# rileyhales/river-route

Hardware: AMD Instinct MI355X
Metric: reach-steps/sec (higher is better)
Workload: dtype f64

## Files before the change

### include/rr_hip.h

```cpp
#ifndef RR_HIP_H
#define RR_HIP_H

#include <stdint.h>

#ifdef __cplusplus
extern "C" {
#endif

#define RR_OK 0
#define RR_E_INVALID (-1)
#define RR_E_NOT_TOPOLOGICAL (-2)
#define RR_E_HIP (-3)
#define RR_E_NO_DEVICE (-4)
#define RR_E_STATE (-5)
#define RR_E_ALLOC (-6)
#define RR_E_UNSUPPORTED (-7)

#define RR_DEVICE_NONE (-1)

typedef struct rr_plan rr_plan;

int rr_version(void);
const char *rr_last_error(void);
int rr_device_count(void);


int rr_plan_create(int64_t n, const int32_t *csc_indptr, const int32_t *csc_indices, int device, rr_plan **out);
void rr_plan_destroy(rr_plan *plan);

int rr_plan_info(const rr_plan *plan, int64_t info[8]);

int rr_plan_layout(const rr_plan *plan, int32_t *perm, int32_t *lag, int32_t *child_ptr);

int rr_plan_tile_info(const rr_plan *plan, int64_t info[8]);
int rr_plan_tile_layout(const rr_plan *plan, int32_t *tile_ptr, int32_t *tile_level, int32_t *perm, int32_t *lag,
                        int32_t *cfirst, uint32_t *ccnt, int32_t *xpos);

int rr_plan_set_coeffs(rr_plan *plan, const double *lhs_off_data, const double *c2, const double *c3,
                       const double *c4_dt);

int rr_plan_set_unit_weights(rr_plan *plan, const double *c1, const double *a_data);

#define RR_MODE_RAPID 0
#define RR_MODE_MUSKINGUM 1
#define RR_MODE_UNIT 2
#define RR_ROWS_NOT_PLAIN 2
#define RR_ROWS_F32_OUT 4
#define RR_ROWS_UH 8
int rr_plan_reserve(rr_plan *plan, int mode, int64_t T, int64_t nsub, int host_rows, int64_t info[8]);

int rr_plan_direct_info(const rr_plan *plan, int64_t info[8], char *why, int64_t why_cap);
int rr_plan_direct_layout(const rr_plan *plan, int32_t *tile_c0, int32_t *tile_nc, int32_t *tile_lag_lo, int32_t *tile_span,
                          int32_t *delay, int32_t *up3, int32_t *xinfo);
int rr_plan_profile_aux(rr_plan *plan, double aux[12]);
#define RR_KERNEL_TICK 0
#define RR_KERNEL_TILE 1
#define RR_KERNEL_DIRECT 2
#define RR_KERNEL_TILE_ENSEMBLE 3
int rr_plan_last_kernel(const rr_plan *plan);

int rr_plan_set_row_format(rr_plan *plan, int in32_big_endian, int out32_big_endian);

int rr_plan_set_options(rr_plan *plan, int64_t rows_per_chunk, int64_t sample_every);

int rr_plan_profile(rr_plan *plan, double prof[10]);


int rr_rapid_route(rr_plan *plan, double *q_t, const double *qlateral, double *discharge,
                   int64_t num_runoff_steps, int64_t num_substeps);

int rr_muskingum_route(rr_plan *plan, double *q_t, double *discharge,
                       int64_t num_output_steps, int64_t num_routing_per_output);

int rr_unit_route(rr_plan *plan, double *q_ch, double *q_full, const double *convolved_lateral,
                  double *discharge, int64_t num_runoff_steps, int64_t num_substeps);

int rr_uh_convolve(int device, const double *kernel, double *state, const double *lateral, double *out,
                   int64_t T, int64_t n_ks, int64_t n);


int rr_rapid_route_dev(rr_plan *plan, double *q_t, const double *qlateral, int64_t ql_rows,
                       double *discharge, int64_t out_rows, int64_t num_runoff_steps, int64_t num_substeps,
                       void *stream);
int rr_muskingum_route_dev(rr_plan *plan, double *q_t, double *discharge, int64_t out_rows,
                           int64_t num_output_steps, int64_t num_routing_per_output, void *stream);
int rr_unit_route_dev(rr_plan *plan, double *q_ch, double *q_full, const double *convolved_lateral,
                      int64_t conv_rows, double *discharge, int64_t out_rows,
                      int64_t num_runoff_steps, int64_t num_substeps, void *stream);
int rr_uh_convolve_dev(int device, const double *kernel, double *state, const double *lateral, double *out,
                       int64_t T, int64_t n_ks, int64_t n, void *stream);

int rr_rapid_route_f32_dev(rr_plan *plan, double *q_t, const double *qlateral, int64_t ql_rows, float *discharge32,
                           int64_t num_runoff_steps, int64_t num_substeps, int64_t factor, void *stream);
int rr_rapid_route_f32in_dev(rr_plan *plan, double *q_t, const float *qlateral32, int64_t ql_rows, double *discharge, int64_t out_rows,
                             float *discharge32, int64_t factor, int64_t T, int64_t nsub, void *stream);

#define RR_ROWS_F32_IN 16
int rr_plan_reserve_ensemble(rr_plan *plan, int64_t members, int64_t T, int64_t nsub, int flags, int64_t info[9]);
int rr_rapid_route_ensemble_dev(rr_plan *plan, int64_t members, double *q_t, int64_t q_pitch, const void *lateral, int lateral_is_f32,
                                int64_t lateral_member_pitch, void *discharge, int discharge_is_f32, int64_t discharge_member_pitch,
                                int64_t factor, int64_t T, int64_t nsub, void *stream);
int rr_muskingum_route_f32_dev(rr_plan *plan, double *q_t, float *discharge32, int64_t num_output_steps,
                               int64_t num_routing_per_output, void *stream);
int rr_unit_route_f32_dev(rr_plan *plan, double *q_ch, double *q_full, const double *convolved_lateral, int64_t conv_rows,
                          float *discharge32, int64_t num_runoff_steps, int64_t num_substeps, int64_t factor, void *stream);

int rr_rapid_route_runoff_dev(rr_plan *plan, double *q_t, int64_t n_points, const int32_t *indptr, const int32_t *indices,
                              const double *weights, const void *runoff, int runoff_is_f32, int64_t stride_t, int64_t stride_p,
                              const double *area, int flags, double *discharge, float *discharge32, int64_t factor,
                              int64_t num_runoff_steps, void *stream);

int rr_unit_route_uh_dev(rr_plan *plan, double *q_ch, double *q_full, double *q_final, const double *uh_kernel, double *uh_state,
                         int64_t n_ks, const double *depth, double *discharge, float *discharge32, int64_t factor,
                         int64_t num_runoff_steps, int64_t num_substeps, void *stream);
int rr_unit_route_uh_f32in_dev(rr_plan *plan, double *q_ch, double *q_full, double *q_final, const double *uh_kernel, double *uh_state,
                               int64_t n_ks, const float *depth32, double *discharge, float *discharge32, int64_t factor,
                               int64_t num_runoff_steps, int64_t num_substeps, void *stream);


int rr_plan_set_boundary(rr_plan *plan, int64_t n_ghost, const int64_t *ghost_reaches, int64_t n_export,
                         const int64_t *export_reaches);

int rr_stream_begin(rr_plan *plan, int has_lateral, const double *q_t, const double *lateral, int64_t lat_rows,
                    double *discharge, int64_t out_rows, int64_t T, int64_t nsub, const double *ghost_series,
                    double *export_series, void *stream);
int rr_stream_advance(rr_plan *plan, int64_t lateral_rows_ready, int64_t ghost_substeps_ready,
                      int64_t *export_substeps_ready);
int rr_stream_end(rr_plan *plan, double *q_t);

int rr_stream_begin_unit(rr_plan *plan, const double *q_ch, const double *q_full, const double *lateral, int64_t lat_rows,
                         double *discharge, int64_t out_rows, int64_t T, int64_t nsub, const double *ghost_series,
                         double *export_series, void *stream);
int rr_stream_end_unit(rr_plan *plan, double *q_ch, double *q_full);

int rr_partition_forest(int64_t n, const int32_t *csc_indptr, const int32_t *csc_indices, int32_t n_parts,
                        int32_t *part_of, int64_t *part_sizes);

int rr_postorder(int64_t n, const int64_t *down_index, int64_t *order);

int rr_resample_cast_dev(int device, const double *discharge, int64_t num_rows, int64_t n, int64_t factor, float *out,
                         void *stream);

#define RR_RUNOFF_CUMULATIVE 1
#define RR_RUNOFF_FORCE_POSITIVE 2
#define RR_RUNOFF_KEEP_NAN 4
int rr_runoff_to_qlateral(int device, int64_t n_rivers, int64_t n_points, int64_t T, const int32_t *indptr,
                          const int32_t *indices, const double *weights, const void *runoff, int runoff_is_f32,
                          int64_t stride_t, int64_t stride_p, const double *area, int flags, double *qlateral);
int rr_runoff_to_qlateral_dev(int device, int64_t n_rivers, int64_t n_points, int64_t T, const int32_t *indptr,
                              const int32_t *indices, const double *weights, const void *runoff, int runoff_is_f32,
                              int64_t stride_t, int64_t stride_p, const double *area, int flags, double *qlateral,
                              void *stream);

#define RR_METRICS_STATE 9
#define RR_METRICS_SCORES 5
int rr_metrics_work_bytes(int64_t n, int64_t rows, int64_t *bytes);
int rr_metrics_update_dev(int device, int64_t n, int64_t rows, const void *y_true, int true_is_f32, int64_t true_pitch,
                          const void *y_pred, int pred_is_f32, int64_t pred_pitch, const int32_t *pred_columns, double *state,
                          void *work, int64_t work_bytes, void *stream);
int rr_metrics_finish_dev(int device, int64_t n, const double *state, double *out, void *stream);

int rr_grid_overlap_area(int device, int64_t n_rows, int64_t n_rings, int64_t n_vertices, int64_t nx, int64_t ny, int64_t n_pairs,
                         const int64_t *row_rings, const int64_t *ring_offsets, const double *ring_weight, const double *lon,
                         const double *lat, const double *x_bounds, const double *y_bounds, const int32_t *row_cells,
                         const int64_t *pair_offsets, double *area);
int rr_grid_overlap_area_dev(int device, int64_t n_rows, int64_t n_rings, int64_t n_vertices, int64_t nx, int64_t ny, int64_t n_pairs,
                             const int64_t *row_rings, const int64_t *ring_offsets, const double *ring_weight, const double *lon,
                             const double *lat, const double *x_bounds, const double *y_bounds, const int32_t *row_cells,
                             const int64_t *pair_offsets, double *area, void *stream);

int rr_rapid_adjoint_work_bytes(rr_plan *plan, int64_t T, int64_t nsub, int64_t *bytes);
int rr_rapid_adjoint_dev(rr_plan *plan, const double *q0, const double *lateral, int64_t lat_rows, const double *discharge,
                         const double *grad_out, const double *grad_qfinal, double *grad_lateral, double *grad_q0, double *grad_coef,
                         void *work, int64_t work_bytes, int64_t T, int64_t nsub, void *stream);

int rr_rapid_adjoint_batch_work_bytes(rr_plan *plan, int64_t members, int64_t T, int64_t nsub, int64_t *bytes);
int rr_rapid_adjoint_batch_dev(rr_plan *plan, int64_t members, const double *q0, int64_t q0_pitch, const double *lateral, int64_t lat_rows,
                               int64_t lat_pitch, const double *discharge, const double *grad_out, int64_t out_pitch,
                               const double *grad_qfinal, double *grad_lateral, double *grad_q0, double *grad_coef, void *work,
                               int64_t work_bytes, int64_t T, int64_t nsub, void *stream);

int rr_unit_adjoint_work_bytes(rr_plan *plan, int64_t T, int64_t nsub, int64_t *bytes);
int rr_unit_adjoint_dev(rr_plan *plan, const double *q_ch0, const double *q_full0, const double *lateral, int64_t lat_rows,
                        const double *discharge, const double *grad_out, const double *grad_qch_final, const double *grad_qfull_final,
                        double *grad_lateral, double *grad_qch0, double *grad_qfull0, double *grad_coef, void *work, int64_t work_bytes,
                        int64_t T, int64_t nsub, void *stream);

// ... 35 lines not shown
```

### river_route_amd/_lib.py

```python
from __future__ import annotations

import ctypes as C
import importlib.util
import os
import subprocess

import numpy as np

_HERE = os.path.dirname(os.path.abspath(__file__))
LIB_PATH = os.environ.get('RR_LIB_PATH') or os.path.join(_HERE, 'librr_hip.so')
CSRC = os.path.join(_HERE, 'csrc')
SOURCES = ('rr_plan.cpp', 'rr_engine.hip')

RR_OK = 0
RR_E_INVALID, RR_E_NOT_TOPOLOGICAL, RR_E_HIP, RR_E_NO_DEVICE, RR_E_STATE, RR_E_ALLOC, RR_E_UNSUPPORTED = \
    -1, -2, -3, -4, -5, -6, -7
RR_DEVICE_NONE = -1


class RRError(RuntimeError):
    def __init__(self, code: int, message: str):
        super().__init__(f'librr_hip error {code}: {message}')
        self.code = code
        self.message = message


SANITIZED_LIB_PATH = os.path.join(_HERE, 'librr_hip_asan.so')


def sanitizer_runtime() -> str | None:
    import glob
    found = sorted(glob.glob('/opt/rocm/lib/llvm/lib/clang/*/lib/linux/libclang_rt.asan-x86_64.so'))
    return found[-1] if found else None


def build(force: bool = False, verbose: bool = False, sanitize: bool = False) -> str:
    srcs = [os.path.join(CSRC, s) for s in SOURCES]
    deps = srcs + [os.path.join(CSRC, f) for f in sorted(os.listdir(CSRC)) if f.endswith('.hpp')] + [os.path.join(os.path.dirname(_HERE), 'include', 'rr_hip.h')]
    target = SANITIZED_LIB_PATH if sanitize else LIB_PATH
    if not force and os.path.exists(target) and all(os.path.getmtime(target) >= os.path.getmtime(d) for d in deps):
        return target
    hipcc = os.environ.get('HIPCC') or ('/opt/rocm/bin/hipcc' if os.path.exists('/opt/rocm/bin/hipcc') else 'hipcc')
    opt = ['-O1', '-g', '-fsanitize=address,undefined', '-fno-gpu-sanitize', '-fno-omit-frame-pointer', '-shared-libsan'] if sanitize else ['-O3']
    cmd = [hipcc, '--offload-arch=gfx950', *opt, '-std=c++17', '-fPIC', '-shared', '-pthread', '-Wall', '-Wno-unused-result',
           *srcs, '-o', target]
    if verbose:
        print(' '.join(cmd))
    subprocess.check_call(cmd)
    return target


def _preload_hip_runtime() -> None:
    try:
        spec = importlib.util.find_spec('torch')
    except (ImportError, ValueError):
        spec = None
    if spec is None or not spec.origin:
        return
    cand = os.path.join(os.path.dirname(spec.origin), 'lib', 'libamdhip64.so')
    if os.path.exists(cand):
        try:
            C.CDLL(cand, mode=C.RTLD_GLOBAL)
        except OSError:
            pass


_i64 = C.c_int64
_vp = C.c_void_p
_lib: C.CDLL | None = None

_SIGNATURES = {
    'rr_version': (C.c_int, []),
    'rr_last_error': (C.c_char_p, []),
    'rr_device_count': (C.c_int, []),
    'rr_plan_create': (C.c_int, [_i64, _vp, _vp, C.c_int, C.POINTER(_vp)]),
    'rr_plan_destroy': (None, [_vp]),
    'rr_plan_info': (C.c_int, [_vp, _vp]),
    'rr_plan_layout': (C.c_int, [_vp, _vp, _vp, _vp]),
    'rr_plan_tile_info': (C.c_int, [_vp, _vp]),
    'rr_plan_tile_layout': (C.c_int, [_vp, _vp, _vp, _vp, _vp, _vp, _vp, _vp]),
    'rr_plan_direct_info': (C.c_int, [_vp, _vp, _vp, _i64]),
    'rr_plan_direct_layout': (C.c_int, [_vp, _vp, _vp, _vp, _vp, _vp, _vp, _vp]),
    'rr_plan_last_kernel': (C.c_int, [_vp]),
    'rr_plan_set_coeffs': (C.c_int, [_vp, _vp, _vp, _vp, _vp]),
    'rr_plan_set_unit_weights': (C.c_int, [_vp, _vp, _vp]),
    'rr_plan_reserve': (C.c_int, [_vp, C.c_int, _i64, _i64, C.c_int, _vp]),
    'rr_plan_set_options': (C.c_int, [_vp, _i64, _i64]),
    'rr_plan_set_row_format': (C.c_int, [_vp, C.c_int, C.c_int]),
    'rr_plan_profile': (C.c_int, [_vp, _vp]),
    'rr_plan_profile_aux': (C.c_int, [_vp, _vp]),
    'rr_rapid_route': (C.c_int, [_vp, _vp, _vp, _vp, _i64, _i64]),
    'rr_muskingum_route': (C.c_int, [_vp, _vp, _vp, _i64, _i64]),
    'rr_unit_route': (C.c_int, [_vp, _vp, _vp, _vp, _vp, _i64, _i64]),
    'rr_uh_convolve': (C.c_int, [C.c_int, _vp, _vp, _vp, _vp, _i64, _i64, _i64]),
    'rr_rapid_route_dev': (C.c_int, [_vp, _vp, _vp, _i64, _vp, _i64, _i64, _i64, _vp]),
    'rr_muskingum_route_dev': (C.c_int, [_vp, _vp, _vp, _i64, _i64, _i64, _vp]),
    'rr_unit_route_dev': (C.c_int, [_vp, _vp, _vp, _vp, _i64, _vp, _i64, _i64, _i64, _vp]),
    'rr_uh_convolve_dev': (C.c_int, [C.c_int, _vp, _vp, _vp, _vp, _i64, _i64, _i64, _vp]),
    'rr_rapid_route_runoff_dev': (C.c_int, [_vp, _vp, _i64, _vp, _vp, _vp, _vp, C.c_int, _i64, _i64, _vp, C.c_int, _vp, _vp, _i64, _i64, _vp]),
    'rr_unit_route_uh_dev': (C.c_int, [_vp, _vp, _vp, _vp, _vp, _vp, _i64, _vp, _vp, _vp, _i64, _i64, _i64, _vp]),
    'rr_unit_route_uh_f32in_dev': (C.c_int, [_vp, _vp, _vp, _vp, _vp, _vp, _i64, _vp, _vp, _vp, _i64, _i64, _i64, _vp]),
    'rr_rapid_route_f32_dev': (C.c_int, [_vp, _vp, _vp, _i64, _vp, _i64, _i64, _i64, _vp]),
    'rr_rapid_route_f32in_dev': (C.c_int, [_vp, _vp, _vp, _i64, _vp, _i64, _vp, _i64, _i64, _i64, _vp]),
    'rr_plan_reserve_ensemble': (C.c_int, [_vp, _i64, _i64, _i64, C.c_int, _vp]),
    'rr_rapid_route_ensemble_dev': (C.c_int, [_vp, _i64, _vp, _i64, _vp, C.c_int, _i64, _vp, C.c_int, _i64, _i64, _i64, _i64, _vp]),
    'rr_muskingum_route_f32_dev': (C.c_int, [_vp, _vp, _vp, _i64, _i64, _vp]),
    'rr_unit_route_f32_dev': (C.c_int, [_vp, _vp, _vp, _vp, _i64, _vp, _i64, _i64, _i64, _vp]),
    'rr_plan_set_boundary': (C.c_int, [_vp, _i64, _vp, _i64, _vp]),
    'rr_stream_begin': (C.c_int, [_vp, C.c_int, _vp, _vp, _i64, _vp, _i64, _i64, _i64, _vp, _vp, _vp]),
    'rr_stream_advance': (C.c_int, [_vp, _i64, _i64, C.POINTER(_i64)]),
    'rr_stream_end': (C.c_int, [_vp, _vp]),
    'rr_stream_begin_unit': (C.c_int, [_vp, _vp, _vp, _vp, _i64, _vp, _i64, _i64, _i64, _vp, _vp, _vp]),
    'rr_stream_end_unit': (C.c_int, [_vp, _vp, _vp]),
    'rr_partition_forest': (C.c_int, [_i64, _vp, _vp, C.c_int32, _vp, _vp]),
    'rr_postorder': (C.c_int, [_i64, _vp, _vp]),
    'rr_resample_cast_dev': (C.c_int, [C.c_int, _vp, _i64, _i64, _i64, _vp, _vp]),
    'rr_runoff_to_qlateral': (C.c_int, [C.c_int, _i64, _i64, _i64, _vp, _vp, _vp, _vp, C.c_int, _i64, _i64, _vp, C.c_int, _vp]),
    'rr_runoff_to_qlateral_dev': (C.c_int, [C.c_int, _i64, _i64, _i64, _vp, _vp, _vp, _vp, C.c_int, _i64, _i64, _vp,
                                            C.c_int, _vp, _vp]),
    'rr_metrics_work_bytes': (C.c_int, [_i64, _i64, C.POINTER(_i64)]),
    'rr_metrics_update_dev': (C.c_int, [C.c_int, _i64, _i64, _vp, C.c_int, _i64, _vp, C.c_int, _i64, _vp, _vp, _vp, _i64, _vp]),
    'rr_metrics_finish_dev': (C.c_int, [C.c_int, _i64, _vp, _vp, _vp]),
    'rr_grid_overlap_area': (C.c_int, [C.c_int, _i64, _i64, _i64, _i64, _i64, _i64, _vp, _vp, _vp, _vp, _vp, _vp, _vp, _vp, _vp, _vp]),
    'rr_grid_overlap_area_dev': (C.c_int, [C.c_int, _i64, _i64, _i64, _i64, _i64, _i64, _vp, _vp, _vp, _vp, _vp, _vp, _vp, _vp, _vp, _vp,
                                           _vp]),
    'rr_rapid_adjoint_work_bytes': (C.c_int, [_vp, _i64, _i64, C.POINTER(_i64)]),
    'rr_rapid_adjoint_dev': (C.c_int, [_vp, _vp, _vp, _i64, _vp, _vp, _vp, _vp, _vp, _vp, _vp, _i64, _i64, _i64, _vp]),
    'rr_rapid_adjoint_batch_work_bytes': (C.c_int, [_vp, _i64, _i64, _i64, C.POINTER(_i64)]),
    'rr_rapid_adjoint_batch_dev': (C.c_int, [_vp, _i64, _vp, _i64, _vp, _i64, _i64, _vp, _vp, _i64, _vp, _vp, _vp, _vp, _vp, _i64, _i64, _i64, _vp]),
    'rr_unit_adjoint_work_bytes': (C.c_int, [_vp, _i64, _i64, C.POINTER(_i64)]),
    'rr_unit_adjoint_dev': (C.c_int, [_vp, _vp, _vp, _vp, _i64, _vp, _vp, _vp, _vp, _vp, _vp, _vp, _vp, _vp, _i64, _i64, _i64, _vp]),
    'rr_unit_adjoint_batch_work_bytes': (C.c_int, [_vp, _i64, _i64, _i64, C.POINTER(_i64)]),
    'rr_unit_adjoint_batch_dev': (C.c_int, [_vp, _i64, _vp, _vp, _i64, _vp, _i64, _i64, _vp, _vp, _i64, _vp, _vp, _vp, _vp, _vp, _vp, _vp, _i64,
                                            _i64, _i64, _vp]),
    'rr_uh_adjoint_work_bytes': (C.c_int, [_i64, _i64, _i64, C.POINTER(_i64)]),
    'rr_uh_adjoint_dev': (C.c_int, [C.c_int, _vp, _vp, _vp, _vp, _vp, _vp, _vp, _vp, _i64, _i64, _i64, _i64, _vp]),
    'rr_metrics_adjoint_work_bytes': (C.c_int, [_i64, C.POINTER(_i64)]),
    'rr_metrics_adjoint_dev': (C.c_int, [C.c_int, _i64, _i64, _vp, C.c_int, _i64, _vp, C.c_int, _i64, _vp, _vp, _i64, _vp, _vp, _vp, _vp, _i64,
                                         _vp, _i64, _vp]),
    'rr_dev_malloc': (C.c_int, [C.c_int, _i64, C.POINTER(_vp)]),
    'rr_dev_free': (C.c_int, [C.c_int, _vp]),
    'rr_dev_upload': (C.c_int, [C.c_int, _vp, _vp, _i64]),
    'rr_dev_download': (C.c_int, [C.c_int, _vp, _vp, _i64]),
    'rr_dev_synchronize': (C.c_int, [C.c_int]),
    'rr_copy_bandwidth': (C.c_int, [C.c_int, _i64, C.c_int, C.POINTER(C.c_double)]),
    'rr_rows_upload': (C.c_int, [C.c_int, _vp, _i64, C.c_char_p, _i64, _i64, _i64, _i64, _vp]),
    'rr_rows_download': (C.c_int, [C.c_int, _vp, _i64, C.c_char_p, _i64, _i64, _i64, _i64, _vp]),
}
EXPORTS = tuple(_SIGNATURES)


def lib() -> C.CDLL:
    global _lib
    if _lib is None:
        if not os.path.exists(LIB_PATH):
            raise RuntimeError(
                f'{LIB_PATH} is missing: the HIP engine is not built and there is no CPU fallback. '
                'Run `python -c "import __graft_entry__ as g; g.build()"` (needs hipcc) first.')
        _preload_hip_runtime()
        handle = C.CDLL(LIB_PATH)
        for name, (res, args) in _SIGNATURES.items():
            fn = getattr(handle, name)
            fn.restype = res
            fn.argtypes = args
        _lib = handle
    return _lib


def check(rc: int) -> None:
    if rc != RR_OK:
        raise RRError(rc, lib().rr_last_error().decode('utf-8', 'replace'))


def device_count() -> int:
    return int(lib().rr_device_count())


def ptr(a) -> int | None:
    if a is None:
        return None
    if isinstance(a, int):
        return a
    if isinstance(a, np.ndarray):
        if not a.flags['C_CONTIGUOUS']:
            raise ValueError('array must be C-contiguous')
        return a.ctypes.data
    if hasattr(a, 'address'):
        return int(a.address)
    if hasattr(a, 'data_ptr'):
        if not a.is_contiguous():
            raise ValueError('tensor must be contiguous')
        return a.data_ptr()
    raise TypeError(f'cannot take the address of {type(a).__name__}')
```

### river_route_amd/csrc/rr_engine.hip

```cpp
#include "rr_common.hpp"
#include "rr_kernels_tick.hpp"
#include "rr_kernels_tile.hpp"
#include "rr_kernels_uh.hpp"
#include "rr_kernels_rec.hpp"
#include "rr_kernels_runoff.hpp"
#include "rr_kernels_direct.hpp"
#include "rr_kernels_metrics.hpp"
#include "rr_kernels_overlap.hpp"
#include "rr_kernels_adjoint.hpp"
#include "rr_kernels_adjoint_unit.hpp"
#include "rr_exec.hpp"


extern "C" {

int rr_version(void) { return RR_VERSION_NUM; }

const char *rr_last_error(void) { return g_err.c_str(); }

int rr_device_count(void)
{
    int c = 0;
    if (hipGetDeviceCount(&c) != hipSuccess) return 0;
    return c;
}

void rr_plan_destroy(rr_plan *P)
{
    if (!P) return;
    if (P->device >= 0 && hipSetDevice(P->device) == hipSuccess) {
        void *ptrs[] = {P->d_child_ptr, P->d_lag, P->d_perm, P->d_inv, P->d_inner_pos, P->d_bidx, P->d_hwc, P->d_w, P->d_c1row_h, P->d_c2,
                        P->d_coef, P->d_coef_unit, P->d_sq, P->d_ss, P->d_si, P->d_sqch, P->d_full, P->d_chan,
                        P->d_tmeta, P->d_pmeta,
                        P->d_tperm, P->d_tinv, P->d_inner_idx, P->d_colmeta, P->d_ghostmeta, P->d_c4_params,
                        P->d_c3, P->d_c4, P->d_x, P->d_isum, P->d_qch, P->d_a2, P->d_c1own, P->d_z, P->d_ring, P->d_stage, P->d_mrows,
                        P->d_slot_a[0], P->d_slot_a[1], P->d_slot_b[0], P->d_slot_b[1], P->d_m_index[0], P->d_m_index[1],
                        P->d_dtiles, P->d_dlane, P->d_dsend_ptr, P->d_dsend_lane, P->d_dcoef, P->d_dq, P->d_ktmeta, P->d_kpmeta, P->d_kperm, P->d_kholecol, P->d_kcoef, P->d_ksq, P->d_kss, P->d_ksi, P->d_ksqch,
                        P->d_kholemeta, P->d_kghostmeta, P->d_esq, P->d_ess, P->d_esi, P->d_adj_down};
        for (void *p : ptrs) if (p) (void)hipFree(p);
        P->pipe.destroy();
        for (hipEvent_t e : P->ev) (void)hipEventDestroy(e);
        for (hipEvent_t e : P->aux_ev) (void)hipEventDestroy(e);
        if (P->ev_first) (void)hipEventDestroy(P->ev_first);
        if (P->ev_last) (void)hipEventDestroy(P->ev_last);
    }
    delete P;
}

int rr_plan_create(int64_t n, const int32_t *csc_indptr, const int32_t *csc_indices, int device, rr_plan **out)
{
    if (!out) return fail(RR_E_INVALID, "rr_plan_create: null out");
    *out = nullptr;
    rr_plan *P = new (std::nothrow) rr_plan();
    if (!P) return fail(RR_E_ALLOC, "rr_plan_create: out of memory");
    if (const char *e = getenv("RR_WAVE")) { P->wave_enabled = atoi(e) != 0; P->wave_forced = atoi(e) == 1; }
    if (const char *e = getenv("RR_REC_BATCHES")) { P->rec_batches = std::max(1, std::min(kRecMaxLaunchBatches, atoi(e))); P->rec_batches_forced = true; }
    if (const char *e = getenv("RR_WAVE_K")) P->wave_K = std::max(kRec, atoi(e) / kRec * kRec);
    std::string err;
    int rc = rr::build_host_plan(n, csc_indptr, csc_indices, P->h, err);
    if (rc) { delete P; return fail(rc, err); }
    if (device != RR_DEVICE_NONE) {
        int count = rr_device_count(), cus = 0;
        if (device >= 0 && device < count && hipDeviceGetAttribute(&cus, hipDeviceAttributeMultiprocessorCount, device) == hipSuccess && cus > 0) P->cu_count = cus;
    }
    {
        P->wave_threads = kTileThreads;
        int32_t block = P->wave_threads;
        if (const char *e = getenv("RR_TILE_BLOCK")) block = std::max(8, std::min(block, atoi(e)));
        std::vector<int32_t> lag_of((size_t)n);
        for (int64_t i = 0; i < n; ++i) lag_of[i] = P->h.lag[P->h.inv[i]];
        rr::build_tile_plan(P->h.down, lag_of, block, P->tp);
        if (const char *e = getenv("RR_DIRECT")) P->direct_enabled = atoi(e) != 0;
        P->direct_block = block;
        rr::build_direct_plan(P->h.down, lag_of, std::min<int32_t>(kDirectLanes, block), kDirectMaxWindow - 2, block, P->dp);
        P->direct_window = 3;
        for (int32_t sp : P->dp.tile_span) P->direct_window = std::max(P->direct_window, sp + 3);
    }
    if (device != RR_DEVICE_NONE) {
        int count = rr_device_count();
        if (device < 0 || device >= count) {
            delete P;
            return fail(RR_E_NO_DEVICE, "rr_plan_create: HIP device " + std::to_string(device) + " not available (" +
                                            std::to_string(count) + " visible)");
        }
        hipError_t e = hipSetDevice(device);
        if (e != hipSuccess) { delete P; return fail(RR_E_HIP, hipGetErrorString(e)); }
        P->device = device;
        {
            size_t free_b = 0, total_b = 0;
            if (hipMemGetInfo(&free_b, &total_b) == hipSuccess) P->dev_total_bytes = total_b;
        }
        if (const char *e2 = getenv("RR_TILE_LEAN")) P->lean_enabled = atoi(e2) != 0;
        for (int v = 0; v < 7; ++v)
            if (hipFuncSetAttribute((const void *)tile_kernel(v < 4 ? (v & 1) != 0 : v == 5, v < 4 && (v & 2) != 0, v >= 4, v == 6), hipFuncAttributeMaxDynamicSharedMemorySize,
                                    (int)tile_lds_bytes(P->wave_threads)) != hipSuccess) {
                (void)hipGetLastError();
                P->wave_enabled = false;
            }
        for (int v = 0; v < 2; ++v)
            if (hipFuncSetAttribute((const void *)tile_ens_kernel(v == 1), hipFuncAttributeMaxDynamicSharedMemorySize, (int)tile_lds_bytes(kTileThreads)) != hipSuccess) {
                (void)hipGetLastError();
                P->ens_enabled = false;
            }
        if (const char *e2 = getenv("RR_UH_PAIRS")) P->uh_pairs = atoi(e2) != 0;
        for (int v = 0; v < 4; ++v)
            (void)hipFuncSetAttribute((const void *)rec_in_uh_kernel((v & 1) != 0, 64, 1 + (v >> 1)), hipFuncAttributeMaxDynamicSharedMemorySize, (int)rec_in_uh_lds_bytes(64, 1 + (v >> 1)));
        (void)hipGetLastError();
        const rr::HostPlan &H = P->h;
        const int64_t ni = (int64_t)H.inner_pos.size();
        rc = dev_alloc(&P->d_child_ptr, n + 1);
        if (!rc) rc = dev_alloc(&P->d_lag, n);
        if (!rc) rc = dev_alloc(&P->d_perm, n);
        if (!rc) rc = dev_alloc(&P->d_inv, n);
        if (!rc) rc = dev_alloc(&P->d_inner_pos, ni);
        if (!rc) rc = dev_alloc(&P->d_hwc, n);
        if (!rc) rc = dev_alloc(&P->d_bidx, n);
        if (!rc) rc = dev_alloc(&P->d_c4_params, n);
        if (!rc && P->tp.ok) {
            const rr::TilePlan &TP = P->tp;
            const int64_t np = TP.np;
            std::vector<int2> cm(n);
            for (int64_t i = 0; i < n; ++i)
                cm[i] = make_int2(TP.inv[i], (TP.lag[TP.inv[i]] & kLagMask) | (H.child_ptr[H.inv[i] + 1] == H.child_ptr[H.inv[i]] ? kColHeadwater : 0));
            std::vector<int32_t> inner_idx;
            inner_idx.reserve(ni);
            for (int64_t i = 0; i < n; ++i) if (H.child_ptr[H.inv[i] + 1] > H.child_ptr[H.inv[i]]) inner_idx.push_back((int32_t)i);
            rc = dev_alloc(&P->d_colmeta, n);
            if (!rc) rc = dev_upload(P->d_colmeta, cm);
            if (!rc) rc = dev_alloc(&P->d_inner_idx, ni);
            if (!rc) rc = dev_upload(P->d_inner_idx, inner_idx);
            if (!rc) rc = upload_tile_meta(P, TP.lag, TP.xpos, TP.tile_flags);
            for (int32_t f : TP.tile_flags) P->n_wide_tiles += (f & kTileWide) ? 1 : 0;
            if (!rc) rc = dev_alloc(&P->d_tperm, np);
            if (!rc) rc = dev_upload(P->d_tperm, TP.perm);
            if (!rc) rc = dev_alloc(&P->d_tinv, n);
            if (!rc) rc = dev_upload(P->d_tinv, TP.inv);
            if (!rc) rc = dev_alloc(&P->d_coef, 3 * np);
            if (!rc) rc = dev_alloc(&P->d_coef_unit, 3 * np);
            if (!rc) rc = dev_alloc(&P->d_sq, np);
            if (!rc) rc = dev_alloc(&P->d_ss, np);
            if (!rc) rc = dev_alloc(&P->d_si, np);
            if (!rc) rc = dev_alloc(&P->d_sqch, np);
            if (!rc) rc = dev_alloc(&P->d_full, n);
            if (!rc) rc = dev_alloc(&P->d_chan, n);
        }
        if (!rc) rc = upload_direct_plan(P);
        if (!rc) rc = dev_alloc(&P->d_w, n);
        if (!rc) rc = dev_alloc(&P->d_c1row_h, n);
        if (!rc) rc = dev_alloc(&P->d_c2, n);
        if (!rc) rc = dev_alloc(&P->d_c3, n);
        if (!rc) rc = dev_alloc(&P->d_c4, n);
        if (!rc) rc = dev_alloc(&P->d_x, 3 * n);
        if (!rc) rc = dev_alloc(&P->d_isum, n);
        if (!rc) rc = dev_alloc(&P->d_qch, n);
        if (!rc) rc = dev_upload(P->d_child_ptr, H.child_ptr);
        if (!rc) rc = dev_upload(P->d_lag, H.lag);
        if (!rc) rc = dev_upload(P->d_perm, H.perm);
        if (!rc) rc = dev_upload(P->d_inv, H.inv);
        if (!rc) rc = dev_upload(P->d_inner_pos, H.inner_pos);
        if (!rc) rc = dev_upload(P->d_hwc, H.hw_children);
        if (rc) { rr_plan_destroy(P); return rc; }
    }
    *out = P;
    return RR_OK;
}

int rr_plan_info(const rr_plan *P, int64_t info[8])
{
    if (!P || !info) return fail(RR_E_INVALID, "rr_plan_info: null argument");
    info[0] = P->h.n; info[1] = P->h.n_edges; info[2] = P->h.depth; info[3] = P->h.widest_level;
    info[4] = P->h.n_headwaters; info[5] = P->h.n_outlets; info[6] = P->h.identity ? 1 : 0; info[7] = P->device;
    return RR_OK;
}

int rr_plan_layout(const rr_plan *P, int32_t *perm, int32_t *lag, int32_t *child_ptr)
{
    if (!P) return fail(RR_E_INVALID, "rr_plan_layout: null plan");
    const size_t n = (size_t)P->h.n;
    if (perm && n) std::memcpy(perm, P->h.perm.data(), n * sizeof(int32_t));
    if (lag && n) std::memcpy(lag, P->h.lag.data(), n * sizeof(int32_t));
    if (child_ptr) std::memcpy(child_ptr, P->h.child_ptr.data(), (n + 1) * sizeof(int32_t));
    return RR_OK;
}

int rr_plan_tile_info(const rr_plan *P, int64_t info[8])
{
    if (!P || !info) return fail(RR_E_INVALID, "rr_plan_tile_info: null argument");
    const rr::TilePlan &T = P->tp;
    info[0] = T.ok ? 1 : 0; info[1] = T.block; info[2] = T.np; info[3] = T.n_ghost; info[4] = T.n_tiles; info[5] = T.n_levels;
    info[6] = P->wave_threads; info[7] = kRecRows;
    return RR_OK;
}

int rr_plan_tile_layout(const rr_plan *P, int32_t *tile_ptr, int32_t *tile_level, int32_t *perm, int32_t *lag, int32_t *cfirst,
                        uint32_t *ccnt, int32_t *xpos)
{
    if (!P) return fail(RR_E_INVALID, "rr_plan_tile_layout: null plan");
    const rr::TilePlan &T = P->tp;
    if (!T.ok) return fail(RR_E_UNSUPPORTED, "rr_plan_tile_layout: this network does not tile (a reach has more upstream reaches than a tile holds)");
    auto copy = [](auto *dst, const auto &src) { if (dst && !src.empty()) std::memcpy(dst, src.data(), src.size() * sizeof(src[0])); };
    copy(tile_ptr, T.tile_ptr); copy(tile_level, T.tile_level); copy(perm, T.perm); copy(lag, T.lag); copy(cfirst, T.cfirst);
    copy(ccnt, T.ccnt); copy(xpos, T.xpos);
    return RR_OK;
}

int rr_plan_direct_info(const rr_plan *P, int64_t info[8], char *why, int64_t why_cap)
{
    if (!P || !info) return fail(RR_E_INVALID, "rr_plan_direct_info: null argument");
    const rr::DirectPlan &D = P->dp;
    info[0] = D.ok ? 1 : 0; info[1] = D.n_tiles; info[2] = D.n_holes; info[3] = D.n_exports; info[4] = D.skel.np; info[5] = D.skel.n_tiles;
    info[6] = D.skel.n_levels; info[7] = P->direct_window;
    if (why && why_cap > 0) { std::strncpy(why, D.why.c_str(), (size_t)why_cap - 1); why[why_cap - 1] = 0; }
    return RR_OK;
}

int rr_plan_direct_layout(const rr_plan *P, int32_t *tile_c0, int32_t *tile_nc, int32_t *tile_lag_lo, int32_t *tile_span, int32_t *delay, int32_t *up3, int32_t *xinfo)
{
    if (!P) return fail(RR_E_INVALID, "rr_plan_direct_layout: null plan");
    const rr::DirectPlan &D = P->dp;
    if (!D.ok) return fail(RR_E_UNSUPPORTED, "rr_plan_direct_layout: the direct row path does not apply to this plan: " + D.why);
    auto copy = [](auto *dst, const auto &src) { if (dst && !src.empty()) std::memcpy(dst, src.data(), src.size() * sizeof(src[0])); };
    copy(tile_c0, D.tile_c0); copy(tile_nc, D.tile_nc); copy(tile_lag_lo, D.tile_lag_lo); copy(tile_span, D.tile_span);
    copy(delay, D.delay); copy(up3, D.up3); copy(xinfo, D.xinfo);
    return RR_OK;
}

int rr_plan_last_kernel(const rr_plan *P)
{
    if (!P) return -1;
    return P->ses.members > 0 ? RR_KERNEL_TILE_ENSEMBLE : (int)P->ses.kernel;
}

int rr_plan_set_options(rr_plan *P, int64_t rows_per_chunk, int64_t sample_every)
{
    if (!P) return fail(RR_E_INVALID, "rr_plan_set_options: null plan");
    if (rows_per_chunk > 0) P->chunk_rows = rows_per_chunk;
    if (sample_every >= 0) P->sample_every = sample_every;
    return RR_OK;
}

int rr_plan_set_row_format(rr_plan *P, int in32_big_endian, int out32_big_endian)
{
    if (!P) return fail(RR_E_INVALID, "rr_plan_set_row_format: null plan");
    if (P->ses.open) return fail(RR_E_STATE, "rr_plan_set_row_format: a routing call is open");
    P->in32_big_endian = in32_big_endian != 0; P->out32_big_endian = out32_big_endian != 0;
    return RR_OK;
}

int rr_plan_set_coeffs(rr_plan *P, const double *lhs_off_data, const double *c2, const double *c3, const double *c4_dt)
{
    int rc = need_device(P);
    if (rc) return rc;
    const rr::HostPlan &H = P->h;
    const int64_t n = H.n;
    if (n > 0 && (!c2 || !c3 || (H.n_edges > 0 && !lhs_off_data)))
        return fail(RR_E_INVALID, "rr_plan_set_coeffs: null coefficient array");
    std::vector<double> w(n), a2(n), a3(n), a4(n, 0.0);
    for (int64_t p = 0; p < n; ++p) {
        const int32_t i = H.perm[p];
        const int32_t e = H.edge_of[i];
        w[p] = e >= 0 ? -lhs_off_data[e] : 0.0;
        a2[p] = c2[i];
        a3[p] = c3[i];
        if (c4_dt) a4[p] = c4_dt[i];
    }
    std::vector<double> c1row(n, 0.0);
    bool uniform = true;
    for (int64_t p = 0; p < n; ++p) {
        const int32_t u0 = H.child_ptr[p], u1 = H.child_ptr[p + 1];
        if (u1 > u0) c1row[p] = w[u0];
        for (int32_t u = u0 + 1; u < u1; ++u) if (w[u] != w[u0]) uniform = false;
    }
    P->weights_uniform = uniform;
    rc = dev_upload(P->d_w, w);
    if (!rc) rc = dev_upload(P->d_c1row_h, c1row);
    if (!rc && P->tp.ok) {
        const rr::TilePlan &TP = P->tp;
        P->h_coef.assign(3 * TP.np, 0.0);
        for (int64_t p = 0; p < TP.np; ++p) {
            if (TP.lag[p] & kTileGhostBit) continue;
            const int32_t i = TP.perm[p];
            P->h_coef[3 * p] = c1row[H.inv[i]]; P->h_coef[3 * p + 1] = c2[i]; P->h_coef[3 * p + 2] = c3[i];
        }
        rc = upload_tile_coef(P);
    }
    {
        P->h_dcoef.assign(4 * (size_t)n, 0.0);
        for (int64_t i = 0; i < n; ++i) { P->h_dcoef[4 * i] = c1row[H.inv[i]]; P->h_dcoef[4 * i + 1] = c2[i]; P->h_dcoef[4 * i + 2] = c3[i]; P->h_dcoef[4 * i + 3] = c4_dt ? c4_dt[i] : 0.0; }
        if (!rc) rc = upload_direct_coef(P);
    }
    if (!rc) rc = dev_upload(P->d_c2, a2);
    if (!rc) rc = dev_upload(P->d_c3, a3);
    if (!rc) rc = dev_upload(P->d_c4, a4);
    if (!rc && c4_dt && n > 0) {
        hipError_t e = hipMemcpy(P->d_c4_params, c4_dt, (size_t)n * sizeof(double), hipMemcpyHostToDevice);
        if (e != hipSuccess) rc = fail(RR_E_HIP, hipGetErrorString(e));
    }
    if (rc) return rc;
    P->coeffs_set = true;
    P->has_c4 = c4_dt != nullptr;
    return RR_OK;
}

int rr_plan_set_unit_weights(rr_plan *P, const double *c1, const double *a_data)
{
    int rc = need_device(P);
    if (rc) return rc;
    if (P->ses.open) return fail(RR_E_STATE, "rr_plan_set_unit_weights: a routing call is open");
    if (!c1 && !a_data) { P->unit_general = false; return RR_OK; }
    const rr::HostPlan &H = P->h;
    const int64_t n = H.n;
    if (!c1 || (H.n_edges > 0 && !a_data)) return fail(RR_E_INVALID, "rr_plan_set_unit_weights: give both arrays, or neither to go back to unit weights");
    if (P->n_ghost > 0 || P->n_export > 0) return fail(RR_E_UNSUPPORTED, "rr_plan_set_unit_weights: general edge data on a partitioned network is not supported");
    std::vector<double> a2(n, 0.0), own(n, 0.0);
    for (int64_t p = 0; p < n; ++p) {
        const int32_t i = H.perm[p], e = H.edge_of[i];
        a2[p] = e >= 0 ? a_data[e] : 0.0;
        own[p] = c1[i];
    }
    if (!P->d_a2) rc = dev_alloc(&P->d_a2, n);
    if (!rc && !P->d_c1own) rc = dev_alloc(&P->d_c1own, n);
    if (!rc && !P->d_z) rc = dev_alloc(&P->d_z, 3 * n);
    if (!rc) rc = dev_upload(P->d_a2, a2);
    if (!rc) rc = dev_upload(P->d_c1own, own);
    if (rc) return rc;
    P->unit_general = true;
    return RR_OK;
}

int rr_plan_reserve(rr_plan *P, int mode, int64_t T, int64_t nsub, int host_rows, int64_t info[8])
{
    int rc = need_device(P);
    if (rc) return rc;
    if (mode < RR_MODE_RAPID || mode > RR_MODE_UNIT || T < 0 || nsub < 1) return fail(RR_E_INVALID, "rr_plan_reserve: unknown mode, negative step count or sub-steps < 1");
    if (!P->coeffs_set) return fail(RR_E_STATE, "rr_plan_reserve before rr_plan_set_coeffs (per-edge weights decide which kernel routes)");
    if (P->ses.open) return fail(RR_E_STATE, "rr_plan_reserve: a routing call is open");
    const Mode m = mode == RR_MODE_RAPID ? Mode::Rapid : (mode == RR_MODE_MUSKINGUM ? Mode::Muskingum : Mode::Unit);
    CallShape shape;
    shape.mode = m; shape.T = T; shape.nsub = nsub;
    shape.host = (host_rows & 1) != 0;
    shape.dev_rows = !shape.host && (host_rows & RR_ROWS_NOT_PLAIN) == 0;
    shape.out32 = (host_rows & RR_ROWS_F32_OUT) != 0;
    shape.uh = (host_rows & RR_ROWS_UH) != 0;
// ... 1210 lines not shown
```

### river_route_amd/csrc/rr_exec.hpp

```cpp
#pragma once


enum class Mode { Rapid, Muskingum, Unit };

struct Rows {
    const double *dev_in = nullptr;
    const float *dev_in32 = nullptr;
    const double *host_in = nullptr;
    int64_t rows_in = 0;
    double *dev_out = nullptr;
    double *host_out = nullptr;
    int64_t rows_out = 0;
    float *dev_out32 = nullptr;
    int64_t out_factor = 1;
    const double *uh_kernel = nullptr, *uh_state = nullptr;
    int64_t uh_nks = 0;
    const RunoffArgs *runoff = nullptr;
    int64_t members = 0, in_pitch = 0, out_pitch = 0;
};

struct CallShape {
    Mode mode = Mode::Rapid;
    int64_t T = 0, nsub = 1;
    bool host = false;
    bool dev_rows = false;
    bool in32 = false;
    bool out32 = false;
    int64_t factor = 1;
    bool uh = false;
    bool runoff = false;
    int64_t ring_in = 0, ring_out = 0;
    int64_t members = 0;
};

enum class Kernel { Tick = RR_KERNEL_TICK, Tile = RR_KERNEL_TILE, Direct = RR_KERNEL_DIRECT };

struct Schedule {
    Kernel kernel = Kernel::Tick;
    int64_t KC = 1;
    int64_t KS = 1;
    int64_t chunks = 0;
    int64_t ring = 0;
    int64_t mrows = 0, stage = 0;
    int64_t rec_nb = 1;
};

struct Session {
    bool open = false;
    Mode mode = Mode::Rapid;
    int64_t T = 0, nsub = 1, total = 0, total_ticks = 0;
    Rows io;
    hipStream_t stream = nullptr;
    Kernel kernel = Kernel::Tick;
    bool in_place = false;
    bool has_in = true;
    int64_t ring_rows = 0;
    int64_t rows_loaded = 0, rows_stored = 0, tau = 0;
    const double *ghost_series = nullptr;
    double *export_series = nullptr;
    TickArgs a{};
    int64_t KC = 1;
    int64_t rec_chunks = 0, in_batches = 0, n_in_batches = 0, out_batches = 0, n_out_batches = 0;
    int64_t rec_nb = 1;
    int64_t ticks_stored = 0;
    int64_t out_limit = std::numeric_limits<int64_t>::max();
    int64_t diag = 0, n_diags = 0, n_macro = 0;
    int64_t ghost_batches = 0;
    int64_t ghost_slack = 0, export_skew = 0;
    TileArgs ta{};
    int64_t n_tasks = 0;
    int64_t d_done = 0;
    int64_t KS = 1;
    bool export_lanes = false, export_skel = false;
    DirectArgs da{};
    bool bracket_open = false;
    int64_t bracket_reaches = 0;
    size_t max_samples = 0;
    int64_t members = 0;
    int64_t ring_stride = 0;
};

struct HostPipe {
    static constexpr int kPinned = 3, kCopyThreads = 8;
    int copy_threads = kCopyThreads;
    int64_t chunk_mib = 512;
    int64_t chunk_rows = 64, ring_chunks = 8;
    double *pin_in[kPinned] = {nullptr, nullptr, nullptr}, *pin_out[kPinned] = {nullptr, nullptr, nullptr};
    double *dev_in = nullptr, *dev_out = nullptr;
    int64_t pin_cap = 0, dev_cap = 0;
    hipStream_t s_h2d = nullptr, s_d2h = nullptr;
    std::vector<hipEvent_t> ev_h2d, ev_d2h, ev_adv;
    void destroy()
    {
        for (int k = 0; k < kPinned; ++k) { if (pin_in[k]) (void)hipHostFree(pin_in[k]); if (pin_out[k]) (void)hipHostFree(pin_out[k]); pin_in[k] = pin_out[k] = nullptr; }
        if (dev_in) (void)hipFree(dev_in);
        if (dev_out) (void)hipFree(dev_out);
        dev_in = dev_out = nullptr; pin_cap = dev_cap = 0;
        for (auto *v : {&ev_h2d, &ev_d2h, &ev_adv}) { for (hipEvent_t e : *v) (void)hipEventDestroy(e); v->clear(); }
        if (s_h2d) (void)hipStreamDestroy(s_h2d);
        if (s_d2h) (void)hipStreamDestroy(s_d2h);
        s_h2d = s_d2h = nullptr;
    }
};

struct rr_plan {
    rr::HostPlan h;
    int device = RR_DEVICE_NONE;
    bool coeffs_set = false, has_c4 = false;
    int64_t chunk_rows = 16, sample_every = 0;

    int32_t *d_child_ptr = nullptr, *d_lag = nullptr, *d_perm = nullptr, *d_inv = nullptr, *d_inner_pos = nullptr;
    int32_t *d_bidx = nullptr;
    uint16_t *d_hwc = nullptr;
    double *d_w = nullptr, *d_c1row_h = nullptr, *d_c2 = nullptr, *d_c3 = nullptr, *d_c4 = nullptr;
    double *d_x = nullptr, *d_isum = nullptr, *d_qch = nullptr;
    double *d_a2 = nullptr, *d_c1own = nullptr, *d_z = nullptr;
    bool unit_general = false;
    double *d_ring = nullptr;
    int64_t ring_cap = 0;
    double *d_stage = nullptr;
    int64_t stage_cap = 0;
    double *d_mrows = nullptr;
    int64_t mrows_cap = 0;
    uint16_t *d_slot_a[2] = {nullptr, nullptr}, *d_slot_b[2] = {nullptr, nullptr};
    int32_t *d_m_index[2] = {nullptr, nullptr};
    int64_t perm_rows_per_block = 2;

    rr::TilePlan tp;
    bool wave_enabled = true, wave_forced = false, weights_uniform = false;
    bool ens_enabled = true;
    int wave_threads = 512;
    int64_t wave_K = 0;
    Schedule sch;
    int64_t kc_cap = int64_t{1} << 20;
    TileMeta *d_tmeta = nullptr;
    int4 *d_pmeta = nullptr;
    int32_t *d_tperm = nullptr, *d_tinv = nullptr;
    int32_t *d_inner_idx = nullptr;
    bool export_inside = false;
    double *d_coef = nullptr;
    double *d_coef_unit = nullptr;
    std::vector<double> h_coef;
    int32_t n_wide_tiles = 0;
    double *d_sq = nullptr, *d_ss = nullptr, *d_si = nullptr, *d_sqch = nullptr;
    double *d_esq = nullptr, *d_ess = nullptr, *d_esi = nullptr;
    int64_t ens_cap = 0;
    double *d_full = nullptr, *d_chan = nullptr;
    int2 *d_colmeta = nullptr;
    int2 *d_ghostmeta = nullptr;
    double *d_c4_params = nullptr;
    size_t dev_total_bytes = 0;
    int cu_count = 256;

    int64_t n_ghost = 0, n_export = 0;
    int64_t ghost_min_lag = 0, export_max_lag = 0;
    std::vector<int32_t> ghost_reach, export_reach;

    Session ses;
    HostPipe pipe;
    rr::DirectPlan dp;
    bool direct_enabled = true;
    bool uh_rows_ok = true;
    int direct_window = 1;
    DirectTile *d_dtiles = nullptr;
    int4 *d_dlane = nullptr;
    int32_t *d_dsend_ptr = nullptr, *d_dsend_lane = nullptr;
    double *d_dcoef = nullptr, *d_dq = nullptr;
    TileMeta *d_ktmeta = nullptr;
    int4 *d_kpmeta = nullptr;
    int32_t *d_kperm = nullptr, *d_kholecol = nullptr;
    double *d_kcoef = nullptr, *d_ksq = nullptr, *d_kss = nullptr, *d_ksi = nullptr, *d_ksqch = nullptr;
    int2 *d_kholemeta = nullptr;
    int2 *d_kghostmeta = nullptr;
    std::vector<double> h_dcoef;
    int32_t direct_block = 0;
    int64_t n_kholes = 0;
    int32_t n_kwide = 0;
    bool in32_big_endian = false, out32_big_endian = false;
    bool lean_enabled = true;
    bool uh_pairs = true;
    int32_t rec_batches = kRecLaunchBatches;
    bool rec_batches_forced = false;
    bool perm_ready = false;
    int32_t *d_adj_down = nullptr;

    static constexpr int kAuxKinds = 4, kAuxSamples = 256;
    std::vector<hipEvent_t> aux_ev;
    std::vector<int> aux_kind;
    int64_t aux_launches[kAuxKinds] = {0, 0, 0, 0};
    std::vector<hipEvent_t> ev;
    std::vector<int64_t> ev_reaches;
    hipEvent_t ev_first = nullptr, ev_last = nullptr;
    int64_t prof_launches = 0, prof_samples = 0, prof_brackets = 0, prof_reach_steps = 0;
    hipStream_t last_stream = nullptr;
};

namespace {

template <typename T>
int dev_alloc(T **p, int64_t count)
{
    *p = nullptr;
    if (count <= 0) count = 1;
    hipError_t e = hipMalloc((void **)p, (size_t)count * sizeof(T));
    if (e != hipSuccess)
        return fail(RR_E_ALLOC, std::string("hipMalloc of ") + std::to_string((size_t)count * sizeof(T)) +
                                    " bytes failed: " + hipGetErrorString(e));
    return RR_OK;
}

template <typename T>
int dev_upload(T *dst, const std::vector<T> &src)
{
    if (src.empty()) return RR_OK;
    HIPCHK(hipMemcpy(dst, src.data(), src.size() * sizeof(T), hipMemcpyHostToDevice));
    return RR_OK;
}

int need_device(const rr_plan *plan)
{
    if (!plan) return fail(RR_E_INVALID, "null plan");
    if (plan->device < 0)
        return fail(RR_E_NO_DEVICE, "this plan is host-only (RR_DEVICE_NONE): the HIP engine has no CPU fallback");
    HIPCHK(hipSetDevice(plan->device));
    return RR_OK;
}

template <typename T>
int ensure_cap(T **buf, int64_t *cap, int64_t count)
{
    if (*cap >= count) return RR_OK;
    if (*buf) { (void)hipFree(*buf); *buf = nullptr; *cap = 0; }
    int rc = dev_alloc(buf, count);
    if (rc) return rc;
    *cap = count;
    return RR_OK;
}

int upload_tile_meta(rr_plan *P, const std::vector<int32_t> &lag, const std::vector<int32_t> &xpos, const std::vector<int32_t> &flags)
{
    const rr::TilePlan &TP = P->tp;
    std::vector<TileMeta> tm((size_t)TP.n_tiles);
    for (int32_t t = 0; t < TP.n_tiles; ++t)
        tm[t] = TileMeta{TP.tile_ptr[t], TP.tile_ptr[t + 1], TP.tile_level[t], TP.tile_lag_lo[t], TP.tile_lag_hi[t], flags[t], 0, 0};
    std::vector<int4> pm((size_t)TP.np);
    for (int64_t p = 0; p < TP.np; ++p) pm[p] = make_int4(lag[p], TP.cfirst[p], xpos[p], (int32_t)TP.ccnt[p]);
    int rc = RR_OK;
    if (!P->d_tmeta) rc = dev_alloc(&P->d_tmeta, TP.n_tiles);
    if (!rc && !P->d_pmeta) rc = dev_alloc(&P->d_pmeta, TP.np);
    if (!rc) rc = dev_upload(P->d_tmeta, tm);
    if (!rc) rc = dev_upload(P->d_pmeta, pm);
    return rc;
}

int upload_tile_coef(rr_plan *P)
{
    if (P->h_coef.empty()) return RR_OK;
    std::vector<double> coef(P->h_coef);
    for (int32_t i : P->ghost_reach) { const int64_t p = P->tp.inv[i]; coef[3 * p] = coef[3 * p + 1] = coef[3 * p + 2] = 0.0; }
    int rc = dev_upload(P->d_coef, coef);
    if (rc) return rc;
    for (int64_t p = 0; p < P->tp.np; ++p)
        if ((P->tp.ccnt[p] & 0xFFFFu) == 0) coef[3 * p] = coef[3 * p + 1] = coef[3 * p + 2] = 0.0;
    return dev_upload(P->d_coef_unit, coef);
}

typedef void (*direct_kernel_t)(const DirectArgs);
direct_kernel_t direct_kernel(bool in32, bool out32, bool sub = false, int unit = 0)
{
    if (unit == 1)
        return sub ? (out32 ? (direct_kernel_t)k_direct<kDirectAhead, false, true, true, 1> : (direct_kernel_t)k_direct<kDirectAhead, false, false, true, 1>)
                   : (out32 ? (direct_kernel_t)k_direct<kDirectAhead, false, true, false, 1> : (direct_kernel_t)k_direct<kDirectAhead, false, false, false, 1>);
#define RR_DK(I_, O_) (sub ? (direct_kernel_t)k_direct<kDirectAhead, I_, O_, true> : (direct_kernel_t)k_direct<kDirectAhead, I_, O_, false>)
    return in32 ? (out32 ? RR_DK(true, true) : RR_DK(true, false)) : (out32 ? RR_DK(false, true) : RR_DK(false, false));
#undef RR_DK
}

int upload_direct_plan(rr_plan *P)
{
    void *old[] = {P->d_dtiles, P->d_dlane, P->d_dsend_ptr, P->d_dsend_lane, P->d_dcoef, P->d_dq, P->d_ktmeta, P->d_kpmeta, P->d_kperm, P->d_kholecol, P->d_kcoef,
                   P->d_ksq, P->d_kss, P->d_ksi, P->d_ksqch, P->d_kholemeta, P->d_kghostmeta};
    for (void *p : old) if (p) (void)hipFree(p);
    P->d_dtiles = nullptr; P->d_dlane = nullptr; P->d_dsend_ptr = P->d_dsend_lane = nullptr; P->d_dcoef = P->d_dq = nullptr; P->d_ktmeta = nullptr; P->d_kpmeta = nullptr;
    P->d_kperm = P->d_kholecol = nullptr; P->d_kcoef = P->d_ksq = P->d_kss = P->d_ksi = P->d_ksqch = nullptr; P->d_kholemeta = P->d_kghostmeta = nullptr;
    P->n_kholes = 0; P->n_kwide = 0;
    P->direct_window = 3;
    for (int32_t sp : P->dp.tile_span) P->direct_window = std::max(P->direct_window, sp + 3);
    if (!P->dp.ok || P->device < 0) return RR_OK;
    const rr::HostPlan &H = P->h;
    const rr::DirectPlan &D = P->dp;
    const rr::TilePlan &K = D.skel;
    const int64_t n = H.n;
    for (int v = 0; v < 12; ++v)
        if (hipFuncSetAttribute((const void *)direct_kernel(v < 8 && (v & 1) != 0, (v & 2) != 0, v < 8 ? (v & 4) != 0 : (v & 1) != 0, v >= 8 ? 1 : 0), hipFuncAttributeMaxDynamicSharedMemorySize, (int)direct_lds_bytes(kDirectMaxWindow)) != hipSuccess) {
            (void)hipGetLastError();
            P->direct_enabled = false;
        }
    std::vector<DirectTile> dt((size_t)D.n_tiles);
    for (int32_t t = 0; t < D.n_tiles; ++t) dt[t] = DirectTile{D.tile_c0[t], D.tile_nc[t], D.tile_lag_lo[t], D.tile_span[t]};
    std::vector<int4> dl((size_t)n);
    for (int64_t i = 0; i < n; ++i) dl[i] = make_int4(D.delay[i], D.up3[i], D.xinfo[i], H.lag[H.inv[i]]);
    int rc = dev_alloc(&P->d_dtiles, D.n_tiles);
    if (!rc) rc = dev_upload(P->d_dtiles, dt);
    if (!rc) rc = dev_alloc(&P->d_dlane, n);
    if (!rc) rc = dev_upload(P->d_dlane, dl);
    if (!rc) rc = dev_alloc(&P->d_dsend_ptr, D.n_tiles + 1);
    if (!rc) rc = dev_upload(P->d_dsend_ptr, D.send_ptr);
    if (!rc) rc = dev_alloc(&P->d_dsend_lane, (int64_t)D.send_lane.size());
    if (!rc) rc = dev_upload(P->d_dsend_lane, D.send_lane);
    if (!rc) rc = dev_alloc(&P->d_dcoef, 4 * n);
    if (!rc) rc = dev_alloc(&P->d_dq, n);
    std::vector<TileMeta> tm((size_t)K.n_tiles);
    std::vector<int32_t> klag(K.lag), kxpos(K.xpos), kflags(K.tile_flags);
    for (size_t e = 0; e < P->export_reach.size(); ++e) {
        const int32_t i = P->export_reach[e];
        if (!D.big[i]) continue;
        const int32_t p = K.inv[i];
        klag[p] |= kExportBit; kxpos[p] = (int32_t)e; kflags[K.tile_of[p]] |= kTileExports;
    }
    for (int32_t t = 0; t < K.n_tiles; ++t) {
        tm[t] = TileMeta{K.tile_ptr[t], K.tile_ptr[t + 1], K.tile_level[t], K.tile_lag_lo[t], K.tile_lag_hi[t], kflags[t], 0, 0};
        P->n_kwide += (kflags[t] & kTileWide) ? 1 : 0;
    }
    std::vector<int4> pm((size_t)K.np);
    for (int64_t p = 0; p < K.np; ++p) pm[p] = make_int4(klag[p], K.cfirst[p], kxpos[p], (int32_t)K.ccnt[p]);
    std::vector<int2> hm, gm;
    std::vector<int32_t> hc;
    for (int64_t i = 0; i < n; ++i)
        if (D.big[i]) { hm.push_back(make_int2(K.inv[i], K.lag[K.inv[i]] & kLagMask)); hc.push_back((int32_t)i); }
    for (int32_t i : P->ghost_reach) { const int32_t g = K.ext_ghost[i]; gm.push_back(make_int2(g, K.lag[g] & kLagMask)); }
    P->n_kholes = (int64_t)hm.size();
    if (!rc) rc = dev_alloc(&P->d_ktmeta, K.n_tiles);
    if (!rc) rc = dev_upload(P->d_ktmeta, tm);
    if (!rc) rc = dev_alloc(&P->d_kpmeta, K.np);
    if (!rc) rc = dev_upload(P->d_kpmeta, pm);
    if (!rc) rc = dev_alloc(&P->d_kperm, K.np);
    if (!rc) rc = dev_upload(P->d_kperm, K.perm);
    if (!rc) rc = dev_alloc(&P->d_kcoef, 3 * K.np);
    if (!rc) rc = dev_alloc(&P->d_ksq, K.np);
    if (!rc) rc = dev_alloc(&P->d_kss, K.np);
    if (!rc) rc = dev_alloc(&P->d_ksi, K.np);
    if (!rc) rc = dev_alloc(&P->d_ksqch, K.np);
    if (!rc) rc = dev_alloc(&P->d_kholemeta, P->n_kholes);
    if (!rc) rc = dev_upload(P->d_kholemeta, hm);
    if (!rc) rc = dev_alloc(&P->d_kholecol, P->n_kholes);
    if (!rc) rc = dev_upload(P->d_kholecol, hc);
    if (!rc) rc = dev_alloc(&P->d_kghostmeta, (int64_t)gm.size());
    if (!rc) rc = dev_upload(P->d_kghostmeta, gm);
    return rc;
}

int upload_direct_coef(rr_plan *P)
{
    if (!P->dp.ok || P->device < 0 || P->h_dcoef.empty()) return RR_OK;
    int rc = dev_upload(P->d_dcoef, P->h_dcoef);
    const rr::TilePlan &K = P->dp.skel;
    std::vector<double> kc(3 * (size_t)K.np, 0.0);
    for (int64_t p = 0; p < K.np; ++p) {
        if (K.lag[p] & kTileGhostBit) continue;
        const int64_t i = K.perm[p];
        kc[3 * p] = P->h_dcoef[4 * i]; kc[3 * p + 1] = P->h_dcoef[4 * i + 1]; kc[3 * p + 2] = P->h_dcoef[4 * i + 2];
    }
    if (!rc) rc = dev_upload(P->d_kcoef, kc);
    return rc;
}

int upload_tiled_permutations(rr_plan *P)
{
    const rr::HostPlan &H = P->h;
    const int64_t n = H.n;
    const int32_t *pis[2] = {H.perm.data(), H.inv.data()};
    int rc = RR_OK;
    for (int w = 0; w < 2 && !rc; ++w) {
        rr::TiledPermutation tp;
        rr::build_tiled_permutation(pis[w], n, kPermE * kPermThreads, tp);
        rc = dev_alloc(&P->d_slot_a[w], n);
        if (!rc) rc = dev_alloc(&P->d_slot_b[w], n);
        if (!rc) rc = dev_alloc(&P->d_m_index[w], n);
        if (!rc) rc = dev_upload(P->d_slot_a[w], tp.slot_a);
        if (!rc) rc = dev_upload(P->d_slot_b[w], tp.slot_b);
        if (!rc) rc = dev_upload(P->d_m_index[w], tp.m_index);
    }
    if (rc) {
        for (int w = 0; w < 2; ++w) {
            if (P->d_slot_a[w]) (void)hipFree(P->d_slot_a[w]);
            if (P->d_slot_b[w]) (void)hipFree(P->d_slot_b[w]);
            if (P->d_m_index[w]) (void)hipFree(P->d_m_index[w]);
            P->d_slot_a[w] = P->d_slot_b[w] = nullptr; P->d_m_index[w] = nullptr;
        }
        return rc;
    }
    P->perm_ready = true;
    return RR_OK;
}

int aux_begin(rr_plan *P, int kind, hipStream_t stream)
{
    const int64_t seq = P->aux_launches[kind]++;
    if (P->sample_every < kSampleGroup || (seq & 3) != 0 || 2 * (P->aux_kind.size() + 1) > P->aux_ev.size()) return -1;
    if (hipEventRecord(P->aux_ev[2 * P->aux_kind.size()], stream) != hipSuccess) return -1;
    P->aux_kind.push_back(kind);
    return (int)P->aux_kind.size() - 1;
}
void aux_end(rr_plan *P, int sample, hipStream_t stream)
{
    if (sample >= 0) (void)hipEventRecord(P->aux_ev[2 * sample + 1], stream);
}


int64_t pick_KC(const rr_plan *P, int64_t total_ticks)
{
    if (P->wave_K > 0) return std::max<int64_t>(1, std::min<int64_t>(P->wave_K, 256) / kRec);
    return total_ticks >= 32768 ? 16 : (total_ticks >= 16384 ? 8 : (total_ticks >= 4096 ? 4 : (total_ticks >= 512 ? 2 : 1)));
}
// ... 80 lines not shown
        const int64_t C = std::max<int64_t>(1, P->chunk_rows), lag_rows = (dmax + nsub - 1) / std::max<int64_t>(1, nsub);
        const bool in_place = P->h.identity && !s.host;
        sch.ring = in_place ? 0 : std::min<int64_t>(T, lag_rows + 2 * C + 2) * n;
        sch.mrows = in_place ? 0 : C * n;
        sch.stage = s.host ? C * n : 0;
    }
    return sch;
}

int host_pipe_prepare(rr_plan *P);

int reserve_core(rr_plan *P, const CallShape &s, Schedule *out)
{
    if (P->h.n == 0 || s.T <= 0) { *out = Schedule(); return RR_OK; }
    Schedule sch;
    for (;;) {
        sch = choose_schedule(P, s);
        if (sch.kernel == Kernel::Direct && s.uh && ensure_cap(&P->d_mrows, &P->mrows_cap, sch.mrows) != RR_OK) {
            (void)hipGetLastError();
            P->uh_rows_ok = false;
            continue;
        }
        if (ensure_cap(&P->d_ring, &P->ring_cap, sch.ring) == RR_OK) break;
        (void)hipGetLastError();
        if (sch.kernel == Kernel::Direct) return fail(RR_E_ALLOC, "route: the skeleton's record ring does not fit on the device");
        if (sch.kernel == Kernel::Tick) return fail(RR_E_ALLOC, "route: the work rows of the streaming kernel do not fit on the device");
        if (s.members > 0) return fail(RR_E_ALLOC, "route: the record rings of " + std::to_string(s.members) + " ensemble members do not fit on the device");
        P->kc_cap = sch.KC / 2;
    }
    int rc = ensure_cap(&P->d_mrows, &P->mrows_cap, sch.mrows);
    if (!rc) rc = ensure_cap(&P->d_stage, &P->stage_cap, sch.stage);
    if (!rc && sch.kernel == Kernel::Tick && !P->perm_ready) rc = upload_tiled_permutations(P);
    if (!rc && sch.kernel == Kernel::Tile && s.host) rc = host_pipe_prepare(P);
    if (rc) return rc;
    if (!P->ev_first) { HIPCHK(hipEventCreate(&P->ev_first)); HIPCHK(hipEventCreate(&P->ev_last)); }
    const int64_t K = sch.KC * kRec, total_ticks = s.T * s.nsub + P->h.depth - 1;
    size_t samples = P->sample_every >= kSampleGroup ? (size_t)std::min<int64_t>(4096, total_ticks / P->sample_every + 1) : 0;
    if (sch.kernel == Kernel::Tile && samples > 0) samples = (size_t)std::min<int64_t>(4096, ((total_ticks + K - 1) / K + P->tp.n_levels) / 4 + 1);
    if (sch.kernel == Kernel::Direct && samples > 0) samples = (size_t)std::min<int64_t>(4096, (s.T + K - 1) / K + 1);
    while (P->ev.size() < 2 * samples) { hipEvent_t e; HIPCHK(hipEventCreate(&e)); P->ev.push_back(e); }
    if (samples > 0) while (P->aux_ev.size() < 2 * rr_plan::kAuxSamples) { hipEvent_t e; HIPCHK(hipEventCreate(&e)); P->aux_ev.push_back(e); }
    *out = sch;
    return RR_OK;
}

int prepare_call(rr_plan *P, const CallShape &s, const char *who)
{
    if (s.host) return reserve_core(P, s, &P->sch);
    if (s.out32 && (s.factor < 1 || s.T % s.factor != 0))
        return fail(RR_E_INVALID, std::string(who) + ": float32 output: the number of rows must be a multiple of factor >= 1");
    if (s.out32 && kRecRows % (s.factor * s.nsub) != 0)
        return fail(RR_E_UNSUPPORTED, std::string(who) + ": float32 output: factor x sub-steps must divide the rows of a record batch (128)");
    const Schedule sch = choose_schedule(P, s);
    if ((s.in32 || s.out32 || s.uh || s.runoff) && sch.kernel == Kernel::Tick)
        return fail(RR_E_UNSUPPORTED, std::string(who) + " needs the time-tiled kernel or the direct row path, which this call does not get");
    const size_t samples = P->sample_every >= kSampleGroup ? 1 : 0;
    if (P->h.n > 0 && s.T > 0 && (sch.ring > P->ring_cap || sch.mrows > P->mrows_cap || sch.stage > P->stage_cap || !P->ev_first || P->ev.size() < 2 * samples ||
                                  (sch.kernel == Kernel::Tick && !P->perm_ready && sch.mrows > 0)))
        return fail(RR_E_STATE, "this call needs " + std::to_string((sch.ring + sch.mrows + sch.stage) * 8) + " bytes of work memory on the device (" +
                                    std::to_string((P->ring_cap + P->mrows_cap + P->stage_cap) * 8) + " reserved): call " +
                                    (s.members > 0 ? "rr_plan_reserve_ensemble(plan, " + std::to_string(s.members) + ", " : std::string("rr_plan_reserve(plan, mode, ")) +
                                    std::to_string(s.T) + ", " + std::to_string(s.nsub) + ", ...) first; the *_dev entry points only enqueue work");
    P->sch = sch;
    return RR_OK;
}

hipStream_t rec_stream(const rr_plan *P) { return P->ses.stream; }

int session_begin(rr_plan *P, Mode mode, int64_t T, int64_t nsub, const Rows &io, hipStream_t stream,
                  const double *ghost_series, double *export_series)
{
    const rr::HostPlan &H = P->h;
    const int64_t n = H.n;
    Session &S = P->ses;
    if (S.open) return fail(RR_E_STATE, "a routing call is already open on this plan (rr_stream_end it first)");
    S = Session();
    S.mode = mode; S.T = T; S.nsub = nsub; S.total = T * nsub; S.io = io; S.stream = stream;
    S.members = io.members;
    S.ghost_series = ghost_series; S.export_series = export_series;
    const int64_t dmax = H.depth - 1;
    S.total_ticks = S.total + dmax;
    if (S.total_ticks >= (int64_t{1} << 31) - (int64_t{1} << 20) || io.rows_in >= (int64_t{1} << 31) || io.rows_out >= (int64_t{1} << 31))
        return fail(RR_E_UNSUPPORTED, "more than 2^31 routing ticks or rows in one call: split it into several calls");
    S.has_in = mode != Mode::Muskingum;
    const bool host_io = io.host_out != nullptr || io.host_in != nullptr;
    S.kernel = P->sch.kernel;
    S.in_place = H.identity && !host_io && S.kernel == Kernel::Tick;
    const int64_t C = std::max<int64_t>(1, P->chunk_rows);

    P->prof_launches = P->prof_samples = P->prof_brackets = 0;
    P->aux_kind.clear();
    for (int k = 0; k < rr_plan::kAuxKinds; ++k) P->aux_launches[k] = 0;
    P->prof_reach_steps = n * S.total * std::max<int64_t>(1, S.members);
    P->ev_reaches.clear();
    P->last_stream = stream;
    S.open = true;
    if (n == 0 || S.total == 0) return RR_OK;
    if (P->n_ghost > 0 && !ghost_series) { S.open = false; return fail(RR_E_INVALID, "plan has ghost reaches but no ghost series was given"); }
    if (P->n_export > 0 && !export_series) { S.open = false; return fail(RR_E_INVALID, "plan has export reaches but no export series was given"); }

    S.KC = P->sch.KC; S.KS = P->sch.KS; S.rec_chunks = P->sch.chunks;
    S.rec_nb = S.kernel == Kernel::Tile ? std::max<int64_t>(1, P->sch.rec_nb) : 1;
    if (S.kernel == Kernel::Direct) {
        if (io.uh_kernel || io.runoff || (!io.dev_out && !io.dev_out32) || (mode == Mode::Unit && (io.dev_in32 || P->n_ghost > 0 || P->n_export > 0)) || nsub > kDirectMaxSub ||
            (io.dev_out32 && (io.out_factor < 1 || (S.KC * kRec) % io.out_factor != 0 || T % io.out_factor != 0))) {
            S.open = false;
            return fail(RR_E_STATE, "route: the direct row path was chosen for a call it does not take");
        }
        const rr::TilePlan &TP = P->dp.skel;
        const int64_t K = S.KC * kRec;
        S.n_tasks = (S.T + K - 1) / K;
        S.n_macro = (S.total_ticks + S.KS * kRec - 1) / (S.KS * kRec);
        S.n_diags = TP.n_tiles > 0 ? S.n_macro + TP.n_levels - 1 : 0;
        S.n_in_batches = (S.total + 14) / kRecRows + 1;
        S.n_out_batches = TP.np > 0 ? (S.total + kRecRows - 1) / kRecRows : 0;
        S.export_skew = 0; S.export_lanes = S.export_skel = false;
        for (int32_t i : P->export_reach) {
            if (!P->dp.big[i]) { S.export_lanes = true; continue; }
            S.export_skel = true;
            const int32_t p = TP.inv[i];
            S.export_skew = std::max<int64_t>(S.export_skew, (int64_t)TP.tile_level[TP.tile_of[p]] * S.KS * kRec + (TP.lag[p] & kLagMask));
        }
        DirectArgs &da = S.da;
        da.tiles = P->d_dtiles; da.n_tiles = P->dp.n_tiles; da.lane = P->d_dlane; da.coef = P->d_dcoef; da.q = P->d_dq; da.qch = nullptr;
        if (mode == Mode::Unit) { da.q = P->d_full; da.qch = P->d_chan; }
        da.send_ptr = P->d_dsend_ptr; da.send_lane = P->d_dsend_lane;
        da.in = S.has_in ? io.dev_in : nullptr; da.out = io.dev_out; da.n = n; da.in_rows = (uint32_t)std::max<int64_t>(1, io.rows_in); da.out_rows = (uint32_t)std::max<int64_t>(1, io.rows_out);
        da.in32 = S.has_in ? io.dev_in32 : nullptr; da.out32 = io.dev_out32; da.factor = (int32_t)std::max<int64_t>(1, io.out_factor);
        da.nsub = (int32_t)nsub; da.inv_nsub = 1.0 / (double)nsub;
        da.in32_sel = P->in32_big_endian ? kSelSwap : kSelNative; da.out32_sel = P->out32_big_endian ? kSelSwap : kSelNative;
        da.rec = P->d_ring; da.rec_chunks = (uint32_t)std::max<int64_t>(1, S.rec_chunks); da.np = (int32_t)TP.np;
        da.K = (int32_t)K; da.total = (int32_t)S.T;
        da.exports = export_series; da.n_export = (int32_t)P->n_export;
        TileArgs &w = S.ta;
        w.tiles = P->d_ktmeta; w.pos = P->d_kpmeta; w.coef = P->d_kcoef;
        w.sq = P->d_ksq; w.ss = P->d_kss; w.si = P->d_ksi; w.sqch = P->d_ksqch;
        w.np = (int32_t)TP.np; w.KC = (int32_t)S.KS;
    }
    if (S.kernel == Kernel::Tile) {
        const rr::TilePlan &TP = P->tp;
        const int64_t K = S.KC * kRec;
        S.n_macro = (S.total_ticks + K - 1) / K;
        S.n_diags = S.n_macro + TP.n_levels - 1;
        S.n_in_batches = (S.total + 14) / kRecRows + 1;
        S.n_out_batches = (S.total + kRecRows - 1) / kRecRows;
        S.export_skew = 0;
        S.ghost_slack = P->ghost_reach.empty() ? 0 : S.total_ticks + (int64_t)TP.n_levels * K;
        for (int32_t i : P->ghost_reach) { const int32_t p = TP.inv[i]; S.ghost_slack = std::min<int64_t>(S.ghost_slack, (int64_t)TP.tile_level[TP.tile_of[p]] * K + (TP.lag[p] & kLagMask)); }
        for (int32_t i : P->export_reach) { const int32_t p = TP.inv[i]; S.export_skew = std::max<int64_t>(S.export_skew, (int64_t)TP.tile_level[TP.tile_of[p]] * K + (TP.lag[p] & kLagMask)); }
        TileArgs &w = S.ta;
        w.tiles = P->d_tmeta; w.pos = P->d_pmeta; w.coef = P->d_coef;
        w.sq = P->d_sq; w.ss = P->d_ss; w.si = P->d_si; w.sqch = P->d_sqch;
        w.np = (int32_t)TP.np; w.KC = (int32_t)S.KC;
        if (S.members > 0) {
            if (S.members > P->ens_cap || (S.rec_chunks * kRec * TP.np) * S.members > P->ring_cap) { S.open = false; return fail(RR_E_STATE, "route: the ensemble was not reserved"); }
            S.ring_stride = S.rec_chunks * kRec * TP.np;
            w.sq = P->d_esq; w.ss = P->d_ess; w.si = P->d_esi; w.sqch = nullptr;
        }
    }
    if (S.kernel != Kernel::Tick) {
        TileArgs &w = S.ta;
        w.exports = export_series; w.n_export = (int32_t)P->n_export;
        w.rec = P->d_ring; w.rec_chunks = Div32((uint32_t)S.rec_chunks);
        w.n_macro = (int32_t)S.n_macro; w.total = (int32_t)S.total;
        w.has_lat = S.has_in ? 1 : 0; w.nsub = Div32((uint32_t)nsub); w.inv_nsub = 1.0 / (double)nsub;
    }
    if (getenv("RR_VERBOSE") && S.kernel == Kernel::Direct)
        fprintf(stderr, "rr: n=%lld T=%lld direct rows: K=%lld tiles=%d window=%d holes=%lld outlets=%lld; skeleton: positions=%lld tiles=%d levels=%d ring_chunks=%lld (%.1f GB)\n",
                (long long)n, (long long)T, (long long)(S.KC * kRec), P->dp.n_tiles, P->direct_window, (long long)P->dp.n_holes, (long long)P->dp.n_exports,
                (long long)P->dp.skel.np, P->dp.skel.n_tiles, P->dp.skel.n_levels, (long long)S.rec_chunks, (double)S.rec_chunks * kRec * P->dp.skel.np * 8 / 1e9);
    else if (getenv("RR_VERBOSE"))
        fprintf(stderr, "rr: n=%lld T=%lld nsub=%lld tiled=%d K=%lld tiles=%d levels=%d block=%d ghosts=%lld ring_chunks=%lld (%.1f GB) rec_batches=%lld lds=%zu\n",
                (long long)n, (long long)T, (long long)nsub, (int)(S.kernel == Kernel::Tile), (long long)(S.KC * kRec), P->tp.n_tiles, P->tp.n_levels, P->tp.block,
                (long long)P->tp.n_ghost, (long long)S.rec_chunks, S.kernel == Kernel::Tile ? (double)S.rec_chunks * kRec * P->tp.np * 8 / 1e9 : 0.0,
                (long long)S.rec_nb, tile_lds_bytes(P->wave_threads));
    if (S.kernel == Kernel::Tick) {
        const int64_t lag_rows = (dmax + nsub - 1) / nsub;
        S.ring_rows = S.in_place ? 0 : std::min<int64_t>(T, lag_rows + 2 * C + 2);
        if (S.ring_rows > 0xFFFFFFFFLL || T > 0x7FFFFFFFLL) { S.open = false; return fail(RR_E_INVALID, "route: too many time rows"); }
        if (S.ring_rows * n > P->ring_cap || (!S.in_place && C * n > P->mrows_cap) || (host_io && C * n > P->stage_cap)) {
            S.open = false;
            return fail(RR_E_STATE, "route: work rows of the streaming kernel were not reserved");
        }
        TickArgs &a = S.a;
        a.child_ptr = P->d_child_ptr; a.lag = P->d_lag; a.w = P->d_w; a.c2 = P->d_c2; a.c3 = P->d_c3; a.c4 = P->d_c4;
        a.c1row = P->weights_uniform ? P->d_c1row_h : nullptr;
        a.isum = P->d_isum; a.bidx = P->d_bidx;
        a.ghost = ghost_series; a.exports = export_series; a.n_ghost = (int32_t)P->n_ghost; a.n_export = (int32_t)P->n_export;
        a.total_substeps = S.total; a.nsub = Div32((uint32_t)nsub); a.inv_nsub = 1.0 / (double)nsub;
        if (S.in_place) {
            a.in = io.dev_in; a.in_ld = n; a.in_rows = Div32((uint32_t)std::max<int64_t>(1, io.rows_in));
            a.out = io.dev_out; a.out_ld = n; a.out_rows = Div32((uint32_t)io.rows_out);
        } else {
            a.in = S.has_in ? P->d_ring : nullptr; a.in_ld = n; a.in_rows = Div32((uint32_t)S.ring_rows);
            a.out = P->d_ring; a.out_ld = n; a.out_rows = Div32((uint32_t)S.ring_rows);
        }
    }
    S.max_samples = P->sample_every >= kSampleGroup ? (size_t)std::min<int64_t>(4096, S.total_ticks / P->sample_every + 1) : 0;
    if (S.kernel == Kernel::Tile && S.max_samples > 0) S.max_samples = (size_t)std::min<int64_t>(4096, S.n_diags / 4 + 1);
    if (S.kernel == Kernel::Direct && S.max_samples > 0) S.max_samples = (size_t)std::min<int64_t>(4096, S.n_tasks);
    S.max_samples = std::min(S.max_samples, P->ev.size() / 2);
    if (!P->ev_first) { S.open = false; return fail(RR_E_STATE, "route: the plan's events were not reserved"); }
    HIPCHK(hipEventRecord(P->ev_first, stream));
    return RR_OK;
}

void permute_rows_via(rr_plan *P, int which, const RowView &src, const RowView &dst, int64_t t0, int nrows, double *mrows, hipStream_t stream)
{
    const int64_t n = P->h.n;
    constexpr int E = kPermE;
    const int64_t tile = (int64_t)E * kPermThreads;
    const int rpb = (int)std::max<int64_t>(1, P->perm_rows_per_block);
    dim3 g((unsigned)((n + tile - 1) / tile), (unsigned)((nrows + rpb - 1) / rpb));
    const size_t lds_bytes = (size_t)tile * sizeof(double);
    hipLaunchKernelGGL(k_perm_a<E>, g, dim3(kPermThreads), lds_bytes, stream, src, mrows, n,
                       (const uint16_t *)P->d_slot_a[which], (const int32_t *)P->d_m_index[which], t0, nrows, rpb);
    hipLaunchKernelGGL(k_perm_b<E>, g, dim3(kPermThreads), lds_bytes, stream, dst, (const double *)mrows, n,
                       (const uint16_t *)P->d_slot_b[which], t0, nrows, rpb);
}

void permute_rows(rr_plan *P, int which, const RowView &src, const RowView &dst, int64_t t0, int nrows)
{
    permute_rows_via(P, which, src, dst, t0, nrows, P->d_mrows, P->ses.stream);
}

int session_load_rows(rr_plan *P, int64_t r0, int64_t r1)
{
    Session &S = P->ses;
    if (S.in_place || !S.has_in) return RR_OK;
    const int64_t n = P->h.n, C = std::max<int64_t>(1, P->chunk_rows);
    const int nrows = (int)(r1 - r0);
    const RowView ring_view{P->d_ring, n, 0, (uint32_t)std::max<int64_t>(1, S.ring_rows)};
    if (S.io.host_in) {
        HIPCHK(hipMemcpyAsync(P->d_stage, S.io.host_in + r0 * n, (size_t)nrows * n * sizeof(double),
                              hipMemcpyHostToDevice, S.stream));
        permute_rows(P, 0, RowView{P->d_stage, n, r0, (uint32_t)C}, ring_view, r0, nrows);
        HIPCHK(hipStreamSynchronize(S.stream));
    } else {
        permute_rows(P, 0, RowView{const_cast<double *>(S.io.dev_in), n, 0, (uint32_t)S.io.rows_in}, ring_view, r0, nrows);
    }
    return RR_OK;
}

int session_store_rows(rr_plan *P, int64_t r0, int64_t r1)
{
    Session &S = P->ses;
    if (S.in_place) return RR_OK;
    const int64_t n = P->h.n, C = std::max<int64_t>(1, P->chunk_rows);
    const RowView ring_view{P->d_ring, n, 0, (uint32_t)std::max<int64_t>(1, S.ring_rows)};
    for (int64_t b0 = r0; b0 < r1; b0 += C) {
        const int nrows = (int)std::min<int64_t>(C, r1 - b0);
        if (S.io.host_out) {
            permute_rows(P, 1, ring_view, RowView{P->d_stage, n, b0, (uint32_t)C}, b0, nrows);
            HIPCHK(hipMemcpyAsync(S.io.host_out + b0 * n, P->d_stage, (size_t)nrows * n * sizeof(double),
                                  hipMemcpyDeviceToHost, S.stream));
            HIPCHK(hipStreamSynchronize(S.stream));
        } else {
            permute_rows(P, 1, ring_view, RowView{S.io.dev_out, n, 0, (uint32_t)S.io.rows_out}, b0, nrows);
        }
    }
    return RR_OK;
}

inline bool tick_window(const rr::HostPlan &H, int64_t tau, int64_t total, int64_t &p_lo, int64_t &p_hi)
{
    p_lo = H.lag_start[std::max<int64_t>(0, tau - total + 1)];
    p_hi = H.lag_start[std::min<int64_t>(tau, H.depth - 1) + 1];
    return p_hi > p_lo;
}

int session_launch_tick(rr_plan *P, int64_t tau)
{
    Session &S = P->ses;
    const int64_t n = P->h.n;
    int64_t p_lo, p_hi;
    if (!tick_window(P->h, tau, S.total, p_lo, p_hi)) return RR_OK;
    TickArgs &a = S.a;
    a.p_lo = (int32_t)p_lo; a.p_hi = (int32_t)p_hi; a.tau = tau;
    a.xc = P->d_x + (tau % 3) * n;
    a.xa = P->d_x + ((tau + 2) % 3) * n;
    a.xb = P->d_x + ((tau + 1) % 3) * n;
    const int64_t phase = S.max_samples > 0 ? P->prof_launches % P->sample_every : -1;
    if (phase == 0 && !S.bracket_open && (size_t)P->prof_brackets < S.max_samples) {
        HIPCHK(hipEventRecord(P->ev[2 * P->prof_brackets], S.stream));
        S.bracket_open = true;
    }
    const dim3 g = grid1(p_hi - p_lo);
    const bool one = S.nsub == 1;
    if (S.mode == Mode::Unit) {
        UnitTickArgs ua{};
        ua.t = a; ua.hw_children = P->d_hwc; ua.qch = P->d_qch;
        ua.a2 = P->unit_general ? P->d_a2 : nullptr; ua.c1own = P->d_c1own;
        if (P->unit_general) { ua.t.c1row = nullptr; ua.zc = P->d_z + (tau % 3) * n; ua.za = P->d_z + ((tau + 2) % 3) * n; }
        if (one) hipLaunchKernelGGL(k_tick_unit<true>, g, dim3(kBlock), 0, S.stream, ua);
        else hipLaunchKernelGGL(k_tick_unit<false>, g, dim3(kBlock), 0, S.stream, ua);
    } else if (S.mode == Mode::Rapid) {
        if (one) hipLaunchKernelGGL((k_tick<true, true>), g, dim3(kBlock), 0, S.stream, a);
        else hipLaunchKernelGGL((k_tick<true, false>), g, dim3(kBlock), 0, S.stream, a);
    } else {
        if (one) hipLaunchKernelGGL((k_tick<false, true>), g, dim3(kBlock), 0, S.stream, a);
        else hipLaunchKernelGGL((k_tick<false, false>), g, dim3(kBlock), 0, S.stream, a);
    }
    if (S.bracket_open) {
        S.bracket_reaches += p_hi - p_lo;
        ++P->prof_samples;
        if (P->prof_samples % kSampleGroup == 0) {
            HIPCHK(hipEventRecord(P->ev[2 * P->prof_brackets + 1], S.stream));
            ++P->prof_brackets;
            P->ev_reaches.push_back(S.bracket_reaches);
            S.bracket_reaches = 0;
            S.bracket_open = false;
        }
    }
    ++P->prof_launches;
    return RR_OK;
}

typedef void (*tile_kernel_t)(const TileArgs);

constexpr int kTileThreads = 512;
tile_kernel_t tile_kernel(bool unit, bool sub, bool lean = false, bool nolat = false)
{
    constexpr int T = kTileThreads;
    if (lean && nolat && !unit && !sub) return (tile_kernel_t)k_tile<T, false, false, true, true>;
    return unit ? (sub ? (tile_kernel_t)k_tile<T, true, true> : (lean ? (tile_kernel_t)k_tile<T, true, false, true> : (tile_kernel_t)k_tile<T, true, false>))
                : (sub ? (tile_kernel_t)k_tile<T, false, true> : (lean ? (tile_kernel_t)k_tile<T, false, false, true> : (tile_kernel_t)k_tile<T, false, false>));
}

tile_kernel_t tile_ens_kernel(bool sub)
{
    constexpr int T = kTileThreads;
    return sub ? (tile_kernel_t)k_tile<T, false, true, false, false, true> : (tile_kernel_t)k_tile<T, false, false, false, false, true>;
}

void launch_tile_diag_ens(rr_plan *P, const TileArgs &w, int64_t tiles)
{
    Session &S = P->ses;
    const int64_t slots = (int64_t)P->cu_count * (1024 / kTileThreads);
    const dim3 g((unsigned)std::min<int64_t>(tiles, std::max<int64_t>(1, (slots + S.members - 1) / S.members)), (unsigned)S.members);
    const size_t lds_bytes = tile_lds_bytes(kTileThreads);
    TileArgs e = w;
    e.tile_filter = 0; e.coef = P->d_coef;
    hipLaunchKernelGGL(tile_ens_kernel(S.nsub > 1), g, dim3((unsigned)kTileThreads), lds_bytes, S.stream, e);
}

int launch_tile_diag(rr_plan *P, const rr::TilePlan &TP, TileArgs &w, int32_t n_wide, const double *coef, const double *coef_unit, int64_t d, bool sampled)
{
    Session &S = P->ses;
    const int64_t l_lo = std::max<int64_t>(0, d - (S.n_macro - 1)), l_hi = std::min<int64_t>(TP.n_levels - 1, d);
    if (l_hi < l_lo) return RR_OK;
    int64_t t_lo = TP.level_start[l_lo], t_hi = TP.level_start[l_hi + 1];
    const int64_t K = (int64_t)w.KC * kRec;
    if (l_lo == 0) {
        const int64_t end0 = TP.level_start[1];
        int64_t hi = std::min<int64_t>(t_hi, end0);
        while (hi > t_lo && (d + 1) * K <= TP.tile_lag_lo[hi - 1]) --hi;
        if (t_hi <= end0) t_hi = hi;
    }
    if (t_hi <= t_lo) return RR_OK;
    w.diag = (int32_t)d; w.t_first = (int32_t)t_lo; w.t_last = (int32_t)t_hi - 1;
    const bool sample = sampled && S.max_samples > 0 && (P->prof_launches % 4) == 0 && (size_t)P->prof_brackets < S.max_samples;
    if (sample) HIPCHK(hipEventRecord(P->ev[2 * P->prof_brackets], S.stream));
    const dim3 g((unsigned)std::min<int64_t>(t_hi - t_lo, (int64_t)P->cu_count * (1024 / P->wave_threads)));
    const size_t lds_bytes = tile_lds_bytes(P->wave_threads);
    const bool unit = S.mode == Mode::Unit;
    const bool lean = S.nsub == 1 && P->lean_enabled;
    if (S.members > 0) {
        launch_tile_diag_ens(P, w, t_hi - t_lo);
    } else {
        w.tile_filter = lean ? 1 : 0;
        w.coef = (lean && unit) ? coef_unit : coef;
        hipLaunchKernelGGL(tile_kernel(unit, S.nsub > 1, lean, S.mode == Mode::Muskingum), g, dim3((unsigned)P->wave_threads), lds_bytes, S.stream, w);
        if (lean && n_wide > 0) {
            w.tile_filter = 2; w.coef = coef;
            hipLaunchKernelGGL(tile_kernel(unit, false, false), g, dim3((unsigned)P->wave_threads), lds_bytes, S.stream, w);
        }
    }
    if (sample) {
        HIPCHK(hipEventRecord(P->ev[2 * P->prof_brackets + 1], S.stream));
        int64_t moved = 0;
        for (int64_t c = t_lo; c < t_hi; ++c) {
            const int64_t m = d - TP.tile_level[c];
            if (m < 0 || m >= S.n_macro || m * K >= TP.tile_lag_hi[c] + S.total || (m + 1) * K <= TP.tile_lag_lo[c]) continue;
            moved += TP.tile_ptr[c + 1] - TP.tile_ptr[c];
        }
        P->ev_reaches.push_back(moved * K * std::max<int64_t>(1, S.members));
        P->prof_samples += K;
        ++P->prof_brackets;
    }
    return RR_OK;
}

bool tile_diag_launches(const rr_plan *P, const rr::TilePlan &TP, int64_t d)
{
    const Session &S = P->ses;
    const int64_t l_lo = std::max<int64_t>(0, d - (S.n_macro - 1)), l_hi = std::min<int64_t>(TP.n_levels - 1, d);
    return l_hi >= l_lo && TP.level_start[l_hi + 1] > TP.level_start[l_lo];
}

int session_launch_diag(rr_plan *P, int64_t d)
{
    int rc = launch_tile_diag(P, P->tp, P->ses.ta, P->n_wide_tiles, P->d_coef, P->d_coef_unit, d, true);
    ++P->prof_launches;
    return rc;
}

void launch_ghost_permute(rr_plan *P, int64_t batch)
{
    Session &S = P->ses;
    RecPermArgs ra{};
    ra.in32_sel = P->in32_big_endian ? kSelSwap : kSelNative; ra.out32_sel = P->out32_big_endian ? kSelSwap : kSelNative;
    ra.rec = P->d_ring; ra.rec_chunks = Div32((uint32_t)S.rec_chunks); ra.n = P->n_ghost; ra.np = S.kernel == Kernel::Direct ? P->dp.skel.np : P->tp.np; ra.T = S.total; ra.total = S.total;
    ra.batch = batch; ra.nsub = Div32(1u); ra.colmeta = S.kernel == Kernel::Direct ? P->d_kghostmeta : P->d_ghostmeta; ra.scale = nullptr;
    ra.rows = RowView{const_cast<double *>(S.ghost_series), P->n_ghost, 0, (uint32_t)S.total};
    ra.factor = Div32(1u);
    hipLaunchKernelGGL(k_rec_in<false>, dim3((unsigned)((P->n_ghost + kRecInCols - 1) / kRecInCols)), dim3(kRecInThreads), 0, rec_stream(P), ra);
}

typedef void (*rec_in_uh_t)(const RecPermArgs, const UhArgs);
constexpr int kUhFusedMaxTaps = 64;
int uh_padded_taps(int64_t n_ks) { return n_ks <= 16 ? 16 : (n_ks <= 48 ? 48 : 64); }
rec_in_uh_t rec_in_uh_kernel(bool sub, int64_t n_ks, int batches, bool in32 = false)
{
    const int nk = uh_padded_taps(n_ks);
#define RR_UHIN_IN(NK_, B_, S_) (in32 ? (rec_in_uh_t)k_rec_in_uh<S_, NK_, B_, true> : (rec_in_uh_t)k_rec_in_uh<S_, NK_, B_, false>)
#define RR_UHIN_SUB(NK_, B_) (sub ? RR_UHIN_IN(NK_, B_, true) : RR_UHIN_IN(NK_, B_, false))
#define RR_UHIN_PICK(NK_) (batches == 2 ? RR_UHIN_SUB(NK_, 2) : RR_UHIN_SUB(NK_, 1))
    return nk == 16 ? RR_UHIN_PICK(16) : (nk == 48 ? RR_UHIN_PICK(48) : RR_UHIN_PICK(64));
#undef RR_UHIN_PICK
#undef RR_UHIN_SUB
#undef RR_UHIN_IN
}

void launch_rec_out(const RecPermArgs &ra, bool sub, int64_t cols, hipStream_t st)
{
    const dim3 g((unsigned)((cols + kRecOutCols - 1) / kRecOutCols));
    if (ra.rows32) {
        if (sub) hipLaunchKernelGGL((k_rec_out<true, true>), g, dim3(kRecOutThreads), 0, st, ra);
        else hipLaunchKernelGGL((k_rec_out<false, true>), g, dim3(kRecOutThreads), 0, st, ra);
    } else {
        if (sub) hipLaunchKernelGGL((k_rec_out<true, false>), g, dim3(kRecOutThreads), 0, st, ra);
        else hipLaunchKernelGGL((k_rec_out<false, false>), g, dim3(kRecOutThreads), 0, st, ra);
    }
}

void launch_rec_permute(rr_plan *P, bool in, int64_t batch, int count = 1)
{
    Session &S = P->ses;
    const int64_t n = P->h.n;
    RecPermArgs ra{};
    ra.batches = count;
    ra.in32_sel = P->in32_big_endian ? kSelSwap : kSelNative; ra.out32_sel = P->out32_big_endian ? kSelSwap : kSelNative;
    ra.rec = P->d_ring; ra.rec_chunks = Div32((uint32_t)S.rec_chunks); ra.n = n; ra.np = P->tp.np; ra.T = S.T; ra.total = S.total; ra.batch = batch;
    ra.nsub = Div32((uint32_t)S.nsub);
    ra.colmeta = P->d_colmeta;
    ra.scale = (in && S.mode == Mode::Rapid) ? P->d_c4_params : nullptr;
    ra.rows = in ? RowView{const_cast<double *>(S.io.dev_in), n, 0, (uint32_t)S.io.rows_in}
                 : RowView{S.io.dev_out, n, 0, (uint32_t)std::max<int64_t>(1, S.io.rows_out)};
    ra.rows32 = in ? nullptr : S.io.dev_out32;
    ra.rows_in32 = in ? S.io.dev_in32 : nullptr;
    ra.factor = Div32((uint32_t)std::max<int64_t>(1, S.io.out_factor));
    ra.clamp = S.nsub > 1 ? 0 : (S.mode == Mode::Unit ? 2 : 1);
    ra.swizzle = in ? 0 : 1;
    const dim3 gp((unsigned)((n + kRecInCols - 1) / kRecInCols));
    const bool sub = S.nsub > 1;
    hipStream_t st = rec_stream(P);
    const int aux = aux_begin(P, in ? 0 : 1, st);
    if (S.members > 0) {
        const RecEnsArgs e{ra, S.ring_stride, in ? S.io.in_pitch : S.io.out_pitch};
        const dim3 ge((unsigned)((n + kRecInCols - 1) / kRecInCols), (unsigned)S.members);
        if (in && ra.rows_in32) {
            if (sub) hipLaunchKernelGGL((k_rec_in<true, true, true>), ge, dim3(kRecInThreads), 0, st, e);
            else hipLaunchKernelGGL((k_rec_in<false, true, true>), ge, dim3(kRecInThreads), 0, st, e);
        } else if (in) {
            if (sub) hipLaunchKernelGGL((k_rec_in<true, false, true>), ge, dim3(kRecInThreads), 0, st, e);
            else hipLaunchKernelGGL((k_rec_in<false, false, true>), ge, dim3(kRecInThreads), 0, st, e);
        } else {
            const dim3 go((unsigned)((n + kRecOutCols - 1) / kRecOutCols), (unsigned)S.members);
            if (ra.rows32) {
                if (sub) hipLaunchKernelGGL((k_rec_out<true, true, true>), go, dim3(kRecOutThreads), 0, st, e);
                else hipLaunchKernelGGL((k_rec_out<false, true, true>), go, dim3(kRecOutThreads), 0, st, e);
            } else {
                if (sub) hipLaunchKernelGGL((k_rec_out<true, false, true>), go, dim3(kRecOutThreads), 0, st, e);
                else hipLaunchKernelGGL((k_rec_out<false, false, true>), go, dim3(kRecOutThreads), 0, st, e);
            }
        }
    } else if (in && S.io.runoff) {
        const dim3 gr((unsigned)((n + kRunoffInThreads - 1) / kRunoffInThreads), (unsigned)kRecBatch);
        if (S.io.runoff->is_f32) hipLaunchKernelGGL(k_rec_in_runoff<float>, gr, dim3(kRunoffInThreads), 0, st, ra, *S.io.runoff);
        else hipLaunchKernelGGL(k_rec_in_runoff<double>, gr, dim3(kRunoffInThreads), 0, st, ra, *S.io.runoff);
    } else if (in && S.io.uh_kernel) {
        UhArgs ua{S.io.uh_kernel, S.io.uh_state, (int32_t)S.io.uh_nks};
        hipLaunchKernelGGL(rec_in_uh_kernel(sub, S.io.uh_nks, count, ra.rows_in32 != nullptr), dim3((unsigned)((n + kUhCols - 1) / kUhCols)), dim3(uh_threads(count)),
                           rec_in_uh_lds_bytes(uh_padded_taps(S.io.uh_nks), count), st, ra, ua);
    } else if (in && ra.rows_in32) {
        if (sub) hipLaunchKernelGGL((k_rec_in<true, true>), gp, dim3(kRecInThreads), 0, st, ra);
        else hipLaunchKernelGGL((k_rec_in<false, true>), gp, dim3(kRecInThreads), 0, st, ra);
    } else if (in) {
        if (sub) hipLaunchKernelGGL(k_rec_in<true>, gp, dim3(kRecInThreads), 0, st, ra);
        else hipLaunchKernelGGL(k_rec_in<false>, gp, dim3(kRecInThreads), 0, st, ra);
    } else {
        launch_rec_out(ra, sub, n, st);
    }
    aux_end(P, aux, st);
}

int session_advance_tile(rr_plan *P, int64_t rows_ready, int64_t ghost_ready, int64_t *export_ready)
{
    Session &S = P->ses;
    const int64_t dmax = P->h.depth - 1, levels = P->tp.n_levels, K = S.KC * kRec;
    const int64_t ticks_ready = std::min(rows_ready, S.T) * S.nsub;
    for (;;) {
        bool progressed = false;
        auto slot_free = [&](int64_t j) {
            const int64_t must_have_left = kRecRows * (j + 1) + kRec - kRec * S.rec_chunks;
            return must_have_left <= 0 || S.ticks_stored >= std::min(S.total, must_have_left);
        };
        if (S.has_in && S.in_batches < S.n_in_batches && ticks_ready >= std::min(kRecRows * (S.in_batches + 1), S.total) && slot_free(S.in_batches)) {
            const int max_count = S.io.runoff ? 1 : (S.io.uh_kernel ? (P->uh_pairs ? 2 : 1) : (int)S.rec_nb);
            int count = 1;
            while (count < max_count && S.in_batches + count < S.n_in_batches &&
                   ticks_ready >= std::min(kRecRows * (S.in_batches + count + 1), S.total) && slot_free(S.in_batches + count)) ++count;
            launch_rec_permute(P, true, S.in_batches, count);
            S.in_batches += count;
            progressed = true;
        }
        if (P->n_ghost > 0 && S.ghost_batches < S.n_in_batches && (!S.has_in || S.ghost_batches < S.in_batches) &&
            ghost_ready >= std::min(kRecRows * (S.ghost_batches + 1), S.total) && slot_free(S.ghost_batches)) {
            launch_ghost_permute(P, S.ghost_batches);
            ++S.ghost_batches;
            progressed = true;
        }
        auto loaded_ticks = [&](int64_t batches) { return batches >= S.n_in_batches ? S.total : std::max<int64_t>(0, kRecRows * batches - 15); };
        const int64_t have = S.has_in ? loaded_ticks(S.in_batches) : S.total;
        const int64_t have_ghost = P->n_ghost > 0 ? loaded_ticks(S.ghost_batches) : S.total;
        S.rows_loaded = have / S.nsub;
        int64_t launched = 0;
        const int64_t batch = std::max<int64_t>(1, kRecRows / K);
        while (S.diag < S.n_diags && launched < batch) {
            const int64_t need_ticks = std::min((S.diag + 1) * K, S.total);
            if (have < need_ticks) break;
            if (have_ghost < std::min(std::max<int64_t>(0, (S.diag + 1) * K - S.ghost_slack), S.total)) break;
            const int64_t top = std::min(std::min(S.diag + 1, S.n_macro) * S.KC - 1, (S.total_ticks - 1) / kRec);
            if (top >= S.rec_chunks && S.ticks_stored < std::min(S.total, kRec * (top - S.rec_chunks + 1))) break;
            int rc = session_launch_diag(P, S.diag);
            if (rc) return rc;
            ++S.diag; ++launched;
            progressed = true;
        }
        const int64_t m_done = S.diag - levels;
        int64_t done = 0;
        if (S.diag >= S.n_diags) done = S.total;
        else if (m_done >= 0) done = std::max<int64_t>(0, (m_done + 1) * K - dmax);
        done = std::min(done, S.total);
        auto out_ready = [&](int64_t j) {
            const int64_t end = std::min(kRecRows * (j + 1), S.total);
            return done >= end && (end + S.nsub - 1) / S.nsub <= S.out_limit;
        };
        while (S.out_batches < S.n_out_batches) {
            int count = 0;
            while (count < S.rec_nb && S.out_batches + count < S.n_out_batches && out_ready(S.out_batches + count)) ++count;
            if (count == 0 || (count < S.rec_nb && S.out_batches + count < S.n_out_batches && progressed)) break;
            launch_rec_permute(P, false, S.out_batches, count);
            S.out_batches += count;
            S.ticks_stored = std::min(S.total, kRecRows * S.out_batches);
            progressed = true;
        }
        if (!progressed) break;
    }
    S.rows_stored = S.ticks_stored / S.nsub;
    if (S.diag >= S.n_diags) S.tau = S.total_ticks;
    if (export_ready) {
        const int64_t e = S.diag >= S.n_diags ? S.total : S.diag * K - S.export_skew;
        *export_ready = std::max<int64_t>(0, std::min(e, S.total));
    }
    return RR_OK;
}

int session_advance_direct(rr_plan *P, int64_t rows_ready, int64_t ghost_ready, int64_t *export_ready)
{
    Session &S = P->ses;
    const rr::TilePlan &TP = P->dp.skel;
    const int64_t dmax = P->h.depth - 1, levels = TP.n_levels, K = S.KC * kRec, Kt = K * S.nsub, KS = S.KS * kRec, per = Kt / KS, n = P->h.n;
    rows_ready = std::min(rows_ready, S.T);
    const bool skel = TP.n_tiles > 0, ghosts = skel && P->n_ghost > 0;
    auto slot_free = [&](int64_t j) {
        const int64_t must_have_left = kRecRows * (j + 1) + kRec - kRec * S.rec_chunks;
        return must_have_left <= 0 || S.ticks_stored >= std::min(S.total, must_have_left);
    };
    for (;;) {
        bool progressed = false;
        while (S.d_done < S.n_tasks) {
            const int64_t d = S.d_done;
            if (rows_ready < std::min((d + 1) * K, S.T)) break;
            if (skel) {
                const int64_t top = std::min((d + 1) * Kt + dmax, S.total_ticks) / kRec;
                if (top >= S.rec_chunks && S.ticks_stored < std::min(S.total, kRec * (top - S.rec_chunks + 1))) break;
            }
            const bool sample = S.max_samples > 0 && (size_t)P->prof_brackets < S.max_samples;
            if (sample) HIPCHK(hipEventRecord(P->ev[2 * P->prof_brackets], S.stream));
            S.da.m = (int32_t)d;
            const dim3 g((unsigned)std::min<int64_t>(P->dp.n_tiles, (int64_t)P->cu_count));
            hipLaunchKernelGGL(direct_kernel(S.io.dev_in32 != nullptr && S.has_in, S.da.out32 != nullptr, S.nsub > 1, S.mode == Mode::Unit ? 1 : 0), g, dim3(kDirectThreads), direct_lds_bytes(P->direct_window), S.stream, S.da);
            if (sample) {
                HIPCHK(hipEventRecord(P->ev[2 * P->prof_brackets + 1], S.stream));
                P->ev_reaches.push_back(n * (std::min((d + 1) * K, S.T) - d * K));
                P->prof_samples += K;
                ++P->prof_brackets;
            }
            ++P->prof_launches;
            ++S.d_done;
            progressed = true;
        }
        const int64_t rows_routed = S.d_done >= S.n_tasks ? S.T : S.d_done * K;
        const int64_t ticks_routed = rows_routed * S.nsub;
        S.rows_loaded = rows_routed;
        while (ghosts && S.ghost_batches < S.n_in_batches) {
            const int64_t need = std::min(kRecRows * (S.ghost_batches + 1), S.total);
            if (ghost_ready < need || need > ticks_routed || !slot_free(S.ghost_batches)) break;
            launch_ghost_permute(P, S.ghost_batches);
            ++S.ghost_batches;
            progressed = true;
        }
        const int64_t ghost_loaded = !ghosts || S.ghost_batches >= S.n_in_batches ? S.total : std::max<int64_t>(0, kRecRows * S.ghost_batches - 15);
        while (skel && S.diag < S.n_diags) {
            const int64_t j = S.diag;
            if (S.d_done < S.n_tasks && j > S.d_done * per - 1) break;
            if (ghost_loaded < std::min(S.total, j * KS)) break;
            if (tile_diag_launches(P, TP, j)) {
                const int aux = aux_begin(P, 2, S.stream);
                int rc = launch_tile_diag(P, TP, S.ta, P->n_kwide, P->d_kcoef, P->d_kcoef, j, false);
                aux_end(P, aux, S.stream);
                if (rc) return rc;
            }
            ++S.diag;
            progressed = true;
        }
        int64_t done = ticks_routed;
        if (skel) {
            const int64_t m_done = S.diag - levels;
            int64_t sk = S.diag >= S.n_diags ? S.total : (m_done >= 0 ? std::max<int64_t>(0, (m_done + 1) * KS - dmax) : 0);
            done = std::min(done, std::min(sk, S.total));
            while (S.out_batches < S.n_out_batches && done >= std::min(kRecRows * (S.out_batches + 1), S.total)) {
                RecPermArgs ra{};
                ra.in32_sel = P->in32_big_endian ? kSelSwap : kSelNative; ra.out32_sel = P->out32_big_endian ? kSelSwap : kSelNative;
                ra.rec = P->d_ring; ra.rec_chunks = Div32((uint32_t)S.rec_chunks); ra.n = P->n_kholes; ra.np = TP.np; ra.T = S.T; ra.total = S.total;
                ra.batch = S.out_batches; ra.nsub = Div32((uint32_t)S.nsub); ra.colmeta = P->d_kholemeta; ra.cols = P->d_kholecol; ra.scale = nullptr;
                ra.rows = RowView{S.io.dev_out, n, 0, (uint32_t)std::max<int64_t>(1, S.io.rows_out)};
                ra.rows32 = S.io.dev_out32;
                ra.factor = Div32((uint32_t)std::max<int64_t>(1, S.io.out_factor)); ra.clamp = S.nsub > 1 ? 0 : 1; ra.swizzle = 0;
                const int aux = aux_begin(P, 3, S.stream);
                if (P->n_kholes > 0) launch_rec_out(ra, S.nsub > 1, P->n_kholes, S.stream);
                aux_end(P, aux, S.stream);
                ++S.out_batches;
                S.ticks_stored = std::min(S.total, kRecRows * S.out_batches);
                progressed = true;
            }
            S.rows_stored = S.ticks_stored / S.nsub;
        } else {
            S.ticks_stored = done; S.rows_stored = done / S.nsub;
        }
        if (!progressed) break;
    }
    if (S.d_done >= S.n_tasks && S.diag >= S.n_diags) S.tau = S.total_ticks;
    if (export_ready) {
        int64_t e = S.d_done >= S.n_tasks ? S.total : S.d_done * Kt;
        if (S.export_skel) e = std::min(e, S.diag >= S.n_diags ? S.total : S.diag * KS - S.export_skew);
        *export_ready = P->n_export > 0 ? std::max<int64_t>(0, std::min(e, S.total)) : S.total;
    }
    return RR_OK;
}

int session_advance(rr_plan *P, int64_t rows_ready, int64_t ghost_ready, int64_t *export_ready)
{
    Session &S = P->ses;
    if (!S.open) return fail(RR_E_STATE, "no routing call is open on this plan");
    const int64_t n = P->h.n, dmax = P->h.depth - 1, C = std::max<int64_t>(1, P->chunk_rows);
    if (export_ready) *export_ready = 0;
    if (n == 0 || S.total == 0) { if (export_ready) *export_ready = S.total; return RR_OK; }
    if (S.kernel == Kernel::Tile) return session_advance_tile(P, rows_ready, std::min(ghost_ready, S.total), export_ready);
    if (S.kernel == Kernel::Direct) return session_advance_direct(P, rows_ready, std::min(ghost_ready, S.total), export_ready);
    rows_ready = std::min(rows_ready, S.T);
    ghost_ready = std::min(ghost_ready, S.total);
    const int64_t ghost_limit = (P->n_ghost == 0 || ghost_ready >= S.total) ? S.total_ticks
                                                                            : ghost_ready + P->ghost_min_lag;
    for (;;) {
        bool progressed = false;
        if (S.has_in && S.rows_loaded < rows_ready) {
            const int64_t r1 = std::min(rows_ready, S.rows_loaded + C);
            int rc = session_load_rows(P, S.rows_loaded, r1);
            if (rc) return rc;
            S.rows_loaded = r1;
            progressed = true;
        }
        const int64_t have_rows = S.has_in ? S.rows_loaded : rows_ready;
        const int64_t lat_limit = have_rows < S.T ? have_rows * S.nsub : S.total_ticks;
        const int64_t batch_limit = S.has_in ? S.total_ticks : S.tau + C * S.nsub;
        const int64_t tau_end = std::min(std::min(lat_limit, ghost_limit), std::min(batch_limit, S.total_ticks));
        for (; S.tau < tau_end; ++S.tau) {
            int rc = session_launch_tick(P, S.tau);
            if (rc) return rc;
            progressed = true;
        }
        int64_t done = S.tau >= S.total_ticks ? S.T : (S.tau - dmax < 0 ? 0 : (S.tau - dmax) / S.nsub);
        done = std::min(done, S.T);
        if (done > S.rows_stored) {
            int rc = session_store_rows(P, S.rows_stored, done);
            if (rc) return rc;
            S.rows_stored = done;
            progressed = true;
        }
        if (!progressed) break;
    }
    if (export_ready) {
        const int64_t e = S.tau >= S.total_ticks ? S.total : S.tau - P->export_max_lag;
        *export_ready = std::max<int64_t>(0, std::min(e, S.total));
    }
    return RR_OK;
}

int session_end(rr_plan *P)
{
    Session &S = P->ses;
    if (!S.open) return fail(RR_E_STATE, "no routing call is open on this plan");
    const bool complete = P->h.n == 0 || S.total == 0 || (S.tau >= S.total_ticks && S.rows_stored >= S.T);
    S.open = false;
    if (!complete && getenv("RR_VERBOSE"))
        fprintf(stderr, "rr: incomplete call: T=%lld total=%lld tau=%lld/%lld rows_loaded=%lld rows_stored=%lld | direct=%d tasks %lld/%lld diag %lld/%lld in_batches %lld ghost_batches %lld/%lld out_batches %lld/%lld "
                        "ticks_stored=%lld K=%lld KS=%lld chunks=%lld macro=%lld\n", (long long)S.T, (long long)S.total, (long long)S.tau, (long long)S.total_ticks, (long long)S.rows_loaded, (long long)S.rows_stored,
                (int)(S.kernel == Kernel::Direct), (long long)S.d_done, (long long)S.n_tasks, (long long)S.diag, (long long)S.n_diags, (long long)S.in_batches, (long long)S.ghost_batches, (long long)S.n_in_batches,
                (long long)S.out_batches, (long long)S.n_out_batches, (long long)S.ticks_stored, (long long)(S.KC * kRec), (long long)(S.KS * kRec), (long long)S.rec_chunks, (long long)S.n_macro);
    if (!complete) return fail(RR_E_STATE, "routing call closed before all of its time steps were routed");
    if (P->h.n == 0 || S.total == 0) return RR_OK;
    if (S.bracket_open) P->prof_samples -= P->prof_samples % kSampleGroup;
    HIPCHK(hipEventRecord(P->ev_last, S.stream));
    HIPCHK(hipGetLastError());
    return RR_OK;
}

int route_core(rr_plan *P, Mode mode, int64_t T, int64_t nsub, const Rows &io, hipStream_t stream)
{
    if (P->n_ghost > 0 || P->n_export > 0)
        return fail(RR_E_STATE, "plan has boundary reaches: use rr_stream_begin / rr_stream_advance / rr_stream_end");
    int rc = session_begin(P, mode, T, nsub, io, stream, nullptr, nullptr);
    if (rc) return rc;
    rc = session_advance(P, T, T * nsub, nullptr);
    if (rc) { P->ses.open = false; return rc; }
    return session_end(P);
}

int check_route_args(rr_plan *P, bool need_c4, int64_t T, int64_t nsub)
{
    int rc = need_device(P);
    if (rc) return rc;
    if (!P->coeffs_set) return fail(RR_E_STATE, "route called before rr_plan_set_coeffs");
    if (need_c4 && !P->has_c4) return fail(RR_E_STATE, "rr_rapid_route needs c4_dt (rr_plan_set_coeffs got NULL)");
    if (T < 0 || nsub < 1) return fail(RR_E_INVALID, "route: need num steps >= 0 and sub-steps >= 1");
    if (nsub > 0x7FFFFFFF) return fail(RR_E_INVALID, "route: too many sub-steps");
    return RR_OK;
}

int launch_state_in(rr_plan *P, const double *d_q, hipStream_t stream)
{
    const int64_t n = P->h.n;
    if (P->sch.kernel != Kernel::Tick) {
        const bool d = P->sch.kernel == Kernel::Direct;
        const int64_t np = d ? P->dp.skel.np : P->tp.np;
        if (d) HIPCHK(hipMemcpyAsync(P->d_dq, d_q, (size_t)n * sizeof(double), hipMemcpyDeviceToDevice, stream));
        if (np > 0)
            hipLaunchKernelGGL(k_tile_state_in, grid1(np), dim3(kBlock), 0, stream, d ? P->d_ksq : P->d_sq, d ? P->d_kss : P->d_ss, d ? P->d_ksi : P->d_si, d_q,
                               d ? P->d_kperm : P->d_tperm, d ? P->d_kpmeta : P->d_pmeta, (int32_t)np);
        return RR_OK;
    }
    hipLaunchKernelGGL(k_state_in, grid1(n), dim3(kBlock), 0, stream, P->d_x, P->d_x + n, P->d_x + 2 * n, d_q,
                       P->d_perm, (int32_t)n);
    return RR_OK;
}

void launch_state_out(rr_plan *P, double *d_q, int64_t total, hipStream_t stream)
{
    const int64_t n = P->h.n;
    if (P->sch.kernel == Kernel::Direct) {
        (void)hipMemcpyAsync(d_q, P->d_dq, (size_t)n * sizeof(double), hipMemcpyDeviceToDevice, stream);
        const int64_t np = P->dp.skel.np;
        if (np > 0) hipLaunchKernelGGL(k_skel_state_out, grid1(np), dim3(kBlock), 0, stream, d_q, (const double *)P->d_ksq, P->d_kperm, P->d_kpmeta, (int32_t)np);
        return;
    }
    if (P->sch.kernel == Kernel::Tile) {
        hipLaunchKernelGGL(k_tile_state_out, grid1(n), dim3(kBlock), 0, stream, d_q, (const double *)P->d_sq, P->d_tinv,
                           (int32_t)n);
        return;
    }
    hipLaunchKernelGGL(k_state_out, grid1(n), dim3(kBlock), 0, stream, d_q, (const double *)P->d_x, n,
                       P->d_lag, P->d_inv, (int32_t)n, total);
}

void parallel_copy(double *dst, const double *src, size_t count, int threads, std::vector<std::thread> &pool)
{
    const size_t per = ((count + threads - 1) / threads + 511) / 512 * 512;
    for (int t = 0; t < threads; ++t) {
        const size_t o = (size_t)t * per;
        if (o >= count) break;
        pool.emplace_back([=] { std::memcpy(dst + o, src + o, std::min(per, count - o) * sizeof(double)); });
    }
}

int host_pipe_prepare(rr_plan *P)
{
    HostPipe &H = P->pipe;
    const int64_t n = P->h.n;
    H.chunk_rows = std::max<int64_t>(16, std::min<int64_t>(4096, ((H.chunk_mib << 20) / (n * 8) + 15) / 16 * 16));
    if (n * 8 * 64 <= (int64_t{1} << 30)) H.chunk_rows = std::max<int64_t>(H.chunk_rows, 64);
    H.ring_chunks = std::max<int64_t>(8, (2 * kRecRows + 15) / H.chunk_rows + 6);
    const int64_t pin_need = H.chunk_rows * n, dev_need = H.ring_chunks * H.chunk_rows * n;
    if (H.pin_cap < pin_need || H.dev_cap < dev_need) {
        H.destroy();
        for (int k = 0; k < HostPipe::kPinned; ++k) {
            if (hipHostMalloc((void **)&H.pin_in[k], (size_t)pin_need * 8, hipHostMallocDefault) != hipSuccess ||
                hipHostMalloc((void **)&H.pin_out[k], (size_t)pin_need * 8, hipHostMallocDefault) != hipSuccess) {
                (void)hipGetLastError(); H.destroy();
                return fail(RR_E_ALLOC, "host pipeline: pinned staging buffers could not be allocated");
            }
        }
        if (hipMalloc((void **)&H.dev_in, (size_t)dev_need * 8) != hipSuccess || hipMalloc((void **)&H.dev_out, (size_t)dev_need * 8) != hipSuccess) {
            (void)hipGetLastError(); H.destroy();
            return fail(RR_E_ALLOC, "host pipeline: device staging rings could not be allocated");
        }
        H.pin_cap = pin_need; H.dev_cap = dev_need;
    }
    if (!H.s_h2d) { HIPCHK(hipStreamCreateWithFlags(&H.s_h2d, hipStreamNonBlocking)); HIPCHK(hipStreamCreateWithFlags(&H.s_d2h, hipStreamNonBlocking)); }
    return RR_OK;
}

int route_host_pipelined(rr_plan *P, Mode mode, int64_t T, int64_t nsub, const double *host_in, double *host_out, hipStream_t stream)
{
    int rc = host_pipe_prepare(P);
    if (rc) return rc;
    HostPipe &H = P->pipe;
    constexpr int kPinned = HostPipe::kPinned;
    const int64_t n = P->h.n, C = H.chunk_rows, NR = H.ring_chunks, nchunks = (T + C - 1) / C;
    auto grow = [&](std::vector<hipEvent_t> &v, size_t count) {
        while (v.size() < count) { hipEvent_t e; if (hipEventCreateWithFlags(&e, hipEventDisableTiming) != hipSuccess) return false; v.push_back(e); }
        return true;
    };
    if (!grow(H.ev_h2d, (size_t)nchunks) || !grow(H.ev_d2h, (size_t)nchunks) || !grow(H.ev_adv, (size_t)4 * nchunks + 64))
        return fail(RR_E_HIP, "host pipeline: event creation failed");
    Rows io;
    io.dev_in = host_in ? H.dev_in : nullptr; io.rows_in = NR * C; io.dev_out = H.dev_out; io.rows_out = NR * C;
    rc = session_begin(P, mode, T, nsub, io, stream, nullptr, nullptr);
    if (rc) return rc;
    Session &S = P->ses;
    auto rows_of = [&](int64_t c) { return std::min(C, T - c * C); };
    std::vector<int64_t> adv_loaded;
    int64_t filled = 0, h2d_issued = 0, d2h_issued = 0, copied_out = 0;
    std::vector<std::thread> pool;
    auto bail = [&](int code, const std::string &msg) {
        for (auto &t : pool) t.join();
        (void)hipStreamSynchronize(H.s_h2d); (void)hipStreamSynchronize(H.s_d2h); (void)hipStreamSynchronize(stream);
        P->ses.open = false;
        return fail(code, msg);
    };
#define RR_PIPE(expr) do { hipError_t e__ = (expr); if (e__ != hipSuccess) return bail(RR_E_HIP, std::string(#expr) + ": " + hipGetErrorString(e__)); } while (0)
    double t_join = 0.0, t_wait = 0.0;
    auto now = [] { return std::chrono::duration<double>(std::chrono::steady_clock::now().time_since_epoch()).count(); };
    while (copied_out < nchunks) {
        pool.clear();
        bool progressed = false;
        const bool fill = host_in && filled < nchunks && filled < h2d_issued + kPinned;
        if (fill) {
            if (filled >= kPinned) { const double t0 = now(); RR_PIPE(hipEventSynchronize(H.ev_h2d[filled - kPinned])); t_wait += now() - t0; }
            parallel_copy(H.pin_in[filled % kPinned], host_in + filled * C * n, (size_t)(rows_of(filled) * n), H.copy_threads, pool);
        }
        bool empty = false;
        if (copied_out < d2h_issued) {
            const hipError_t q = hipEventQuery(H.ev_d2h[copied_out]);
            if (q == hipSuccess) empty = true;
            else if (q != hipErrorNotReady) return bail(RR_E_HIP, std::string("hipEventQuery: ") + hipGetErrorString(q));
        }
        if (empty) {
            parallel_copy(host_out + copied_out * C * n, H.pin_out[copied_out % kPinned], (size_t)(rows_of(copied_out) * n), H.copy_threads, pool);
        }
        if (host_in && h2d_issued < filled) {
            const int64_t c = h2d_issued;
            bool slot_ready = true;
            if (c >= NR) {
                const int64_t need = std::min(T, (c - NR + 1) * C);
                size_t a = 0;
                while (a < adv_loaded.size() && adv_loaded[a] < need) ++a;
                if (a < adv_loaded.size()) RR_PIPE(hipStreamWaitEvent(H.s_h2d, H.ev_adv[a], 0));
                else slot_ready = false;
            }
            if (slot_ready) {
                RR_PIPE(hipMemcpyAsync(H.dev_in + (c % NR) * C * n, H.pin_in[c % kPinned], (size_t)(rows_of(c) * n) * 8, hipMemcpyHostToDevice, H.s_h2d));
                RR_PIPE(hipEventRecord(H.ev_h2d[c], H.s_h2d));
                RR_PIPE(hipStreamWaitEvent(stream, H.ev_h2d[c], 0));
                ++h2d_issued;
                progressed = true;
            }
        }
        if (S.tau < S.total_ticks || S.rows_stored < T) {
            const int64_t ready = host_in ? std::min(T, h2d_issued * C) : T;
            S.out_limit = std::min(T, d2h_issued * C) + NR * C;
            if (d2h_issued > 0) RR_PIPE(hipStreamWaitEvent(stream, H.ev_d2h[d2h_issued - 1], 0));
            const int64_t before_diag = S.diag, before_in = S.in_batches, before_out = S.out_batches;
            rc = session_advance(P, ready, S.total, nullptr);
            if (rc) { for (auto &t : pool) t.join(); P->ses.open = false; return rc; }
            if (S.diag != before_diag || S.in_batches != before_in || S.out_batches != before_out) {
                progressed = true;
                if (adv_loaded.size() < H.ev_adv.size() - 1) {
                    RR_PIPE(hipEventRecord(H.ev_adv[adv_loaded.size()], stream));
                    adv_loaded.push_back(S.rows_loaded);
                }
            }
        }
        while (d2h_issued < nchunks && std::min(T, (d2h_issued + 1) * C) <= S.rows_stored && d2h_issued < copied_out + kPinned) {
            const int64_t k = d2h_issued;
            RR_PIPE(hipEventRecord(H.ev_adv.back(), stream));
            RR_PIPE(hipStreamWaitEvent(H.s_d2h, H.ev_adv.back(), 0));
            RR_PIPE(hipMemcpyAsync(H.pin_out[k % kPinned], H.dev_out + (k % NR) * C * n, (size_t)(rows_of(k) * n) * 8, hipMemcpyDeviceToHost, H.s_d2h));
            RR_PIPE(hipEventRecord(H.ev_d2h[k], H.s_d2h));
            ++d2h_issued;
// ... 198 lines not shown
```

### river_route_amd/csrc/rr_kernels_rec.hpp

```cpp
#pragma once

namespace {

constexpr int kRecCols = 32, kRecBatch = 8, kRecThreads = 256;
constexpr int kRecInThreads = kRecThreads, kRecOutThreads = kRecThreads;
constexpr int kRecInCols = kRecCols, kRecOutCols = kRecCols;
constexpr int kRecRows = 16 * kRecBatch;
constexpr int kRecLaunchBatches = 4, kRecMaxLaunchBatches = 8;

struct RecPermArgs {
    double *rec;
    Div32 rec_chunks;
    int64_t n, np, T, total, batch;
    Div32 nsub;
    const int2 *colmeta;
    const double *scale;
    RowView rows;
    const float *rows_in32;
    float *rows32;
    Div32 factor;
    const int32_t *cols;
    int32_t swizzle;
    int32_t clamp;
    uint32_t in32_sel, out32_sel;
    int32_t batches;
};

struct RecEnsArgs : RecPermArgs {
    int64_t ring_stride, row_pitch;
};
template <bool ENS> using RecArgsOf = typename std::conditional<ENS, RecEnsArgs, RecPermArgs>::type;
__device__ __forceinline__ const RecPermArgs &member_args(const RecPermArgs &a) { return a; }
__device__ __forceinline__ RecPermArgs member_args(const RecEnsArgs &e)
{
    RecPermArgs a = e;
    const int64_t m = blockIdx.y;
    a.rec += m * e.ring_stride;
    a.rows.base += m * e.row_pitch;
    if (a.rows_in32) a.rows_in32 += m * e.row_pitch;
    if (a.rows32) a.rows32 += m * e.row_pitch;
    return a;
}

constexpr int32_t kColHeadwater = 1 << 30;

constexpr int kRecTileRows = 16 * kRecBatch + 15;
constexpr int kRecTileLd = kRecCols + 1;

__device__ __forceinline__ uint32_t ring_chunk(const Div32 &chunks, uint32_t first, uint32_t ahead)
{
    const uint32_t c = first + ahead;
    return c >= chunks.d ? c - chunks.d : c;
}

template <bool SUB, int THREADS = kRecThreads, int BATCH = kRecBatch, bool LDSMETA = false, int COLS = kRecCols>
__device__ __forceinline__ void write_records(const RecPermArgs &a, const double *tile, int64_t col0, int64_t batch, int64_t tick_first, int64_t row_first,
                                              const int2 *smeta = nullptr, const double *sscale = nullptr)
{
    constexpr int R = 16 * BATCH + 15;
    const int tid = threadIdx.x;
    static_assert(COLS * BATCH * 8 % THREADS == 0, "records of a tile must divide among the threads");
    constexpr int IT = COLS * BATCH * 8 / THREADS;
    int2 meta[LDSMETA ? 1 : IT];
    double f[LDSMETA ? 1 : IT];
    if constexpr (!LDSMETA) {
#pragma unroll
        for (int it = 0; it < IT; ++it) {
            const int64_t i = col0 + (it * THREADS + tid) / (8 * BATCH);
            meta[it] = i < a.n ? a.colmeta[i] : make_int2(-1, 0);
        }
#pragma unroll
        for (int it = 0; it < IT; ++it) {
            const int64_t i = col0 + (it * THREADS + tid) / (8 * BATCH);
            f[it] = (a.scale && i < a.n) ? a.scale[i] : 1.0;
        }
    }
    const uint32_t chunk_first = a.rec_chunks.mod((uint32_t)kRecBatch * (uint32_t)batch);
#pragma unroll(LDSMETA ? (SUB ? 2 : 4) : IT)
    for (int it = 0; it < IT; ++it) {
        const int piece = it * THREADS + tid;
        const int c = piece / (8 * BATCH), k = (piece >> 3) % BATCH, part = piece & 7;
        const int2 m = LDSMETA ? smeta[c] : meta[LDSMETA ? 0 : it];
        const double scale = LDSMETA ? sscale[c] : f[LDSMETA ? 0 : it];
        const int32_t p = m.x;
        if (p < 0) continue;
        const int32_t lag = m.y & kLagMask;
        const int o = lag & 15;
        const uint32_t chunk = ring_chunk(a.rec_chunks, chunk_first, (uint32_t)(lag >> 4) + k);
        const int r = 15 - o + 16 * k + 2 * part;
        double v0, v1;
        if (SUB) {
            const int64_t t0 = tick_first + r, t1 = t0 + 1;
            uint32_t s;
            const int r0 = t0 < 0 ? 0 : (int)((int64_t)a.nsub.div((uint32_t)t0, s) - row_first);
            const int r1 = t1 < 0 ? 0 : (int)((int64_t)a.nsub.div((uint32_t)t1, s) - row_first);
            v0 = tile[min(r0, R - 1) * (COLS + 1) + c] * scale; v1 = tile[min(r1, R - 1) * (COLS + 1) + c] * scale;
        } else {
            v0 = tile[r * (COLS + 1) + c] * scale; v1 = tile[(r + 1) * (COLS + 1) + c] * scale;
        }
        double2 *dst = reinterpret_cast<double2 *>(a.rec + rec_elem(chunk, a.np, p)) + part;
        typedef double d2 __attribute__((ext_vector_type(2)));
        *reinterpret_cast<d2 *>(dst) = d2{v0, v1};
    }
}

template <bool SUB, bool IN32 = false, bool ENS = false>
__global__ __launch_bounds__(kRecInThreads, 4) void k_rec_in(const RecArgsOf<ENS> args)
{
    const RecPermArgs &a = member_args(args);
    constexpr int R = kRecTileRows, G = kRecInThreads / kRecInCols;
    __shared__ double tile[R * (kRecInCols + 1)];
    __shared__ int2 smeta[kRecInCols];
    __shared__ double sscale[kRecInCols];
    const int tid = threadIdx.x;
    auto first_row = [&](int64_t tick_first) -> int64_t {
        uint32_t sub_unused;
        return SUB ? (int64_t)a.nsub.div((uint32_t)(tick_first < 0 ? 0 : tick_first), sub_unused) : tick_first;
    };
    int64_t tick_first = kRecRows * a.batch - 15;
    int64_t row_first = first_row(tick_first);
    constexpr int RPT = (R + G - 1) / G;
    const int c = tid % kRecInCols, r0 = tid / kRecInCols;
    const int need = SUB ? (int)((uint32_t)(R - 1) / a.nsub.d) + 2 : R;
    const uint32_t n_tiles = (uint32_t)((a.n + kRecInCols - 1) / kRecInCols);
    if (blockIdx.x >= n_tiles) return;
    const int64_t col0 = (int64_t)(a.swizzle ? xcd_swizzle(blockIdx.x, n_tiles) : blockIdx.x) * kRecInCols;
    const int64_t i = min(col0 + c, a.n - 1);
    const bool live = col0 + c < a.n;
    auto load = [&](int64_t t) -> double {
        const int64_t off = a.rows.offset(t < 0 ? 0 : (t >= a.T ? a.T - 1 : t)) + i;
        return IN32 ? (double)f32_from_file(a.rows_in32[off], a.in32_sel) : a.rows.base[off];
    };
    {
        double v[RPT];
        int2 cm = make_int2(-1, 0);
        double cs = 1.0;
        if (tid < kRecInCols) {
            cm = live ? a.colmeta[i] : make_int2(-1, 0);
            cs = a.scale ? a.scale[i] : 1.0;
        }
#pragma unroll
        for (int q = 0; q < RPT; ++q) v[q] = load(row_first + min(r0 + q * G, need - 1));
#pragma unroll
        for (int q = 0; q < RPT; ++q) {
            const int r = r0 + q * G;
            const int64_t row = row_first + r;
            if (r < R) tile[r * (kRecInCols + 1) + c] = (row >= 0 && row < a.T && live) ? v[q] : 0.0;
        }
        if (tid < kRecInCols) { smeta[c] = cm; sscale[c] = cs; }
    }
    __syncthreads();
    const int nb = a.batches > 1 ? a.batches : 1;
    for (int b = 1; b < nb; ++b) {
        constexpr int NPT = kRecRows / G, KPT = 3;
        const int64_t tick_next = tick_first + kRecRows, row_next = first_row(tick_next);
        const int shift = (int)(row_next - row_first), keep = max(need - shift, 0);
        double v[NPT], kv[KPT];
#pragma unroll
        for (int q = 0; q < NPT; ++q) {
            const int r = keep + r0 + q * G;
            if (r < need) v[q] = load(row_next + r);
        }
        write_records<SUB, kRecInThreads, kRecBatch, true, kRecInCols>(a, tile, col0, a.batch + b - 1, tick_first, row_first, smeta, sscale);
#pragma unroll
        for (int q = 0; q < KPT; ++q) {
            const int r = r0 + q * G;
            if (r < keep) kv[q] = tile[(shift + r) * (kRecInCols + 1) + c];
        }
        __syncthreads();
#pragma unroll
        for (int q = 0; q < KPT; ++q) {
            const int r = r0 + q * G;
            if (r < keep) tile[r * (kRecInCols + 1) + c] = kv[q];
        }
#pragma unroll
        for (int q = 0; q < NPT; ++q) {
            const int r = keep + r0 + q * G;
            const int64_t row = row_next + r;
            if (r < need) tile[r * (kRecInCols + 1) + c] = (row >= 0 && row < a.T && live) ? v[q] : 0.0;
        }
        __syncthreads();
        tick_first = tick_next; row_first = row_next;
    }
    write_records<SUB, kRecInThreads, kRecBatch, true, kRecInCols>(a, tile, col0, a.batch + nb - 1, tick_first, row_first, smeta, sscale);
}

struct UhArgs {
    const double *kernel, *state;
    int32_t n_ks;
};
constexpr int kUhCols = 16, kUhTileLd = kUhCols + 1;
constexpr int kUhMaxBatches = 2;
constexpr int uh_threads(int batches) { return 32 * kRecBatch * batches; }
constexpr int uh_tile_rows(int batches) { return 16 * kRecBatch * batches + 15; }
constexpr int uh_groups(int batches) { return uh_threads(batches) / kUhCols; }
constexpr int uh_rows_per_thread(int batches) { return (uh_tile_rows(batches) + uh_groups(batches) - 1) / uh_groups(batches); }
constexpr int uh_win_rows(int batches) { return uh_groups(batches) * uh_rows_per_thread(batches); }
constexpr size_t rec_in_uh_lds_bytes(int nk, int batches) { return (size_t)((uh_win_rows(batches) + nk - 1) + nk) * kUhTileLd * sizeof(double); }

template <bool SUB, int NK, int BATCHES, bool IN32 = false>
__global__ __launch_bounds__(uh_threads(BATCHES)) void k_rec_in_uh(const RecPermArgs a, const UhArgs u)
{
    constexpr int R = uh_tile_rows(BATCHES), G = uh_groups(BATCHES), RP = uh_rows_per_thread(BATCHES);
    constexpr int ROWS = uh_win_rows(BATCHES) + NK - 1, DATA = R + NK - 1;
    extern __shared__ __attribute__((aligned(16))) double uh_lds[];
    double *dt = uh_lds;
    double *tp = uh_lds + ROWS * kUhTileLd;
    const int tid = threadIdx.x, c = tid % kUhCols, g = tid / kUhCols;
    const int64_t col0 = (int64_t)(a.swizzle ? xcd_swizzle(blockIdx.x, gridDim.x) : blockIdx.x) * kUhCols;
    const int64_t tick_first = kRecRows * a.batch - 15;
    uint32_t sub_unused;
    const int64_t row_first = SUB ? (int64_t)a.nsub.div((uint32_t)(tick_first < 0 ? 0 : tick_first), sub_unused) : tick_first;
    const int need = SUB ? (int)((uint32_t)(R - 1) / a.nsub.d) + 2 : R;
    const int64_t i = min(col0 + c, a.n - 1);
    const bool live = col0 + c < a.n;
    const int32_t tb = (int32_t)row_first - (NK - 1) + g;
    {
        constexpr int DPT = (ROWS + G - 1) / G, TPT = (NK + G - 1) / G;
        double dv[DPT], tv[TPT];
        if constexpr (SUB) {
#pragma unroll
            for (int q = 0; q < DPT; ++q) {
                const int64_t t = row_first - (NK - 1) + min(g + q * G, need + NK - 2);
                const int64_t off = a.rows.offset(t < 0 ? 0 : (t >= a.T ? a.T - 1 : t)) + i;
                dv[q] = IN32 ? (double)f32_from_file(a.rows_in32[off], a.in32_sel) : a.rows.base[off];
            }
        } else {
            constexpr int QM = (NK - 1 + 15 + G - 1) / G;
            static_assert(QM < DPT, "the tile is longer than the rows before it");
            const uint32_t d = a.rows.rows.d, step = a.rows.rows.mod((uint32_t)G);
            uint32_t m[DPT];
            m[QM] = a.rows.rows.mod((uint32_t)(tb + G * QM - (int32_t)a.rows.t0));
#pragma unroll
            for (int q = QM + 1; q < DPT; ++q) { const uint32_t x = m[q - 1] + step; m[q] = x >= d ? x - d : x; }
#pragma unroll
            for (int q = QM - 1; q >= 0; --q) m[q] = m[q + 1] >= step ? m[q + 1] - step : m[q + 1] + d - step;
#pragma unroll
            for (int q = 0; q < DPT; ++q) {
                const int64_t off = (int64_t)m[q] * a.rows.ld + i;
                dv[q] = IN32 ? (double)f32_from_file(a.rows_in32[off], a.in32_sel) : a.rows.base[off];
            }
        }
#pragma unroll
        for (int q = 0; q < TPT; ++q) tv[q] = u.kernel[(int64_t)min(g + q * G, u.n_ks - 1) * a.n + i];
#pragma unroll
        for (int q = 0; q < DPT; ++q) {
            const int r = g + q * G;
            const bool inside = (uint32_t)(tb + q * G) < (uint32_t)a.T;
            if (r < ROWS) dt[r * kUhTileLd + c] = (live && inside && r < DATA) ? dv[q] : 0.0;
        }
#pragma unroll
        for (int q = 0; q < TPT; ++q) {
            const int k = g + q * G;
            if (k < NK) tp[k * kUhTileLd + c] = (live && k < u.n_ks) ? tv[q] : 0.0;
        }
    }
    __syncthreads();
    const int rb = g * RP;
    const bool mine = !SUB || rb < need;
    double acc[RP];
    if (mine) {
        const double *wp = dt + rb * kUhTileLd + c;
        if (row_first < (int64_t)u.n_ks) {
#pragma unroll
            for (int j = 0; j < RP; ++j) {
                const int64_t t = row_first + rb + j;
                acc[j] = (live && t >= 0 && t < u.n_ks && t < a.T) ? u.state[t * a.n + i] : 0.0;
            }
        } else {
#pragma unroll
            for (int j = 0; j < RP; ++j) acc[j] = 0.0;
        }
        const double *kp = tp + c;
        constexpr int KH = NK / 2;
        static_assert(NK % 2 == 0, "taps are padded to an even count");
#pragma unroll
        for (int h = 0; h < 2; ++h) {
            double tap[KH];
#pragma unroll
            for (int k = 0; k < KH; ++k) tap[k] = kp[(h * KH + k) * kUhTileLd];
#pragma unroll
            for (int w = RP - 1 + NK - 1 - h * KH; w >= NK - 1 - h * KH - (KH - 1); --w) {
                const double x = wp[w * kUhTileLd];
#pragma unroll
                for (int j = 0; j < RP; ++j) {
                    const int k = j + NK - 1 - w - h * KH;
                    if (k >= 0 && k < KH) acc[j] = __builtin_fma(tap[k], x, acc[j]);
                }
            }
        }
    }
    __syncthreads();
    if (mine) {
        double *op = dt + rb * kUhTileLd + c;
#pragma unroll
        for (int j = 0; j < RP; ++j) op[j * kUhTileLd] = acc[j];
    }
    __syncthreads();
    write_records<SUB, uh_threads(BATCHES), kRecBatch * BATCHES, false, kUhCols>(a, dt, col0, a.batch, tick_first, row_first);
}

template <bool SUB, bool OUT32, bool ENS = false>
__global__ __launch_bounds__(kRecOutThreads) void k_rec_out(const RecArgsOf<ENS> args)
{
    const RecPermArgs &a = member_args(args);
    constexpr int S = 16 * (kRecBatch + 1);
    __shared__ double recs[kRecOutCols][S + 1];
    __shared__ int2 smeta[kRecOutCols];
    const int tid = threadIdx.x;
    static_assert(kRecOutCols * (kRecBatch + 1) * 8 % kRecOutThreads == 0, "record pieces of a tile must divide among the threads");
    static_assert(kRecOutCols * 8 == kRecOutThreads, "one 16-byte piece of the records kept between batches per thread");
    constexpr int IT = kRecOutCols * (kRecBatch + 1) * 8 / kRecOutThreads, ITN = kRecOutCols * kRecBatch * 8 / kRecOutThreads;
    const uint32_t n_tiles = (uint32_t)((a.n + kRecOutCols - 1) / kRecOutCols);
    if (blockIdx.x >= n_tiles) return;
    const int64_t col0 = (int64_t)(a.swizzle ? xcd_swizzle(blockIdx.x, n_tiles) : blockIdx.x) * kRecOutCols;
    typedef double d2 __attribute__((ext_vector_type(2)));
    {
        d2 v[IT];
        const uint32_t chunk_first = a.rec_chunks.mod((uint32_t)kRecBatch * (uint32_t)a.batch);
        {
            int2 meta[IT];
#pragma unroll
            for (int it = 0; it < IT; ++it) {
                const int64_t i = col0 + (it * kRecOutThreads + tid) / ((kRecBatch + 1) * 8);
                meta[it] = i < a.n ? a.colmeta[i] : make_int2(0, 0);
            }
#pragma unroll
            for (int it = 0; it < IT; ++it) {
                const int piece = it * kRecOutThreads + tid;
                const int k = (piece >> 3) % (kRecBatch + 1), part = piece & 7;
                const uint32_t chunk = ring_chunk(a.rec_chunks, chunk_first, (uint32_t)((meta[it].y & kLagMask) >> 4) + k);
                v[it] = reinterpret_cast<const d2 *>(a.rec + rec_elem(chunk, a.np, meta[it].x))[part];
            }
        }
#pragma unroll
        for (int it = 0; it < IT; ++it) {
            const int piece = it * kRecOutThreads + tid;
// ... 86 lines not shown
```

### river_route_amd/csrc/rr_plan.cpp

```cpp
#include "rr_plan.hpp"

#include <algorithm>
#include <cstdlib>
#include <limits>
#include <utility>
#include <vector>

#include "../../include/rr_hip.h"

namespace rr {

void build_tiled_permutation(const int32_t *pi, int64_t n, int32_t tile, TiledPermutation &T)
{
    T = TiledPermutation();
    T.n = n;
    T.tile = tile;
    if (n == 0) return;
    const int64_t nt = (n + tile - 1) / tile;
    std::vector<int32_t> q_of(n);
    for (int64_t q = 0; q < n; ++q) q_of[pi[q]] = (int32_t)q;
    std::vector<int64_t> run(nt * nt + 1, 0);
    for (int64_t i = 0; i < n; ++i) ++run[(int64_t)(q_of[i] / tile) * nt + i / tile + 1];
    for (size_t k = 1; k < run.size(); ++k) run[k] += run[k - 1];
    std::vector<int32_t> g_of(n);
// ... 182 lines not shown
    std::vector<int32_t> tile_of_reach(n, -1);
    std::vector<int32_t> roots;
    if (!skeleton_only) for (int64_t v = 0; v < n; ++v) if (small_root(v)) roots.push_back((int32_t)v);
    std::stable_sort(roots.begin(), roots.end(), [&](int32_t a, int32_t b) { return lag_of[a] < lag_of[b]; });
    int32_t n_tiles = 0;
    {
        constexpr size_t kWindow = 768;
        std::vector<uint8_t> used(roots.size(), 0);
        size_t head = 0;
        while (head < roots.size()) {
            if (used[head]) { ++head; continue; }
            int64_t room = block;
            for (size_t i = head; i < roots.size() && room > 0; ++i) {
                if (used[i]) continue;
                if (sub[roots[i]] > room) break;
                used[i] = 1; tile_of_reach[roots[i]] = n_tiles; room -= sub[roots[i]];
            }
            while (room > 0) {
                int64_t best = -1, best_size = 0;
                size_t seen = 0;
                for (size_t i = head; i < roots.size() && seen < kWindow; ++i) {
                    if (used[i]) continue;
                    ++seen;
                    if (sub[roots[i]] <= room && sub[roots[i]] > best_size) { best = (int64_t)i; best_size = sub[roots[i]]; }
                }
                if (best < 0) break;
                used[best] = 1; tile_of_reach[roots[best]] = n_tiles; room -= best_size;
            }
            ++n_tiles;
        }
    }
    const int32_t n_level0 = n_tiles;
    std::vector<int32_t> tile_level((size_t)n_tiles, 0);

    std::vector<int32_t> bigs;
    for (int64_t v = 0; v < n; ++v) if (big(v)) bigs.push_back((int32_t)v);
    std::vector<int64_t> res(n, 0);
    std::vector<uint8_t> cut(n, 0);
    std::vector<std::pair<int64_t, int32_t>> kids;
    for (int32_t v : bigs) {
        int64_t total = 1;
        kids.clear();
        for (int32_t e = up_ptr[v]; e < up_ptr[v + 1]; ++e) {
            const int32_t c = up_idx[e];
            if (big(c)) { kids.emplace_back(res[c], c); total += res[c]; } else ++total;
        }
        if (total > block) {
            std::sort(kids.begin(), kids.end(), [](const auto &a, const auto &b) { return a.first != b.first ? a.first > b.first : a.second < b.second; });
            for (const auto &k : kids) {
                if (total <= block) break;
                cut[k.second] = 1;
                total -= k.first - 1;
            }
        }
        if (total > block || up_ptr[v + 1] - up_ptr[v] > 65535) return;
        res[v] = total;
    }
    std::vector<int32_t> piece_root(n, -1), piece_level(n, 0);
    std::vector<int32_t> pieces;
    for (auto it = bigs.rbegin(); it != bigs.rend(); ++it) {
        const int32_t v = *it;
        if (down[v] < 0 || cut[v]) { piece_root[v] = v; pieces.push_back(v); piece_level[v] = 1; }
        else piece_root[v] = piece_root[down[v]];
    }
    for (int32_t v : bigs)
        if (cut[v]) { const int32_t r = piece_root[down[v]]; piece_level[r] = std::max(piece_level[r], piece_level[v] + 1); }
    std::sort(pieces.begin(), pieces.end(), [&](int32_t a, int32_t b) {
        if (piece_level[a] != piece_level[b]) return piece_level[a] < piece_level[b];
        return lag_of[a] != lag_of[b] ? lag_of[a] < lag_of[b] : a < b; });
    {
        std::vector<int64_t> room;
        int32_t cur = -1, first_tile = n_tiles;
        std::vector<int32_t> tile_of_piece(n, -1);
        for (int32_t r : pieces) {
            if (piece_level[r] != cur) { cur = piece_level[r]; first_tile = n_tiles; room.clear(); }
            size_t b = 0;
            for (; b < room.size(); ++b) if (room[b] >= res[r]) break;
            if (b == room.size()) { room.push_back(block); tile_level.push_back(cur); ++n_tiles; }
            room[b] -= res[r];
            tile_of_piece[r] = first_tile + (int32_t)b;
        }
        for (int32_t v : bigs) tile_of_reach[v] = tile_of_piece[piece_root[v]];
    }
    if (!skeleton_only)
        for (int64_t v = n - 1; v >= 0; --v)
            if (!big(v) && !small_root(v)) tile_of_reach[v] = tile_of_reach[down[v]];
    (void)n_level0;

    T.n_tiles = n_tiles;
    T.tile_level = tile_level;
    T.n_levels = tile_level.empty() ? 0 : tile_level.back() + 1;
    T.level_start.assign((size_t)T.n_levels + 1, 0);
    for (int32_t t = 0; t < n_tiles; ++t) ++T.level_start[tile_level[t] + 1];
    for (int32_t l = 0; l < T.n_levels; ++l) T.level_start[l + 1] += T.level_start[l];
    std::vector<int32_t> root_ptr((size_t)n_tiles + 1, 0);
    auto tile_root = [&](int64_t v) { return down[v] < 0 || tile_of_reach[down[v]] != tile_of_reach[v]; };
    for (int64_t v = 0; v < n; ++v) if (tile_of_reach[v] >= 0 && tile_root(v)) ++root_ptr[tile_of_reach[v] + 1];
    for (int32_t t = 0; t < n_tiles; ++t) root_ptr[t + 1] += root_ptr[t];
    std::vector<int32_t> root_list(root_ptr[n_tiles]), rfill(root_ptr.begin(), root_ptr.end() - 1);
    for (int64_t v = n - 1; v >= 0; --v) if (tile_of_reach[v] >= 0 && tile_root(v)) root_list[rfill[tile_of_reach[v]]++] = (int32_t)v;

    T.inv.assign(n, -1);
    T.tile_ptr.assign((size_t)n_tiles + 1, 0);
    T.tile_lag_lo.assign(n_tiles, 0); T.tile_lag_hi.assign(n_tiles, 0);
    std::vector<int32_t> ghost_positions;
    for (int32_t t = 0; t < n_tiles; ++t) {
        const int64_t base = (int64_t)T.perm.size();
        T.tile_ptr[t] = (int32_t)base;
        for (int32_t k = root_ptr[t]; k < root_ptr[t + 1]; ++k) {
            T.perm.push_back(root_list[k]); T.lag.push_back(lag_of[root_list[k]]);
        }
        for (int64_t head = base; head < (int64_t)T.perm.size(); ++head) {
            const int32_t v = T.perm[head];
            if (T.lag[head] & kTileGhost) { T.cfirst.push_back((int32_t)head); T.ccnt.push_back(0u); continue; }
            T.inv[v] = (int32_t)head;
            uint32_t cnt = 0, hw = 0;
            T.cfirst.push_back((int32_t)T.perm.size());
            for (int pass = 0; pass < 2; ++pass)
                for (int32_t e = up_ptr[v]; e < up_ptr[v + 1]; ++e) {
                    const int32_t c = up_idx[e];
                    if (is_hw(c) != (pass == 0)) continue;
                    const bool ghost = tile_of_reach[c] != t;
                    T.perm.push_back(c);
                    T.lag.push_back(lag_of[c] | (ghost ? kTileGhost : 0));
                    if (ghost) ghost_positions.push_back((int32_t)T.perm.size() - 1);
                    ++cnt; if (pass == 0) ++hw;
                }
            T.ccnt.push_back(cnt | (hw << 16));
        }
        int32_t lo = std::numeric_limits<int32_t>::max(), hi = 0;
        for (int64_t p = base; p < (int64_t)T.perm.size(); ++p) { const int32_t l = T.lag[p] & (kTileExport - 1); lo = std::min(lo, l); hi = std::max(hi, l); }
        T.tile_lag_lo[t] = lo; T.tile_lag_hi[t] = hi;
        if ((int64_t)T.perm.size() - base > block) return;
    }
    T.np = (int64_t)T.perm.size();
    T.tile_ptr[n_tiles] = (int32_t)T.np;
    T.tile_flags.assign(n_tiles, 0);
    for (int32_t t = 0; t < n_tiles; ++t)
        for (int32_t p = T.tile_ptr[t]; p < T.tile_ptr[t + 1]; ++p)
            if ((T.ccnt[p] & 0xFFFFu) > 3) { T.tile_flags[t] = 1; break; }
    T.n_ghost = (int64_t)ghost_positions.size();
    T.xpos.assign(T.np, -1);
    T.tile_of.assign(T.np, 0);
    for (int32_t t = 0; t < n_tiles; ++t) for (int32_t p = T.tile_ptr[t]; p < T.tile_ptr[t + 1]; ++p) T.tile_of[p] = t;
    if (skeleton_only) T.ext_ghost.assign(n, -1);
    for (int32_t g : ghost_positions) {
        const int32_t src = T.inv[T.perm[g]];
        if (src < 0) { T.ext_ghost[T.perm[g]] = g; continue; }
        T.xpos[g] = src; T.xpos[src] = g; T.lag[src] |= kTileExport;
    }
    T.ok = true;
}

void build_direct_plan(const std::vector<int32_t> &down, const std::vector<int32_t> &lag_of, int32_t lanes, int32_t wmax, int32_t skel_block,
                       DirectPlan &D, const std::vector<uint8_t> *ghost, const std::vector<int32_t> *export_slot)
{
    D = DirectPlan();
    D.lanes = lanes; D.wmax = wmax;
    const int64_t n = (int64_t)down.size();
    if (n == 0) { D.why = "empty network"; return; }
    if (lanes > 1023) { D.why = "more lanes than a lane number holds"; return; }
    std::vector<int32_t> sub(n, 1), height(n, 1), first(n), indeg(n, 0);
    for (int64_t v = 0; v < n; ++v) first[v] = (int32_t)v;
    for (int64_t c = 0; c < n; ++c)
        if (down[c] >= 0) {
            const int32_t d = down[c];
            sub[d] += sub[c]; height[d] = std::max(height[d], height[c] + 1); first[d] = std::min(first[d], first[c]); ++indeg[d];
        }
    D.big.assign(n, 0);
    for (int64_t v = 0; v < n; ++v) D.big[v] = (sub[v] > lanes || height[v] > wmax) ? 1 : 0;
    auto small_root = [&](int64_t v) { return !D.big[v] && (down[v] < 0 || D.big[down[v]]); };
    auto is_ghost = [&](int64_t v) { return ghost && (*ghost)[v] != 0; };
    if (ghost)
        for (int64_t v = 0; v < n; ++v)
            if (is_ghost(v)) for (int64_t w = down[v]; w >= 0 && !D.big[w]; w = down[w]) D.big[w] = 1;
    for (int64_t v = 0; v < n; ++v) {
        if (is_ghost(v) && (indeg[v] != 0 || down[v] < 0)) { D.why = "a boundary ghost is not a headwater with a downstream reach"; return; }
        if (export_slot && (*export_slot)[v] >= 0 && down[v] >= 0) { D.why = "a boundary export has a downstream reach in this plan"; return; }
        if (D.big[v]) continue;
        if (indeg[v] > 3) { D.why = "a reach of a small subtree has more than three upstream reaches"; return; }
        if (small_root(v) && first[v] != (int32_t)v - sub[v] + 1) { D.why = "a small subtree is not a contiguous range of the params order"; return; }
    }
    D.delay.assign(n, 0); D.up3.assign(n, 0x3FFFFFFF); D.xinfo.assign(n, -1);
    std::vector<int32_t> tile_of(n, -1);
    int64_t c = 0;
    while (c < n) {
        const int64_t c0 = c;
        int32_t lo = std::numeric_limits<int32_t>::max(), hi = -1, senders = 0;
        while (c < n) {
            int64_t c1;
            int32_t ulo = lo, uhi = hi, us = senders;
            if (D.big[c]) { c1 = c + 1; ++us; }
            else {
                int64_t r = c;
                while (!small_root(r)) r = down[r];
                if (first[r] != c) { D.why = "internal: a small subtree does not start where the previous unit ended"; return; }
                c1 = r + 1;
                if (down[r] >= 0 && !is_ghost(r)) ++us;
                if (!is_ghost(r)) for (int64_t v = c; v < c1; ++v) { ulo = std::min(ulo, lag_of[v]); uhi = std::max(uhi, lag_of[v]); }
            }
            if (c1 - c0 > lanes || (uhi >= 0 && uhi - ulo + 1 > wmax) || us > kDirectSenders) break;
            lo = ulo; hi = uhi; senders = us; c = c1;
        }
        if (c == c0) { D.why = "internal: a unit does not fit an empty tile"; return; }
        const int32_t t = D.n_tiles++;
        D.tile_c0.push_back((int32_t)c0); D.tile_nc.push_back((int32_t)(c - c0));
        D.tile_lag_lo.push_back(hi < 0 ? 0 : lo); D.tile_span.push_back(hi < 0 ? 0 : hi - lo);
        for (int64_t v = c0; v < c; ++v) {
            tile_of[v] = t;
            if (D.big[v]) { D.delay[v] = kDirectHole; ++D.n_holes; }
            else if (is_ghost(v)) D.delay[v] = kDirectHole;
            else D.delay[v] = lag_of[v] - lo;
        }
    }
    std::vector<int32_t> filled(n, 0);
    for (int pass = 0; pass < 2; ++pass)
        for (int64_t u = 0; u < n; ++u) {
            const int32_t d = down[u];
            if (d < 0 || D.big[d] || (indeg[u] == 0) != (pass == 0)) continue;
            const int32_t lane = (int32_t)(u - D.tile_c0[tile_of[d]]);
            const int k = filled[d]++;
            D.up3[d] = (D.up3[d] & ~(0x3FF << (10 * k))) | (lane << (10 * k));
            if (pass == 0) D.up3[d] = (int32_t)((uint32_t)D.up3[d] + (1u << 30));
        }
    if (D.n_holes * 10 > n) { D.why = "more than a tenth of the reaches have subtrees too large or too tall for a direct tile"; return; }
    build_tile_plan(down, lag_of, skel_block, D.skel, &D.big, true);
    if (!D.skel.ok) { D.why = "the skeleton does not tile"; return; }
    for (int64_t v = 0; v < n; ++v) {
        if (D.big[v]) D.xinfo[v] = D.skel.inv[v];
        else if (small_root(v) && down[v] >= 0) {
            if (D.skel.ext_ghost[v] < 0) { D.why = "internal: an outlet below the skeleton has no ghost"; return; }
            if (is_ghost(v)) continue;
            D.xinfo[v] = D.skel.ext_ghost[v]; ++D.n_exports;
        }
    }
    if (export_slot)
        for (int64_t v = 0; v < n; ++v)
            if ((*export_slot)[v] >= 0 && !D.big[v]) { D.delay[v] |= kDirectExport; D.xinfo[v] = (*export_slot)[v]; }
    D.send_ptr.assign((size_t)D.n_tiles + 1, 0);
    for (int32_t t = 0; t < D.n_tiles; ++t) {
        for (int32_t v = D.tile_c0[t]; v < D.tile_c0[t] + D.tile_nc[t]; ++v)
            if (D.xinfo[v] >= 0 && !(D.delay[v] & kDirectExport)) {
                D.delay[v] |= ((int32_t)(D.send_lane.size() - D.send_ptr[t]) + 1) << kDirectSenderShift;
                D.send_lane.push_back((v - D.tile_c0[t]) | (D.big[v] ? kDirectHole : 0));
            }
        D.send_ptr[t + 1] = (int32_t)D.send_lane.size();
        if (D.send_ptr[t + 1] - D.send_ptr[t] > kDirectSenders) { D.why = "internal: a tile has more senders than one wave forwards"; return; }
    }
    D.ok = true;
}

constexpr int64_t kPostorderSmall = 256;

bool postorder(const int64_t *down, int64_t n, int64_t *order)
{
    if (n == 0) return true;
    std::vector<int64_t> up_ptr(n + 1, 0), pending(n, 0), sub(n, 1);
    for (int64_t i = 0; i < n; ++i) {
        if (down[i] >= n || down[i] == i) return false;
        if (down[i] >= 0) ++up_ptr[down[i] + 1];
    }
    for (int64_t i = 0; i < n; ++i) { pending[i] = up_ptr[i + 1]; up_ptr[i + 1] += up_ptr[i]; }
    std::vector<int64_t> up_idx(up_ptr[n]), fill(up_ptr.begin(), up_ptr.end() - 1), queue;
    for (int64_t i = 0; i < n; ++i) if (down[i] >= 0) up_idx[fill[down[i]]++] = i;
    queue.reserve(n);
    for (int64_t i = 0; i < n; ++i) if (pending[i] == 0) queue.push_back(i);
    for (size_t h = 0; h < queue.size(); ++h) {
        const int64_t v = queue[h], d = down[v];
        if (d >= 0) { sub[d] += sub[v]; if (--pending[d] == 0) queue.push_back(d); }
    }
    if ((int64_t)queue.size() != n) return false;
    for (int64_t v = 0; v < n; ++v)
        std::sort(up_idx.begin() + up_ptr[v], up_idx.begin() + up_ptr[v + 1], [&](int64_t a, int64_t b) {
            const bool la = sub[a] > kPostorderSmall, lb = sub[b] > kPostorderSmall;
            if (la != lb) return lb;
            if (sub[a] != sub[b]) return la ? sub[a] < sub[b] : sub[a] > sub[b];
            return a < b; });
    int64_t k = 0;
    std::vector<std::pair<int64_t, int64_t>> stack;
    for (int64_t root = 0; root < n; ++root) {
        if (down[root] >= 0) continue;
        stack.emplace_back(root, up_ptr[root]);
        while (!stack.empty()) {
            auto &top = stack.back();
            if (top.second < up_ptr[top.first + 1]) { const int64_t c = up_idx[top.second++]; stack.emplace_back(c, up_ptr[c]); }
            else { order[k++] = top.first; stack.pop_back(); }
        }
    }
    return k == n;
}

int build_host_plan(int64_t n, const int32_t *indptr, const int32_t *indices, HostPlan &P, std::string &err)
{
    if (n < 0 || (n > 0 && (!indptr))) { err = "rr_plan_create: null csc_indptr or negative n"; return RR_E_INVALID; }
    if (n > (int64_t)std::numeric_limits<int32_t>::max() - 1) { err = "rr_plan_create: n exceeds int32 range"; return RR_E_INVALID; }
    P = HostPlan();
    P.n = n;
    if (n == 0) { P.child_ptr.assign(1, 0); P.lag_start.assign(1, 0); P.identity = true; return RR_OK; }
    if (indptr[0] != 0) { err = "rr_plan_create: csc_indptr[0] must be 0"; return RR_E_INVALID; }

    std::vector<int32_t> down(n, -1);
    P.edge_of.assign(n, -1);
    for (int64_t c = 0; c < n; ++c) {
        const int64_t a = indptr[c], b = indptr[c + 1];
        if (b < a) { err = "rr_plan_create: csc_indptr is not non-decreasing"; return RR_E_INVALID; }
        if (b - a > 1) {
// ... 107 lines not shown
```

### river_route_amd/csrc/rr_plan.hpp

```cpp
#pragma once
#include <cstdint>
#include <string>
#include <vector>

namespace rr {

struct HostPlan {
    int64_t n = 0;
    int64_t n_edges = 0;
    int32_t depth = 0;
    int64_t widest_level = 0;
    int64_t n_headwaters = 0;
    int64_t n_outlets = 0;
    bool identity = false;

    std::vector<int32_t> perm;
    std::vector<int32_t> inv;
    std::vector<int32_t> lag;
    std::vector<int32_t> child_ptr;
    std::vector<uint16_t> hw_children;
    std::vector<int64_t> lag_start;
    std::vector<int32_t> edge_of;
    std::vector<int32_t> inner_pos;
    std::vector<int32_t> down;
};

struct TiledPermutation {
    int64_t n = 0;
    int32_t tile = 0;
    std::vector<uint16_t> slot_a;
    std::vector<int32_t> m_index;
    std::vector<uint16_t> slot_b;
};
void build_tiled_permutation(const int32_t *pi, int64_t n, int32_t tile, TiledPermutation &out);

void partition_forest(const std::vector<int32_t> &down, int32_t n_parts, int32_t *part_of, std::vector<int64_t> &sizes);


constexpr int32_t kTileGhost = 1 << 28;
constexpr int32_t kTileExport = 1 << 27;
struct TilePlan {
    bool ok = false;
    int32_t block = 0;
    int64_t np = 0;
    int64_t n_ghost = 0;
    int32_t n_tiles = 0, n_levels = 0;
    std::vector<int32_t> tile_ptr;
    std::vector<int32_t> tile_level;
    std::vector<int32_t> tile_lag_lo, tile_lag_hi;
    std::vector<int32_t> tile_flags;
    std::vector<int32_t> level_start;
    std::vector<int32_t> perm;
    std::vector<int32_t> inv;
    std::vector<int32_t> lag;
    std::vector<int32_t> cfirst;
    std::vector<uint32_t> ccnt;
    std::vector<int32_t> xpos;
    std::vector<int32_t> tile_of;
    std::vector<int32_t> ext_ghost;
};
void build_tile_plan(const std::vector<int32_t> &down, const std::vector<int32_t> &lag_of, int32_t block, TilePlan &out,
                     const std::vector<uint8_t> *big = nullptr, bool skeleton_only = false);

constexpr int32_t kDirectHole = 1 << 30;
constexpr int32_t kDirectSenderShift = 8, kDirectDelayMask = 0xFF;
constexpr int32_t kDirectExport = 1 << 15;
struct DirectPlan {
    bool ok = false;
    std::string why;
    int32_t lanes = 0, wmax = 0;
    int32_t n_tiles = 0;
    int64_t n_holes = 0, n_exports = 0;
    std::vector<int32_t> tile_c0, tile_nc, tile_lag_lo, tile_span;
    std::vector<int32_t> delay;
    std::vector<int32_t> up3;
    std::vector<int32_t> xinfo;
    std::vector<uint8_t> big;
    std::vector<int32_t> send_ptr;
    std::vector<int32_t> send_lane;
    TilePlan skel;
};
constexpr int32_t kDirectSenders = 64;
void build_direct_plan(const std::vector<int32_t> &down, const std::vector<int32_t> &lag_of, int32_t lanes, int32_t wmax, int32_t skel_block,
                       DirectPlan &out, const std::vector<uint8_t> *ghost = nullptr, const std::vector<int32_t> *export_slot = nullptr);

bool postorder(const int64_t *down, int64_t n, int64_t *order);

int build_host_plan(int64_t n, const int32_t *indptr, const int32_t *indices, HostPlan &plan, std::string &err);

}
```

### river_route_amd/engine.py

```python
from __future__ import annotations

import ctypes as C

import numpy as np

from . import _lib
from ._lib import RRError, check, ptr

__all__ = ['Plan', 'RRError', 'uh_convolve', 'uh_convolve_dev', 'uh_adjoint_work_bytes', 'uh_adjoint_dev', 'runoff_to_qlateral', 'DeviceBuffer', 'partition_forest', 'synchronize',
           'resample_cast_dev', 'copy_bandwidth', 'runoff_to_qlateral_dev', 'rows_upload', 'rows_download', 'metrics_work_bytes',
           'metrics_update_dev', 'metrics_finish_dev', 'metrics_adjoint_work_bytes', 'metrics_adjoint_dev', 'grid_overlap_area',
           'grid_overlap_area_dev']


MODE_RAPID, MODE_MUSKINGUM, MODE_UNIT = 0, 1, 2
REC_BATCH_ROWS = 128


def _f64(a, name):
    a = np.ascontiguousarray(a, dtype=np.float64)
    if not a.flags['WRITEABLE']:
        a = a.copy()
    return a


def _inplace_f64(a, name, shape):
    if not (isinstance(a, np.ndarray) and a.dtype == np.float64 and a.flags['C_CONTIGUOUS'] and a.flags['WRITEABLE']):
        raise TypeError(f'{name} must be a writeable C-contiguous float64 numpy array (it is updated in place)')
    if a.shape != shape:
        raise ValueError(f'{name} has shape {a.shape}, expected {shape}')
    return a


class Plan:

    def __init__(self, csc_indptr, csc_indices, device: int = 0):
        indptr = np.ascontiguousarray(csc_indptr, dtype=np.int32)
        indices = np.ascontiguousarray(csc_indices, dtype=np.int32)
        if indptr.ndim != 1 or indptr.shape[0] < 1:
            raise ValueError('csc_indptr must be a 1-D array of length n + 1')
        self.n = int(indptr.shape[0] - 1)
        if indices.shape[0] != int(indptr[-1]):
            raise ValueError('csc_indices length does not match csc_indptr[-1]')
        self.device = int(device)
        self._h = C.c_void_p()
        check(_lib.lib().rr_plan_create(self.n, ptr(indptr), ptr(indices) if indices.size else None,
                                        self.device, C.byref(self._h)))
        self._indptr, self._indices = indptr, indices
        info = np.zeros(8, dtype=np.int64)
        check(_lib.lib().rr_plan_info(self._h, ptr(info)))
        self.n_edges, self.depth, self.widest_level, self.n_headwaters, self.n_outlets = (int(v) for v in info[1:6])
        self.identity_order = bool(info[6])
        self.n_inner = self.n - self.n_headwaters

    def close(self) -> None:
        if getattr(self, '_h', None) is not None and self._h.value:
            _lib.lib().rr_plan_destroy(self._h)
            self._h = C.c_void_p()

    def __del__(self):
        try:
            self.close()
        except Exception:
            pass

    def __enter__(self):
        return self

    def __exit__(self, *exc):
        self.close()

    def layout(self):
        perm = np.empty(self.n, dtype=np.int32)
        lag = np.empty(self.n, dtype=np.int32)
        child_ptr = np.empty(self.n + 1, dtype=np.int32)
        check(_lib.lib().rr_plan_layout(self._h, ptr(perm), ptr(lag), ptr(child_ptr)))
        return perm, lag, child_ptr

    def tile_info(self) -> dict:
        info = np.zeros(8, dtype=np.int64)
        check(_lib.lib().rr_plan_tile_info(self._h, ptr(info)))
        return dict(ok=bool(info[0]), block=int(info[1]), positions=int(info[2]), ghosts=int(info[3]), tiles=int(info[4]),
                    levels=int(info[5]), threads=int(info[6]), batch_rows=int(info[7]))

    def tile_layout(self) -> dict:
        t = self.tile_info()
        nt, npos = t['tiles'], t['positions']
        out = dict(tile_ptr=np.empty(nt + 1, np.int32), tile_level=np.empty(nt, np.int32), perm=np.empty(npos, np.int32),
                   lag=np.empty(npos, np.int32), cfirst=np.empty(npos, np.int32), ccnt=np.empty(npos, np.uint32),
                   xpos=np.empty(npos, np.int32))
        check(_lib.lib().rr_plan_tile_layout(self._h, *(ptr(out[k]) for k in ('tile_ptr', 'tile_level', 'perm', 'lag', 'cfirst',
                                                                               'ccnt', 'xpos'))))
        return out

    def set_options(self, rows_per_chunk: int = 0, sample_every: int = -1) -> None:
        check(_lib.lib().rr_plan_set_options(self._h, int(rows_per_chunk), int(sample_every)))

    def set_row_format(self, in32_big_endian: bool = False, out32_big_endian: bool = False) -> None:
        check(_lib.lib().rr_plan_set_row_format(self._h, int(bool(in32_big_endian)), int(bool(out32_big_endian))))

    def profile(self) -> dict:
        p = np.zeros(10, dtype=np.float64)
        check(_lib.lib().rr_plan_profile(self._h, ptr(p)))
        return dict(launches=int(p[0]), sampled=int(p[1]), sampled_ms=float(p[2]), min_ms=float(p[3]),
                    max_ms=float(p[4]), sampled_reaches=float(p[5]), region_ms=float(p[6]), reach_steps=float(p[7]),
                    brackets=int(p[8]), ticks_per_launch=int(p[9]))

    def profile_aux(self) -> dict:
        a = np.zeros(12, dtype=np.float64)
        check(_lib.lib().rr_plan_profile_aux(self._h, ptr(a)))
        names = ('k_rec_in', 'k_rec_out', 'k_tile (skeleton)', 'k_rec_out (holes)')
        return {nm: dict(launches=int(a[3 * k]), sampled=int(a[3 * k + 1]), sampled_ms=float(a[3 * k + 2])) for k, nm in enumerate(names) if a[3 * k] > 0}

    def set_coeffs(self, lhs_off_data, c2, c3, c4_dt=None) -> None:
        lhs = _f64(lhs_off_data, 'lhs_off_data')
        c2, c3 = _f64(c2, 'c2'), _f64(c3, 'c3')
        if lhs.shape != (self.n_edges,) or c2.shape != (self.n,) or c3.shape != (self.n,):
            raise ValueError('coefficient arrays do not match the plan (lhs_off_data per CSC entry, c2/c3 per reach)')
        c4 = None
        if c4_dt is not None:
            c4 = _f64(c4_dt, 'c4_dt')
            if c4.shape != (self.n,):
                raise ValueError('c4_dt must have one value per reach')
        check(_lib.lib().rr_plan_set_coeffs(self._h, ptr(lhs) if lhs.size else None, ptr(c2), ptr(c3), ptr(c4)))

    def set_unit_weights(self, c1=None, a_data=None) -> None:
        if c1 is None and a_data is None:
            check(_lib.lib().rr_plan_set_unit_weights(self._h, None, None))
            return
        c1, a = _f64(c1, 'c1'), _f64(a_data, 'a_data')
        if c1.shape != (self.n,) or a.shape != (self.n_edges,):
            raise ValueError('c1 must have one value per reach and a_data one per CSC entry')
        check(_lib.lib().rr_plan_set_unit_weights(self._h, ptr(c1), ptr(a) if a.size else None))

    def rapid_route(self, q_t, qlateral, discharge_array, num_substeps: int) -> None:
        ql = np.ascontiguousarray(qlateral, dtype=np.float64)
        if ql.ndim != 2 or ql.shape[1] != self.n:
            raise ValueError(f'qlateral must have shape (T, {self.n})')
        T = ql.shape[0]
        _inplace_f64(q_t, 'q_t', (self.n,))
        _inplace_f64(discharge_array, 'discharge_array', (T, self.n))
        check(_lib.lib().rr_rapid_route(self._h, ptr(q_t), ptr(ql), ptr(discharge_array), T, int(num_substeps)))

    def muskingum_route(self, q_t, discharge_array, num_output_steps: int, num_routing_per_output: int) -> None:
        _inplace_f64(q_t, 'q_t', (self.n,))
        _inplace_f64(discharge_array, 'discharge_array', (int(num_output_steps), self.n))
        check(_lib.lib().rr_muskingum_route(self._h, ptr(q_t), ptr(discharge_array), int(num_output_steps),
                                            int(num_routing_per_output)))

    def unit_route(self, q_ch, q_full, convolved_lateral, discharge_array, num_substeps: int) -> None:
        conv = np.ascontiguousarray(convolved_lateral, dtype=np.float64)
        if conv.ndim != 2 or conv.shape[1] != self.n:
            raise ValueError(f'convolved_lateral must have shape (T, {self.n})')
        T = conv.shape[0]
        _inplace_f64(q_ch, 'q_ch', (self.n_inner,))
        _inplace_f64(q_full, 'q_full', (self.n_inner,))
        _inplace_f64(discharge_array, 'discharge_array', (T, self.n))
        check(_lib.lib().rr_unit_route(self._h, ptr(q_ch), ptr(q_full), ptr(conv), ptr(discharge_array), T,
                                       int(num_substeps)))

    def reserve(self, mode: int, T: int, num_substeps: int = 1, host_rows: bool = False, plain_rows: bool = True, f32_out: bool = False, uh: bool = False) -> dict:
        info = np.zeros(8, dtype=np.int64)
        check(_lib.lib().rr_plan_reserve(self._h, int(mode), int(T), int(num_substeps), int(bool(host_rows)) | (0 if plain_rows else 2) | (4 if f32_out else 0) | (8 if uh else 0), ptr(info)))
        if int(info[0]) == 0 and int(T) * int(num_substeps) >= 32 and self.n > 0 and not getattr(self, '_warned_streaming', False):
            import logging
            self._warned_streaming = True
            logging.getLogger('river_route_amd').warning(
                'routing %d reaches (network depth %d) with the streaming kernel k_tick: the time-tiled kernel does not apply to this call '
                '(record ring too large for the device, per-edge weights, or a reach with more tributaries than a tile holds); '
                'expect about a third of its rate', self.n, self.depth)
        return dict(tiled=int(info[0]) == 1, direct=int(info[0]) == 2, ticks_per_launch=int(info[1]), ring_chunks=int(info[2]), work_bytes=int(info[3]),
                    staging_bytes=int(info[4]), pinned_bytes=int(info[5]), pipeline_ticks=int(info[6]), ring_bytes=int(info[7]))

    def direct_info(self) -> dict:
        info = np.zeros(8, dtype=np.int64)
        why = C.create_string_buffer(256)
        check(_lib.lib().rr_plan_direct_info(self._h, ptr(info), C.cast(why, C.c_void_p), 256))
        return dict(ok=bool(info[0]), tiles=int(info[1]), holes=int(info[2]), outlets=int(info[3]), skeleton_positions=int(info[4]),
                    skeleton_tiles=int(info[5]), skeleton_levels=int(info[6]), window_rows=int(info[7]), why=why.value.decode())

    def direct_layout(self) -> dict:
        nt = self.direct_info()['tiles']
        out = dict(tile_c0=np.empty(nt, np.int32), tile_nc=np.empty(nt, np.int32), tile_lag_lo=np.empty(nt, np.int32), tile_span=np.empty(nt, np.int32),
                   delay=np.empty(self.n, np.int32), up3=np.empty(self.n, np.int32), xinfo=np.empty(self.n, np.int32))
        check(_lib.lib().rr_plan_direct_layout(self._h, *(ptr(out[k]) for k in ('tile_c0', 'tile_nc', 'tile_lag_lo', 'tile_span', 'delay', 'up3', 'xinfo'))))
        return out

    def last_kernel(self) -> str:
        return ('tick', 'tile', 'direct', 'tile_ensemble')[int(_lib.lib().rr_plan_last_kernel(self._h))]

    def rapid_route_dev(self, q_t, qlateral, ql_rows, discharge, out_rows, T, num_substeps, stream=None) -> None:
        self.reserve(MODE_RAPID, T, num_substeps)
        check(_lib.lib().rr_rapid_route_dev(self._h, ptr(q_t), ptr(qlateral), int(ql_rows), ptr(discharge),
                                            int(out_rows), int(T), int(num_substeps), stream))

    def rapid_adjoint_work_bytes(self, T: int, num_substeps: int = 1) -> int:
        out = C.c_int64(0)
        check(_lib.lib().rr_rapid_adjoint_work_bytes(self._h, int(T), int(num_substeps), C.byref(out)))
        return int(out.value)

    def rapid_adjoint_dev(self, q0, lateral, lat_rows, discharge, grad_out, grad_qfinal, grad_lateral, grad_q0, grad_coef, work,
                          work_bytes, T, num_substeps, stream=None) -> None:
        check(_lib.lib().rr_rapid_adjoint_dev(self._h, ptr(q0), ptr(lateral), int(lat_rows), ptr(discharge), ptr(grad_out),
                                              ptr(grad_qfinal), ptr(grad_lateral), ptr(grad_q0), ptr(grad_coef), ptr(work),
                                              int(work_bytes), int(T), int(num_substeps), stream))

    def rapid_adjoint_batch_work_bytes(self, members: int, T: int, num_substeps: int = 1) -> int:
        out = C.c_int64(0)
        check(_lib.lib().rr_rapid_adjoint_batch_work_bytes(self._h, int(members), int(T), int(num_substeps), C.byref(out)))
        return int(out.value)

    def rapid_adjoint_batch_dev(self, members, q0, q0_pitch, lateral, lat_rows, lat_pitch, discharge, grad_out, out_pitch, grad_qfinal,
                                grad_lateral, grad_q0, grad_coef, work, work_bytes, T, num_substeps, stream=None) -> None:
        check(_lib.lib().rr_rapid_adjoint_batch_dev(self._h, int(members), ptr(q0), int(q0_pitch), ptr(lateral), int(lat_rows), int(lat_pitch),
                                                    ptr(discharge), ptr(grad_out), int(out_pitch), ptr(grad_qfinal), ptr(grad_lateral),
                                                    ptr(grad_q0), ptr(grad_coef), ptr(work), int(work_bytes), int(T), int(num_substeps),
                                                    stream))

    def unit_adjoint_work_bytes(self, T: int, num_substeps: int = 1) -> int:
        out = C.c_int64(0)
        check(_lib.lib().rr_unit_adjoint_work_bytes(self._h, int(T), int(num_substeps), C.byref(out)))
        return int(out.value)

    def unit_adjoint_dev(self, q_ch0, q_full0, lateral, lat_rows, discharge, grad_out, grad_qch_final, grad_qfull_final, grad_lateral,
                         grad_qch0, grad_qfull0, grad_coef, work, work_bytes, T, num_substeps, stream=None) -> None:
        check(_lib.lib().rr_unit_adjoint_dev(self._h, ptr(q_ch0), ptr(q_full0), ptr(lateral), int(lat_rows), ptr(discharge), ptr(grad_out),
                                             ptr(grad_qch_final), ptr(grad_qfull_final), ptr(grad_lateral), ptr(grad_qch0), ptr(grad_qfull0),
                                             ptr(grad_coef), ptr(work), int(work_bytes), int(T), int(num_substeps), stream))

    def unit_adjoint_batch_work_bytes(self, members: int, T: int, num_substeps: int = 1) -> int:
        out = C.c_int64(0)
        check(_lib.lib().rr_unit_adjoint_batch_work_bytes(self._h, int(members), int(T), int(num_substeps), C.byref(out)))
        return int(out.value)

    def unit_adjoint_batch_dev(self, members, q_ch0, q_full0, state_pitch, lateral, lat_rows, lat_pitch, discharge, grad_out, out_pitch,
                               grad_qch_final, grad_qfull_final, grad_lateral, grad_qch0, grad_qfull0, grad_coef, work, work_bytes, T,
# ... 343 lines not shown
```

Before: 121.1 billion.

## Route eligible headwater reaches inside the record-ingest pass instead of the tile kernel

Headwater reaches (no upstream children) that sit off tile boundaries and outside wide tiles are marked eligible. Their linear recurrence is evaluated inside the k_rec_in transpose kernel, with the carry kept in a per-column device buffer. The tile kernel then sees these positions flagged as ghost-like with zeroed coefficients, so the serial tile recurrence should do less work. In exchange it adds more metadata and coefficient buffers, extra LDS in the ingest kernel, and a plan-time marking pass. It is enabled by default only for lean single-substep, single-member Rapid and Unit runs.

```diff
diff --git a/include/rr_hip.h b/include/rr_hip.h
--- a/include/rr_hip.h
+++ b/include/rr_hip.h
@@ -33,6 +33,7 @@
 int rr_plan_layout(const rr_plan *plan, int32_t *perm, int32_t *lag, int32_t *child_ptr);
 
 int rr_plan_tile_info(const rr_plan *plan, int64_t info[8]);
+int rr_plan_inpass_info(const rr_plan *plan, int64_t info[5]);
 int rr_plan_tile_layout(const rr_plan *plan, int32_t *tile_ptr, int32_t *tile_level, int32_t *perm, int32_t *lag,
                         int32_t *cfirst, uint32_t *ccnt, int32_t *xpos);
 
diff --git a/river_route_amd/_lib.py b/river_route_amd/_lib.py
--- a/river_route_amd/_lib.py
+++ b/river_route_amd/_lib.py
@@ -78,6 +78,7 @@
     'rr_plan_info': (C.c_int, [_vp, _vp]),
     'rr_plan_layout': (C.c_int, [_vp, _vp, _vp, _vp]),
     'rr_plan_tile_info': (C.c_int, [_vp, _vp]),
+    'rr_plan_inpass_info': (C.c_int, [_vp, _vp]),
     'rr_plan_tile_layout': (C.c_int, [_vp, _vp, _vp, _vp, _vp, _vp, _vp, _vp]),
     'rr_plan_direct_info': (C.c_int, [_vp, _vp, _vp, _i64]),
     'rr_plan_direct_layout': (C.c_int, [_vp, _vp, _vp, _vp, _vp, _vp, _vp, _vp]),
diff --git a/river_route_amd/csrc/rr_engine.hip b/river_route_amd/csrc/rr_engine.hip
--- a/river_route_amd/csrc/rr_engine.hip
+++ b/river_route_amd/csrc/rr_engine.hip
@@ -36,7 +36,7 @@
                         P->d_c3, P->d_c4, P->d_x, P->d_isum, P->d_qch, P->d_a2, P->d_c1own, P->d_z, P->d_ring, P->d_stage, P->d_mrows,
                         P->d_slot_a[0], P->d_slot_a[1], P->d_slot_b[0], P->d_slot_b[1], P->d_m_index[0], P->d_m_index[1],
                         P->d_dtiles, P->d_dlane, P->d_dsend_ptr, P->d_dsend_lane, P->d_dcoef, P->d_dq, P->d_ktmeta, P->d_kpmeta, P->d_kperm, P->d_kholecol, P->d_kcoef, P->d_ksq, P->d_kss, P->d_ksi, P->d_ksqch,
-                        P->d_kholemeta, P->d_kghostmeta, P->d_esq, P->d_ess, P->d_esi, P->d_adj_down};
+                        P->d_kholemeta, P->d_kghostmeta, P->d_esq, P->d_ess, P->d_esi, P->d_adj_down, P->d_pmeta_hw, P->d_coef_hw, P->d_hwcoef, P->d_hwq};
         for (void *p : ptrs) if (p) (void)hipFree(p);
         P->pipe.destroy();
         for (hipEvent_t e : P->ev) (void)hipEventDestroy(e);
@@ -53,6 +53,7 @@
     *out = nullptr;
     rr_plan *P = new (std::nothrow) rr_plan();
     if (!P) return fail(RR_E_ALLOC, "rr_plan_create: out of memory");
+    if (const char *e = getenv("RR_HW_INPASS")) P->hw_inpass = atoi(e) != 0;
     if (const char *e = getenv("RR_WAVE")) { P->wave_enabled = atoi(e) != 0; P->wave_forced = atoi(e) == 1; }
     if (const char *e = getenv("RR_REC_BATCHES")) { P->rec_batches = std::max(1, std::min(kRecMaxLaunchBatches, atoi(e))); P->rec_batches_forced = true; }
     if (const char *e = getenv("RR_WAVE_K")) P->wave_K = std::max(kRec, atoi(e) / kRec * kRec);
@@ -119,15 +120,10 @@
         if (!rc && P->tp.ok) {
             const rr::TilePlan &TP = P->tp;
             const int64_t np = TP.np;
-            std::vector<int2> cm(n);
-            for (int64_t i = 0; i < n; ++i)
-                cm[i] = make_int2(TP.inv[i], (TP.lag[TP.inv[i]] & kLagMask) | (H.child_ptr[H.inv[i] + 1] == H.child_ptr[H.inv[i]] ? kColHeadwater : 0));
             std::vector<int32_t> inner_idx;
             inner_idx.reserve(ni);
             for (int64_t i = 0; i < n; ++i) if (H.child_ptr[H.inv[i] + 1] > H.child_ptr[H.inv[i]]) inner_idx.push_back((int32_t)i);
-            rc = dev_alloc(&P->d_colmeta, n);
-            if (!rc) rc = dev_upload(P->d_colmeta, cm);
-            if (!rc) rc = dev_alloc(&P->d_inner_idx, ni);
+            rc = dev_alloc(&P->d_inner_idx, ni);
             if (!rc) rc = dev_upload(P->d_inner_idx, inner_idx);
             if (!rc) rc = upload_tile_meta(P, TP.lag, TP.xpos, TP.tile_flags);
             for (int32_t f : TP.tile_flags) P->n_wide_tiles += (f & kTileWide) ? 1 : 0;
@@ -137,6 +133,9 @@
             if (!rc) rc = dev_upload(P->d_tinv, TP.inv);
             if (!rc) rc = dev_alloc(&P->d_coef, 3 * np);
             if (!rc) rc = dev_alloc(&P->d_coef_unit, 3 * np);
+            if (!rc) rc = dev_alloc(&P->d_coef_hw, 3 * np);
+            if (!rc) rc = dev_alloc(&P->d_hwcoef, 3 * n);
+            if (!rc) rc = dev_alloc(&P->d_hwq, n);
             if (!rc) rc = dev_alloc(&P->d_sq, np);
             if (!rc) rc = dev_alloc(&P->d_ss, np);
             if (!rc) rc = dev_alloc(&P->d_si, np);
@@ -189,6 +188,19 @@
     const rr::TilePlan &T = P->tp;
     info[0] = T.ok ? 1 : 0; info[1] = T.block; info[2] = T.np; info[3] = T.n_ghost; info[4] = T.n_tiles; info[5] = T.n_levels;
     info[6] = P->wave_threads; info[7] = kRecRows;
+    return RR_OK;
+}
+
+int rr_plan_inpass_info(const rr_plan *P, int64_t info[5])
+{
+    if (!P || !info) return fail(RR_E_INVALID, "rr_plan_inpass_info: null argument");
+    for (int k = 0; k < 5; ++k) info[k] = 0;
+    info[0] = P->hw_inpass ? 1 : 0;
+    if (!P->tp.ok) return RR_OK;
+    std::vector<int32_t> lag(P->tp.lag);
+    for (int32_t i : P->ghost_reach) lag[P->tp.inv[i]] |= kGhostBit;
+    std::vector<uint8_t> elig;
+    rr::mark_inpass_headwaters(P->tp, lag, kGhostBit, elig, info + 1);
     return RR_OK;
 }
 
diff --git a/river_route_amd/csrc/rr_exec.hpp b/river_route_amd/csrc/rr_exec.hpp
--- a/river_route_amd/csrc/rr_exec.hpp
+++ b/river_route_amd/csrc/rr_exec.hpp
@@ -78,6 +78,7 @@
     size_t max_samples = 0;
     int64_t members = 0;
     int64_t ring_stride = 0;
+    bool hw = false;
 };
 
 struct HostPipe {
@@ -140,6 +141,13 @@
     bool export_inside = false;
     double *d_coef = nullptr;
     double *d_coef_unit = nullptr;
+    bool hw_inpass = true;
+    std::vector<uint8_t> hw_elig;
+    int64_t hw_counts[4] = {0, 0, 0, 0};
+    int4 *d_pmeta_hw = nullptr;
+    double *d_coef_hw = nullptr;
+    double *d_hwcoef = nullptr;
+    double *d_hwq = nullptr;
     std::vector<double> h_coef;
     int32_t n_wide_tiles = 0;
     double *d_sq = nullptr, *d_ss = nullptr, *d_si = nullptr, *d_sqch = nullptr;
@@ -250,6 +258,18 @@
     if (!rc && !P->d_pmeta) rc = dev_alloc(&P->d_pmeta, TP.np);
     if (!rc) rc = dev_upload(P->d_tmeta, tm);
     if (!rc) rc = dev_upload(P->d_pmeta, pm);
+    rr::mark_inpass_headwaters(TP, lag, kGhostBit, P->hw_elig, P->hw_counts);
+    if (!P->hw_inpass) { P->hw_elig.assign((size_t)TP.np, 0); P->hw_counts[0] = 0; }
+    for (int64_t p = 0; p < TP.np; ++p) if (P->hw_elig[p]) pm[p].x |= kTileGhostBit;
+    const rr::HostPlan &H = P->h;
+    std::vector<int2> cm((size_t)H.n);
+    for (int64_t i = 0; i < H.n; ++i)
+        cm[i] = make_int2(TP.inv[i], (TP.lag[TP.inv[i]] & kLagMask) | (H.child_ptr[H.inv[i] + 1] == H.child_ptr[H.inv[i]] ? kColHeadwater : 0) |
+                                         (P->hw_elig[TP.inv[i]] ? kColInpass : 0));
+    if (!rc && !P->d_pmeta_hw) rc = dev_alloc(&P->d_pmeta_hw, TP.np);
+    if (!rc) rc = dev_upload(P->d_pmeta_hw, pm);
+    if (!rc && !P->d_colmeta) rc = dev_alloc(&P->d_colmeta, H.n);
+    if (!rc) rc = dev_upload(P->d_colmeta, cm);
     return rc;
 }
 
@@ -260,6 +280,17 @@
     for (int32_t i : P->ghost_reach) { const int64_t p = P->tp.inv[i]; coef[3 * p] = coef[3 * p + 1] = coef[3 * p + 2] = 0.0; }
     int rc = dev_upload(P->d_coef, coef);
     if (rc) return rc;
+    {
+        std::vector<double> hw(coef);
+        for (int64_t p = 0; p < P->tp.np; ++p)
+            if (P->hw_elig[p]) hw[3 * p] = hw[3 * p + 1] = hw[3 * p + 2] = 0.0;
+        rc = dev_upload(P->d_coef_hw, hw);
+        if (rc) return rc;
+        std::vector<double> col(3 * (size_t)P->h.n);
+        for (int64_t i = 0; i < P->h.n; ++i) for (int k = 0; k < 3; ++k) col[3 * i + k] = coef[3 * (int64_t)P->tp.inv[i] + k];
+        rc = dev_upload(P->d_hwcoef, col);
+        if (rc) return rc;
+    }
     for (int64_t p = 0; p < P->tp.np; ++p)
         if ((P->tp.ccnt[p] & 0xFFFFu) == 0) coef[3 * p] = coef[3 * p + 1] = coef[3 * p + 2] = 0.0;
     return dev_upload(P->d_coef_unit, coef);
@@ -646,6 +677,8 @@
         w.tiles = P->d_tmeta; w.pos = P->d_pmeta; w.coef = P->d_coef;
         w.sq = P->d_sq; w.ss = P->d_ss; w.si = P->d_si; w.sqch = P->d_sqch;
         w.np = (int32_t)TP.np; w.KC = (int32_t)S.KC;
+        S.hw = P->hw_inpass && P->lean_enabled && nsub == 1 && S.members == 0 &&
+               (mode == Mode::Unit || (mode == Mode::Rapid && !io.runoff && !io.uh_kernel));
         if (S.members > 0) {
             if (S.members > P->ens_cap || (S.rec_chunks * kRec * TP.np) * S.members > P->ring_cap) { S.open = false; return fail(RR_E_STATE, "route: the ensemble was not reserved"); }
             S.ring_stride = S.rec_chunks * kRec * TP.np;
@@ -664,10 +697,10 @@
                 (long long)n, (long long)T, (long long)(S.KC * kRec), P->dp.n_tiles, P->direct_window, (long long)P->dp.n_holes, (long long)P->dp.n_exports,
                 (long long)P->dp.skel.np, P->dp.skel.n_tiles, P->dp.skel.n_levels, (long long)S.rec_chunks, (double)S.rec_chunks * kRec * P->dp.skel.np * 8 / 1e9);
     else if (getenv("RR_VERBOSE"))
-        fprintf(stderr, "rr: n=%lld T=%lld nsub=%lld tiled=%d K=%lld tiles=%d levels=%d block=%d ghosts=%lld ring_chunks=%lld (%.1f GB) rec_batches=%lld lds=%zu\n",
+        fprintf(stderr, "rr: n=%lld T=%lld nsub=%lld tiled=%d K=%lld tiles=%d levels=%d block=%d ghosts=%lld ring_chunks=%lld (%.1f GB) rec_batches=%lld lds=%zu hw_inpass=%d (%lld of %lld headwater positions)\n",
                 (long long)n, (long long)T, (long long)nsub, (int)(S.kernel == Kernel::Tile), (long long)(S.KC * kRec), P->tp.n_tiles, P->tp.n_levels, P->tp.block,
                 (long long)P->tp.n_ghost, (long long)S.rec_chunks, S.kernel == Kernel::Tile ? (double)S.rec_chunks * kRec * P->tp.np * 8 / 1e9 : 0.0,
-                (long long)S.rec_nb, tile_lds_bytes(P->wave_threads));
+                (long long)S.rec_nb, tile_lds_bytes(P->wave_threads), (int)S.hw, (long long)(S.hw ? P->hw_counts[0] : 0), (long long)P->hw_counts[1]);
     if (S.kernel == Kernel::Tick) {
         const int64_t lag_rows = (dmax + nsub - 1) / nsub;
         S.ring_rows = S.in_place ? 0 : std::min<int64_t>(T, lag_rows + 2 * C + 2);
@@ -864,7 +897,13 @@
     } else {
         w.tile_filter = lean ? 1 : 0;
         w.coef = (lean && unit) ? coef_unit : coef;
+        const int4 *const pos = w.pos;
+        if (lean && S.hw) {
+            w.pos = P->d_pmeta_hw;
+            if (!unit) w.coef = P->d_coef_hw;
+        }
         hipLaunchKernelGGL(tile_kernel(unit, S.nsub > 1, lean, S.mode == Mode::Muskingum), g, dim3((unsigned)P->wave_threads), lds_bytes, S.stream, w);
+        w.pos = pos;
         if (lean && n_wide > 0) {
             w.tile_filter = 2; w.coef = coef;
             hipLaunchKernelGGL(tile_kernel(unit, false, false), g, dim3((unsigned)P->wave_threads), lds_bytes, S.stream, w);
@@ -958,6 +997,8 @@
     ra.swizzle = in ? 0 : 1;
     const dim3 gp((unsigned)((n + kRecInCols - 1) / kRecInCols));
     const bool sub = S.nsub > 1;
+    const bool hw = in && S.hw && S.mode == Mode::Rapid;
+    if (hw) { ra.hw_coef = P->d_hwcoef; ra.hw_carry = P->d_hwq; }
     hipStream_t st = rec_stream(P);
     const int aux = aux_begin(P, in ? 0 : 1, st);
     if (S.members > 0) {
@@ -989,9 +1030,11 @@
                            rec_in_uh_lds_bytes(uh_padded_taps(S.io.uh_nks), count), st, ra, ua);
     } else if (in && ra.rows_in32) {
         if (sub) hipLaunchKernelGGL((k_rec_in<true, true>), gp, dim3(kRecInThreads), 0, st, ra);
+        else if (hw) hipLaunchKernelGGL((k_rec_in<false, true, false, true>), gp, dim3(kRecInThreads), 0, st, ra);
         else hipLaunchKernelGGL((k_rec_in<false, true>), gp, dim3(kRecInThreads), 0, st, ra);
     } else if (in) {
         if (sub) hipLaunchKernelGGL(k_rec_in<true>, gp, dim3(kRecInThreads), 0, st, ra);
+        else if (hw) hipLaunchKernelGGL((k_rec_in<false, false, false, true>), gp, dim3(kRecInThreads), 0, st, ra);
         else hipLaunchKernelGGL(k_rec_in<false>, gp, dim3(kRecInThreads), 0, st, ra);
     } else {
         launch_rec_out(ra, sub, n, st);
@@ -1261,6 +1304,7 @@
         const bool d = P->sch.kernel == Kernel::Direct;
         const int64_t np = d ? P->dp.skel.np : P->tp.np;
         if (d) HIPCHK(hipMemcpyAsync(P->d_dq, d_q, (size_t)n * sizeof(double), hipMemcpyDeviceToDevice, stream));
+        if (!d && P->hw_inpass) HIPCHK(hipMemcpyAsync(P->d_hwq, d_q, (size_t)n * sizeof(double), hipMemcpyDeviceToDevice, stream));
         if (np > 0)
             hipLaunchKernelGGL(k_tile_state_in, grid1(np), dim3(kBlock), 0, stream, d ? P->d_ksq : P->d_sq, d ? P->d_kss : P->d_ss, d ? P->d_ksi : P->d_si, d_q,
                                d ? P->d_kperm : P->d_tperm, d ? P->d_kpmeta : P->d_pmeta, (int32_t)np);
diff --git a/river_route_amd/csrc/rr_kernels_rec.hpp b/river_route_amd/csrc/rr_kernels_rec.hpp
--- a/river_route_amd/csrc/rr_kernels_rec.hpp
+++ b/river_route_amd/csrc/rr_kernels_rec.hpp
@@ -24,6 +24,8 @@
     int32_t clamp;
     uint32_t in32_sel, out32_sel;
     int32_t batches;
+    const double *hw_coef;
+    double *hw_carry;
 };
 
 struct RecEnsArgs : RecPermArgs {
@@ -43,6 +45,7 @@
 }
 
 constexpr int32_t kColHeadwater = 1 << 30;
+constexpr int32_t kColInpass = 1 << 29;
 
 constexpr int kRecTileRows = 16 * kRecBatch + 15;
 constexpr int kRecTileLd = kRecCols + 1;
@@ -104,14 +107,16 @@
     }
 }
 
-template <bool SUB, bool IN32 = false, bool ENS = false>
+template <bool SUB, bool IN32 = false, bool ENS = false, bool HW = false>
 __global__ __launch_bounds__(kRecInThreads, 4) void k_rec_in(const RecArgsOf<ENS> args)
 {
+    static_assert(!HW || (!SUB && !ENS), "headwaters are routed by the in-pass only with one sub-step per row, single member");
     const RecPermArgs &a = member_args(args);
     constexpr int R = kRecTileRows, G = kRecInThreads / kRecInCols;
     __shared__ double tile[R * (kRecInCols + 1)];
     __shared__ int2 smeta[kRecInCols];
     __shared__ double sscale[kRecInCols];
+    __shared__ double shw[5][HW ? kRecInCols : 1];
     const int tid = threadIdx.x;
     auto first_row = [&](int64_t tick_first) -> int64_t {
         uint32_t sub_unused;
@@ -135,9 +140,14 @@
         double v[RPT];
         int2 cm = make_int2(-1, 0);
         double cs = 1.0;
+        double hc1 = 0.0, hc2 = 0.0, hc3 = 0.0, hq = 0.0;
         if (tid < kRecInCols) {
             cm = live ? a.colmeta[i] : make_int2(-1, 0);
             cs = a.scale ? a.scale[i] : 1.0;
+            if constexpr (HW) {
+                hc1 = a.hw_coef[3 * i]; hc2 = a.hw_coef[3 * i + 1]; hc3 = a.hw_coef[3 * i + 2];
+                hq = a.hw_carry[i];
+            }
         }
 #pragma unroll
         for (int q = 0; q < RPT; ++q) v[q] = load(row_first + min(r0 + q * G, need - 1));
@@ -147,9 +157,46 @@
             const int64_t row = row_first + r;
             if (r < R) tile[r * (kRecInCols + 1) + c] = (row >= 0 && row < a.T && live) ? v[q] : 0.0;
         }
-        if (tid < kRecInCols) { smeta[c] = cm; sscale[c] = cs; }
+        if (tid < kRecInCols) {
+            smeta[c] = cm; sscale[c] = cs;
+            if constexpr (HW) { shw[0][c] = hc1; shw[1][c] = hc2; shw[2][c] = hc3; shw[3][c] = hq; shw[4][c] = (cm.y & kColInpass) ? 1.0 : cs; }
+        }
     }
     __syncthreads();
+    auto route_headwaters = [&](int64_t first) {
+        if (tid >= kRecInCols) return;
+        const int2 m = smeta[tid];
+        if (m.x < 0 || !(m.y & kColInpass)) return;
+        const double c1 = shw[0][tid], c2 = shw[1][tid], c3 = shw[2][tid], sc = sscale[tid];
+        double q = shw[3][tid];
+        const int r_first = 15 - (m.y & 15);
+        double *col = tile + r_first * (kRecInCols + 1) + tid;
+        const int64_t t_first = first + r_first;
+        constexpr int kBlk = 8;
+#pragma unroll 1
+        for (int b = 0; b < kRecRows; b += kBlk) {
+            double x[kBlk];
+#pragma unroll
+            for (int k = 0; k < kBlk; ++k) x[k] = col[(b + k) * (kRecInCols + 1)] * sc;
+            const int64_t t0 = t_first + b;
+            if (t0 >= 0 && t0 + kBlk <= a.T) {
+#pragma unroll
+                for (int k = 0; k < kBlk; ++k) { q = __builtin_fma(c1, 0.0, __builtin_fma(c2, 0.0, __builtin_fma(c3, q, x[k]))); x[k] = q; }
+            } else {
+#pragma unroll
+                for (int k = 0; k < kBlk; ++k) {
+                    const bool in = t0 + k >= 0 && t0 + k < a.T;
+                    const double qn = __builtin_fma(c1, 0.0, __builtin_fma(c2, 0.0, __builtin_fma(c3, q, x[k])));
+                    q = in ? qn : q; x[k] = in ? qn : x[k];
+                }
+            }
+#pragma unroll
+            for (int k = 0; k < kBlk; ++k) col[(b + k) * (kRecInCols + 1)] = x[k];
+        }
+        shw[3][tid] = q;
+    };
+    const double *wscale = HW ? shw[4] : sscale;
+    if constexpr (HW) { route_headwaters(tick_first); __syncthreads(); }
     const int nb = a.batches > 1 ? a.batches : 1;
     for (int b = 1; b < nb; ++b) {
         constexpr int NPT = kRecRows / G, KPT = 3;
@@ -161,7 +208,7 @@
             const int r = keep + r0 + q * G;
             if (r < need) v[q] = load(row_next + r);
         }
-        write_records<SUB, kRecInThreads, kRecBatch, true, kRecInCols>(a, tile, col0, a.batch + b - 1, tick_first, row_first, smeta, sscale);
+        write_records<SUB, kRecInThreads, kRecBatch, true, kRecInCols>(a, tile, col0, a.batch + b - 1, tick_first, row_first, smeta, wscale);
 #pragma unroll
         for (int q = 0; q < KPT; ++q) {
             const int r = r0 + q * G;
@@ -181,8 +228,12 @@
         }
         __syncthreads();
         tick_first = tick_next; row_first = row_next;
-    }
-    write_records<SUB, kRecInThreads, kRecBatch, true, kRecInCols>(a, tile, col0, a.batch + nb - 1, tick_first, row_first, smeta, sscale);
+        if constexpr (HW) { route_headwaters(tick_first); __syncthreads(); }
+    }
+    if constexpr (HW) {
+        if (tid < kRecInCols && live && (smeta[tid].y & kColInpass)) a.hw_carry[i] = shw[3][tid];
+    }
+    write_records<SUB, kRecInThreads, kRecBatch, true, kRecInCols>(a, tile, col0, a.batch + nb - 1, tick_first, row_first, smeta, wscale);
 }
 
 struct UhArgs {
diff --git a/river_route_amd/csrc/rr_plan.cpp b/river_route_amd/csrc/rr_plan.cpp
--- a/river_route_amd/csrc/rr_plan.cpp
+++ b/river_route_amd/csrc/rr_plan.cpp
@@ -358,6 +358,22 @@
     T.ok = true;
 }
 
+int64_t mark_inpass_headwaters(const TilePlan &T, const std::vector<int32_t> &lag, int32_t boundary_ghost, std::vector<uint8_t> &eligible, int64_t counts[4])
+{
+    eligible.assign((size_t)T.np, 0);
+    int64_t c[4] = {0, 0, 0, 0};
+    for (int64_t p = 0; p < T.np; ++p) {
+        if ((lag[p] & kTileGhost) || (T.ccnt[p] & 0xFFFFu) != 0) continue;
+        ++c[1];
+        if (lag[p] & (kTileExport | boundary_ghost)) { ++c[2]; continue; }
+        if (T.tile_flags[T.tile_of[p]] & 1) { ++c[3]; continue; }
+        eligible[p] = 1;
+        ++c[0];
+    }
+    if (counts) for (int k = 0; k < 4; ++k) counts[k] = c[k];
+    return c[0];
+}
+
 void build_direct_plan(const std::vector<int32_t> &down, const std::vector<int32_t> &lag_of, int32_t lanes, int32_t wmax, int32_t skel_block,
                        DirectPlan &D, const std::vector<uint8_t> *ghost, const std::vector<int32_t> *export_slot)
 {
diff --git a/river_route_amd/csrc/rr_plan.hpp b/river_route_amd/csrc/rr_plan.hpp
--- a/river_route_amd/csrc/rr_plan.hpp
+++ b/river_route_amd/csrc/rr_plan.hpp
@@ -62,6 +62,9 @@
 void build_tile_plan(const std::vector<int32_t> &down, const std::vector<int32_t> &lag_of, int32_t block, TilePlan &out,
                      const std::vector<uint8_t> *big = nullptr, bool skeleton_only = false);
 
+int64_t mark_inpass_headwaters(const TilePlan &tp, const std::vector<int32_t> &lag, int32_t boundary_ghost, std::vector<uint8_t> &eligible,
+                               int64_t counts[4] = nullptr);
+
 constexpr int32_t kDirectHole = 1 << 30;
 constexpr int32_t kDirectSenderShift = 8, kDirectDelayMask = 0xFF;
 constexpr int32_t kDirectExport = 1 << 15;
diff --git a/river_route_amd/engine.py b/river_route_amd/engine.py
--- a/river_route_amd/engine.py
+++ b/river_route_amd/engine.py
@@ -82,6 +82,12 @@
         check(_lib.lib().rr_plan_tile_info(self._h, ptr(info)))
         return dict(ok=bool(info[0]), block=int(info[1]), positions=int(info[2]), ghosts=int(info[3]), tiles=int(info[4]),
                     levels=int(info[5]), threads=int(info[6]), batch_rows=int(info[7]))
+
+    def inpass_info(self) -> dict:
+        info = np.zeros(5, dtype=np.int64)
+        check(_lib.lib().rr_plan_inpass_info(self._h, ptr(info)))
+        return dict(enabled=bool(info[0]), eligible=int(info[1]), headwater_positions=int(info[2]), mirrored_or_boundary=int(info[3]),
+                    wide_tile=int(info[4]))
 
     def tile_layout(self) -> dict:
         t = self.tile_info()
```

Measured after the change: 130.1 billion, median of 6. 7.4% higher.
